# niclasborlin/dbat

Measured on AMD Instinct MI355X. Metric: LM iterations/sec, higher is better.
Workload: dtype f64

## Files before the change

### dbat_amd/csrc/dbat_core.hip

```cpp
#include <hip/hip_runtime.h>
#include <rocblas/rocblas.h>
#include <rocsolver/rocsolver.h>
#include <rccl/rccl.h>

#include <chrono>
#include <cmath>
#include <cstdio>
#include <cstdlib>
#include <memory>
#include <string>
#include <thread>
#include <type_traits>
#include <utility>
#include <atomic>
#include <vector>

#include "../../include/dbat_hip.h"
#include "chol_df.hpp"
#include "kernels.hpp"
#include "sig.hpp"
#include "heavy.hpp"
#include "plan.hpp"
#include "resect.hpp"
#include "robust.hpp"
// ... 82 lines not shown
    DevBuf<double> io_fixed, px, cam_w, z_prw, z_prv, o_uv, o_w;
    bool deterministic = false;
    DevBuf<double> det_cam_part, det_io_part, det_rr, det_u;
    DevBuf<int32_t> det_cam_chunks;
    DevBuf<double> o_rhs;
    bool uv_pre = false;
    DevBuf<uint8_t> z_est, z_mine, o_lc, o_pidx;
    DevBuf<int32_t> tile_batch, tile_cam_start, tile_cams, tile_io_start, tile_iocols;
    DevBuf<uint8_t> tile_io_simple;
    DevBuf<uint8_t> tile_cam_io;
    DevBuf<int32_t> sg_chunk, sg_tile_chunk0, sg_gcam;
    int64_t sg_nchunks = 0;
    DevBuf<uint8_t> sg_lc;
    DevBuf<double> sg_uv, sg_w;
    bool use_sig = false;
    int sig_rb = 4;
    int tile_ncx = 6;
    int64_t ntiles = 0;
    size_t lds_tile2 = 0, lds_tile3 = 0;
    int tile2_pc = TILE2_PC;
    bool use_tile2 = true;
    enum class TileRoute { none, sig, tile3, tile2 } route = TileRoute::none;
    DevBuf<int64_t> o_row, batch_start, x2z, giant_start, cm_chunk_start;
    DevBuf<int32_t> cm_pt, cm_chunk_cam, tile_order;
    DevBuf<double> cm_uv, cm_w;
    int64_t n_cm_chunks = 0, n_cm_chunks_all = 0;
    DevBuf<double> giant_W;
    int64_t ngiant = 0;
    bool use_heavy = false;
    HeavyDev hv{};
    DevBuf<int32_t> hv_obs_dst, hv_pt_io0, hv_io_dst, hv_io_pt, hv_pt_y, hv_grp_nb, hv_grp_row, hv_task, hv_ops;
    DevBuf<uint8_t> hv_obs_ld, hv_obs_ioloc, hv_io_ld;
    DevBuf<double> hv_Z;
    int giant_threads = 256;
    DevBuf<CamRec> cams, cams_f;
    bool cams_at_lin = false;

    const char *env_df_trace = nullptr;
    DevBuf<unsigned> gctr;
    DevBuf<double> gpart, rpart;
    DevBuf<double> z, zt, dz, zlin, vtmp, vtmp2, xbuf;
    DevBuf<double> red;
    DevBuf<double> jn2c, dscale, rhs, Vinv, gp, jn2p, partial, scal;
    DevBuf<int> info;
    DevBuf<double> linv, ldiag;
    DataflowChol dfchol;
    DataflowChol dfchol_ip;
    bool use_perm = true;
    bool mg_subtree = false;
    DevBuf<uint8_t> piv_have;
    bool chol_in_place = false;
    int64_t ldS = 0;
    CholEnvelope env;
    DevBuf<unsigned long long> pivmm;
    double *S = nullptr, *g_red = nullptr, *g_c = nullptr, *diagU = nullptr, *red_scal = nullptr;
    int64_t red_count = 0;
    DevBuf<double> pk;
    DevBuf<int> col_bend;
    DevBuf<int64_t> col_off;
    int64_t pk_s_count = 0;
    int env_tail0 = 0;
    int64_t nb = 0, nobs = 0;
    int grid_obs = 1, grid_z = 1, grid_zs = 1;
    size_t lds_build = 0, lds_back = 0, lds_cov = 0;
    ncclComm_t nccl = nullptr;
    dbat_hip_allreduce_fn allreduce = nullptr;
    void *allreduce_user = nullptr;
    DevBuf<double> zgather;
    bool multi() const { return nccl != nullptr || allreduce != nullptr; }
    struct { const void *kernel; size_t bytes; } lds_opt_in[8] = {};
    int n_lds_opt_in = 0;
    template <auto K, class... A>
    void launch(dim3 grid, dim3 block, size_t lds, A &&...args) {
        if (lds > 65536) {
            int i = 0;
            while (i < n_lds_opt_in && lds_opt_in[i].kernel != (const void *)K) ++i;
            if (i == n_lds_opt_in || lds_opt_in[i].bytes < lds) {
                if (i == 8) throw DeviceError{"internal: more kernels with over 64 KiB of LDS than the opt-in table holds"};
                HIPCHK(hipFuncSetAttribute((const void *)K, hipFuncAttributeMaxDynamicSharedMemorySize, (int)lds));
                lds_opt_in[i] = {(const void *)K, lds};
                n_lds_opt_in = std::max(n_lds_opt_in, i + 1);
            }
        }
        dbat::launch<K>(grid, block, lds, stream, std::forward<A>(args)...);
    }
    double f_lin = 0, trace_jtj = 0, lambda_lin = 0;
    int scale_lin = 0;
    bool have_lin = false;
    bool s_valid = false;
    bool s_dense_dirty = true;
    int n_res_evals = 0, n_lin = 0, n_solves = 0, n_trace_only = 0;

    ~Core() {
        for (auto &e : ev) if (e) (void)hipEventDestroy(e);
        for (auto &e : kev) if (e) (void)hipEventDestroy(e);
        for (auto &e : st_ev) if (e) (void)hipEventDestroy(e);
        dfchol.release(); dfchol_ip.release();
        if (hpin) (void)hipHostFree(hpin);
        if (nccl) (void)ncclCommDestroy(nccl);
        if (blas) rocblas_destroy_handle(blas);
        if (stream) (void)hipStreamDestroy(stream);
    }

    void init(const dbat_hip_problem &pb) {
        const bool init_clock = env_int("DBAT_HIP_PLAN_STATS", 0) >= 2;
        auto t_init = std::chrono::steady_clock::now();
        auto lapi = [&](const char *what) {
            if (!init_clock) return;
            const auto now = std::chrono::steady_clock::now();
            fprintf(stderr, "[create clock] %-60s %8.1f ms\n", what, std::chrono::duration<double, std::milli>(now - t_init).count());
            t_init = now;
        };
        device = pb.device;
        HIPCHK(hipSetDevice(pb.device));
        {
            hipDeviceProp_t prop;
            HIPCHK(hipGetDeviceProperties(&prop, pb.device));
            n_cu = std::max(1, prop.multiProcessorCount);
        }
        HIPCHK(hipStreamCreate(&stream));
        HIPCHK(hipHostMalloc((void **)&hpin, 64 * sizeof(double), hipHostMallocMapped | hipHostMallocCoherent));
        memset(hpin, 0, 64 * sizeof(double));
        {
            const double big = 1e300;
            memcpy(&hpin[48], &big, 8); hpin[49] = 0.0; memcpy(&hpin[50], &big, 8); hpin[51] = 0.0;
        }
        lapi("device, stream, pinned mailbox (the first call of a process initialises the HIP runtime: ~0.1 s)");
        for (auto &e : ev) HIPCHK(hipEventCreate(&e));
        for (auto &e : kev) HIPCHK(hipEventCreate(&e));
        lapi("events");
        nb = (int64_t)P.batch_start.size() - 1;
        nobs = (int64_t)P.o_cam.size();
        cam_ncol.upload(P.cam_ncol); cam_col.upload(P.cam_col); cam_iorow.upload(P.cam_iorow);
        cam_eo_est.upload(P.cam_eo_est); io_src.upload(P.io_src); io_fixed.upload(P.io_fixed);
        px.upload(P.px); cam_w.upload(P.cam_w);
        z_est.upload(P.z_est); z_mine.upload(P.z_mine); z_prw.upload(P.z_prw); z_prv.upload(P.z_prv);
        o_cam.upload(P.o_cam); o_pt.upload(P.o_pt); o_uv.upload(P.o_uv); o_w.upload(P.o_w);
        o_seg.upload(P.o_seg); o_row.upload(P.o_row); batch_start.upload(P.batch_start);
        x2z.upload(P.x2z);
        o_lc.upload(P.o_lc); o_pidx.upload(P.o_pidx); tile_batch.upload(P.tile_batch); tile_cam_start.upload(P.tile_cam_start); tile_cams.upload(P.tile_cams);
        tile_io_start.upload(P.tile_io_start); tile_iocols.upload(P.tile_iocols); tile_cam_io.upload(P.tile_cam_io);
        tile_ncx = P.shared_eo ? MAXCOL : (P.ncolmax <= 6 ? 6 : (P.ncolmax <= 14 ? 14 : (P.ncolmax <= 15 ? 15 : MAXCOL)));
        ntiles = (P.CMAX && P.nb_tiled > 0) ? (int64_t)P.tile_batch.size() - 1 : 0;
        d.nc = P.nc; d.np = P.np; d.nIOrows = P.nIOrows; d.nK = P.nK; d.nP = P.nP; d.nIOu = P.nIOu;
        d.ncolmax = P.ncolmax; d.BT = P.BT; d.NS = P.NS; d.NZ = P.NZ; d.nobs = nobs; d.nb = nb;
        d.cam_ncol = cam_ncol.p; d.cam_col = cam_col.p; d.cam_iorow = cam_iorow.p; d.cam_eo_est = cam_eo_est.p;
        d.io_src = io_src.p; d.io_fixed = io_fixed.p; d.px = px.p; d.cam_w = cam_w.p;
        d.z_est = z_est.p; d.z_mine = z_mine.p; d.z_prw = z_prw.p; d.z_prv = z_prv.p;
        d.o_cam = o_cam.p; d.o_pt = o_pt.p; d.o_uv = o_uv.p; d.o_w = P.uniform_w ? nullptr : o_w.p;
        pw = !P.uniform_w;
        d.o_seg = o_seg.p; d.o_row = o_row.p; d.batch_start = batch_start.p;
        d.CMAX = P.CMAX; d.ablate = env_int("DBAT_HIP_ABLATE", 0); d.trace_only = 0;
        d.any_prior = 0;
        for (double w : P.z_prw) if (w > 0) { d.any_prior = 1; break; }
        d.deterministic = 0; d.det_cam_part = d.det_io_part = d.det_rr = d.det_u = nullptr; d.det_cam_chunks = nullptr;
        env_df_trace = env_get("DBAT_HIP_DF_TRACE");
        d.ntiles = (int)ntiles; d.o_lc = o_lc.p; d.o_pidx = o_pidx.p;
        tile_order.upload(P.tile_order); d.tile_order = tile_order.p;
        cm_pt.upload(P.cm_pt); cm_uv.upload(P.cm_uv); cm_w.upload(P.cm_w);
        cm_chunk_cam.upload(P.cm_chunk_cam); cm_chunk_start.upload(P.cm_chunk_start);
        n_cm_chunks = P.n_cm_chunks_tiled; n_cm_chunks_all = (int64_t)P.cm_chunk_cam.size();
        ngiant = P.giant_start.empty() ? 0 : (int64_t)P.giant_start.size() - 1;
        if (ngiant > 0) {
            giant_start.upload(P.giant_start);
            giant_W.alloc((size_t)(P.giant_start.back() - P.giant_start.front()) * P.ncolmax * 3);
        }
        d.ngiant = (int)ngiant; d.giant_start = giant_start.p; d.giant_W = giant_W.p;
        use_heavy = P.hv_ok;
        if (use_heavy) {
            hv_obs_dst.upload(P.hv_obs_dst); hv_obs_ld.upload(P.hv_obs_ld); hv_obs_ioloc.upload(P.hv_obs_ioloc);
            hv_pt_io0.upload(P.hv_pt_io0); hv_io_dst.upload(P.hv_io_dst); hv_io_ld.upload(P.hv_io_ld); hv_io_pt.upload(P.hv_io_pt);
            hv_pt_y.upload(P.hv_pt_y); hv_grp_nb.upload(P.hv_grp_nb); hv_grp_row.upload(P.hv_grp_row);
            hv_task.upload(P.hv_task); hv_ops.upload(P.hv_ops);
            hv_Z.alloc((size_t)P.hv_z_doubles);
            HIPCHK(hipMemset(hv_Z.p, 0, (size_t)P.hv_z_doubles * sizeof(double)));
            hv.obs_dst = hv_obs_dst.p; hv.obs_ld = hv_obs_ld.p; hv.obs_ioloc = hv_obs_ioloc.p; hv.pt_io0 = hv_pt_io0.p;
            hv.io_dst = hv_io_dst.p; hv.io_ld = hv_io_ld.p; hv.io_pt = hv_io_pt.p; hv.pt_y = hv_pt_y.p;
            hv.grp_nb = hv_grp_nb.p; hv.grp_row = hv_grp_row.p; hv.task = hv_task.p; hv.ops = hv_ops.p;
            hv.obs0 = P.hv_obs0; hv.pt0 = P.hv_pt0; hv.ntasks = P.hv_ntasks; hv.max_batch_slots = P.hv_max_batch_slots;
        }
        if (const char *e = env_get("DBAT_HIP_GIANT_THREADS")) giant_threads = atoi(e);
        d.tile_batch = tile_batch.p; d.tile_cam_start = tile_cam_start.p; d.tile_cams = tile_cams.p;
        d.tile_io_start = tile_io_start.p; d.tile_iocols = tile_iocols.p; d.tile_cam_io = tile_cam_io.p;
        tile_io_simple.upload(P.tile_io_simple); d.tile_io_simple = P.tile_io_simple.empty() ? nullptr : tile_io_simple.p;
        use_sig = P.sg_ok && ntiles > 0 && tile_ncx <= 14;
        if (use_sig) {
            sg_chunk.upload(P.sg_chunk); sg_tile_chunk0.upload(P.sg_tile_chunk0); sg_lc.upload(P.sg_lc); sg_gcam.upload(P.sg_gcam);
            sg_nchunks = (int64_t)P.sg_chunk.size() / 8;
            sg_uv.upload(P.sg_uv);
            if (!P.uniform_w) sg_w.upload(P.sg_w);
            sig_rb = P.sg_rows_max <= 64 ? 4 : 5;
        }
        lapi("allocations and uploads of the plan");
        cams.alloc(P.nc); cams_f.alloc(P.nc);
        z.alloc(P.NZ); zt.alloc(P.NZ); dz.alloc(P.NZ); zlin.alloc(P.NZ); vtmp.alloc(P.NZ); vtmp2.alloc(P.NZ);
        xbuf.alloc(std::max<int64_t>(P.n, 1));
        ldS = ((P.NS + 1 + 7) / 8) * 8;
        d.ldS = ldS;
        const int64_t s_count = ldS * (P.NS + 1);
        red_count = s_count + 3 * P.NS + 8;
        red.alloc(red_count);
        S = red.p; g_red = S + s_count; g_c = g_red + P.NS; diagU = g_c + P.NS; red_scal = diagU + P.NS;
        ldiag.alloc(P.NS);
        {
            std::vector<int> first((size_t)P.NS, 0);
            for (int c = 0; c < P.nc; ++c)
                for (int k = 0; k < 6; ++k) first[(size_t)6 * c + k] = 6 * P.cam_first[c];
            if (P.shared_eo) env.build_dense((int)P.NS);
            else env.build((int)P.NS, 6 * P.nc, first);
            {
                const int NSi = (int)P.NS;
                std::vector<int> cb((size_t)NSi);
                std::vector<int64_t> co((size_t)NSi + 1, 0);
                env_tail0 = env.tail0;
                for (int c = 0; c < NSi; ++c) {
                    const int be = c >= env.tail0 ? c : std::min(std::max(env.band_end[c / CHOL_NB], c + 1), env.tail0);
                    cb[c] = be;
                    co[c + 1] = co[c] + (be - c) + (NSi - std::max(env.tail0, be));
                }
                pk_s_count = co[NSi];
                col_bend.upload(cb); col_off.upload(co);
            }
            use_perm = !P.shared_eo;
            if (!dfchol_ip.setup_inplace(env, ldS)) throw DeviceError{"out of device memory (Cholesky schedule)"};
            if (use_perm) {
                if (!dfchol.setup_permuted(P.nc, P.nIOu, P.cam_adj.data(), P.cam_adj_words, P.nd, P.rank))
                    throw DeviceError{"out of device memory (Cholesky schedule)"};
            }
            mg_subtree = P.mg_subtree && use_perm && dfchol.two_phase;
            if (mg_subtree) {
                std::vector<uint8_t> have((size_t)P.NS, 0);
                for (int c = 0; c < P.nc; ++c)
                    if (P.nd.cam_owner[c] < 0 || P.nd.cam_owner[c] == P.rank) for (int k = 0; k < 6; ++k) have[(size_t)6 * c + k] = 1;
                for (int64_t z = 6 * (int64_t)P.nc; z < P.NS; ++z) have[z] = 1;
                piv_have.upload(have);
            }
            linv.alloc(std::max(dfchol_ip.linv_doubles(), use_perm ? dfchol.linv_doubles() : (size_t)0));
        }
        lapi("envelope, schedules of the factorisation");
        jn2c.alloc(P.NS); dscale.alloc(P.NS); rhs.alloc(P.NS);
        Vinv.alloc((size_t)6 * P.np); gp.alloc((size_t)3 * P.np); jn2p.alloc((size_t)3 * P.np);
        HIPCHK(hipMemset(Vinv.p, 0, (size_t)6 * P.np * 8));
        HIPCHK(hipMemset(gp.p, 0, (size_t)3 * P.np * 8));
        HIPCHK(hipMemset(jn2p.p, 0, (size_t)3 * P.np * 8));
        grid_obs = (int)std::max<int64_t>(1, std::min<int64_t>(cdiv(nobs, 256), env_grid_obs()));
        grid_z = (int)std::max<int64_t>(1, std::min<int64_t>(cdiv(P.NZ, 256), 2048));
        grid_zs = (int)std::max<int64_t>(1, std::min<int64_t>(cdiv(P.NZ, 2048), 256));
        scal.alloc((size_t)16 + 4 * (size_t)P.nranks);
        HIPCHK(hipMemset(scal.p, 0, ((size_t)16 + 4 * (size_t)P.nranks) * sizeof(double)));
        info.alloc(1);
        pivmm.alloc(4);
        gctr.alloc(16); HIPCHK(hipMemset(gctr.p, 0, 16 * sizeof(unsigned)));
        rpart.alloc((size_t)grid_obs);
        gpart.alloc((size_t)8 * std::max<int64_t>(std::max<int64_t>(grid_z, cdiv(P.NS, 256)), 2048));
        lds_build = ((size_t)P.BT * P.ncolmax * 3 + (size_t)P.BT * 18) * sizeof(double);
        lds_back = (size_t)P.BT * 6 * sizeof(double);
        lds_cov = ((size_t)P.BT * P.ncolmax * 3 + (size_t)P.BT * 6) * sizeof(double);
        tile2_pc = TILE2_PC;
        static_assert(Plan::PMAX == 256 / 2, "k_build_tile2 / k_build_tile3 lay out NPROD / 2 points per batch");
        lds_tile2 = ((size_t)TILE2_NBUF * 3 * tile2_pc * TILE_LD + (size_t)2 * Plan::PMAX * 9 + (size_t)Plan::PMAX * 15 + TILE_LD) * sizeof(double);
        lds_tile3 = ((size_t)TILE3_NBUF * 3 * TILE3_PC * TILE_LD + (size_t)2 * Plan::PMAX * 9 + (size_t)2 * Plan::PMAX * 9 + TILE_LD) * sizeof(double);
        use_tile2 = P.BT == 256 && P.ncolmax <= 15;
        if (ntiles <= 0) route = TileRoute::none;
        else if (use_sig) route = TileRoute::sig;
        else if (use_tile2 && !P.with_io && tile_ncx == 6) route = TileRoute::tile3;
        else if (use_tile2 && (tile_ncx == 14 || tile_ncx == 15)) route = TileRoute::tile2;
        else throw DeviceError{"internal: tiles without a tile kernel"};
        partial.alloc((size_t)4 * std::max<int64_t>(std::max<int64_t>(std::max<int64_t>(nb + ntiles + ngiant + (int64_t)P.sg_chunk.size() / 8, n_cm_chunks_all), 2048), 1));
        HIPCHK(hipMemcpy(z.p, P.z0.data(), P.NZ * 8, hipMemcpyHostToDevice));
        HIPCHK(hipMemset(dz.p, 0, P.NZ * 8));
        HIPCHK(hipMemset(zt.p, 0, P.NZ * 8));
        precompute_image_side();
        HIPCHK(hipDeviceSynchronize());
        lapi("work arrays, image side");
    }

    void precompute_image_side() {
        uv_pre = !P.with_io;
        d.o_uv_raw = o_uv.p; d.uv_pre = uv_pre ? 1 : 0;
        if (!uv_pre || nobs == 0) return;
        prep_cams(z.p, cams_f.p);
        if (!o_rhs.p) o_rhs.alloc((size_t)2 * nobs);
        with_value<2, 3, 4, 5>(P.model, [&](auto M) {
            launch<k_uv_to_rhs<M>>(dim3((unsigned)cdiv(nobs, 256)), dim3(256), 0, d.nK, d.nP, cams_f.p, nobs, o_cam.p, o_uv.p, o_rhs.p);
            if (n_cm_chunks_all > 0) launch<k_uv_to_rhs_cm<M>>(dim3((unsigned)n_cm_chunks_all), dim3(256), 0, d.nK, d.nP, cams_f.p, cm_chunk_cam.p, cm_chunk_start.p, cm_uv.p);
            if (use_sig && sg_nchunks > 0) launch<k_uv_to_rhs_sig<M>>(dim3((unsigned)sg_nchunks), dim3(64), 0, d.nK, d.nP, cams_f.p, sg_chunk.p, sg_gcam.p, sg_uv.p);
        });
        d.o_uv = o_rhs.p;
    }

    void set_values(bool io_changed) {
        robust_reset();
        HIPCHK(hipMemcpyAsync(z.p, P.z0.data(), P.NZ * 8, hipMemcpyHostToDevice, stream));
        HIPCHK(hipMemcpyAsync(io_fixed.p, P.io_fixed.data(), P.io_fixed.size() * 8, hipMemcpyHostToDevice, stream));
        if (d.any_prior) {
            HIPCHK(hipMemcpyAsync(z_prw.p, P.z_prw.data(), P.NZ * 8, hipMemcpyHostToDevice, stream));
            HIPCHK(hipMemcpyAsync(z_prv.p, P.z_prv.data(), P.NZ * 8, hipMemcpyHostToDevice, stream));
        }
        HIPCHK(hipStreamSynchronize(stream));
        if (uv_pre && io_changed && nobs > 0) {
            HIPCHK(hipMemcpy(cm_uv.p, P.cm_uv.data(), P.cm_uv.size() * 8, hipMemcpyHostToDevice));
            if (use_sig && sg_nchunks > 0) HIPCHK(hipMemcpy(sg_uv.p, P.sg_uv.data(), P.sg_uv.size() * 8, hipMemcpyHostToDevice));
            d.o_uv = o_uv.p;
            precompute_image_side();
            HIPCHK(hipStreamSynchronize(stream));
        }
        cams_at_lin = false; have_lin = false; s_valid = false; pend_build = false; lin_pending = false;
        lambda_lin = 0; scale_lin = 0; f_lin = 0; trace_jtj = 0; near_singular = false; chol_in_place = false; replicate_next = false;
        n_res_evals = n_lin = n_solves = n_trace_only = 0;
    }

    static int env_grid_obs() { return std::min(std::max(1, env_int("DBAT_HIP_GRID_OBS", 1536)), 1 << 20); }

    int64_t tile_kernel_mfma() const {
        if (route == TileRoute::none) return 0;
        int64_t n = 0;
        if (route == TileRoute::sig) {
            for (int64_t t = 0; t < ntiles; ++t) {
                const int nio = tile_ncx > 6 ? P.tile_io_start[t + 1] - P.tile_io_start[t] : 0;
                for (int64_t q = P.sg_tile_chunk0[t]; q < P.sg_tile_chunk0[t + 1]; ++q) {
                    const int npts = P.sg_chunk[8 * q + 1], k = P.sg_chunk[8 * q + 2];
                    const int ppr = std::min(SIG_PPR, 64 / std::max(k, 1)), rbk = (6 * k + nio + 1 + 15) >> 4;
                    for (int p0 = 0; p0 < npts; p0 += ppr) n += (int64_t)((3 * std::min(ppr, npts - p0) + 3) >> 2) * (rbk * (rbk + 1) / 2);
                }
            }
            return n;
        }
        const int pc = route == TileRoute::tile3 ? TILE3_PC : tile2_pc;
        for (int64_t b = 0; b < P.nb_tiled; ++b) {
            const int64_t o1 = P.batch_start[b + 1];
            const int npts = o1 > P.batch_start[b] ? (int)P.o_pidx[o1 - 1] + 1 : 0;
            for (int p0 = 0; p0 < npts; p0 += pc) n += (int64_t)((3 * std::min(pc, npts - p0) + 3) >> 2) * 36;
        }
        return n;
    }

    bool lin_pending = false;
    bool det_timeout_pending = false;
    unsigned long long mb_seq = 0;
    bool mb_armed = false;
    void sync() {
        bool done = false;
        if (mb_armed) {
            volatile unsigned long long *slot = reinterpret_cast<volatile unsigned long long *>(hpin) + 63;
            const auto t_end = std::chrono::steady_clock::now() + std::chrono::milliseconds(20);
            for (;;) {
                for (int spin = 0; spin < 512 && !done; ++spin) { done = *slot == mb_seq; if (!done) cpu_relax(); }
                if (done || std::chrono::steady_clock::now() >= t_end) break;
            }
            __atomic_thread_fence(__ATOMIC_ACQUIRE);
            mb_armed = false;
        }
        if (!done) HIPCHK(hipStreamSynchronize(stream));
        if (det_timeout_pending) {
            det_timeout_pending = false;
            unsigned n_to = 0;
            memcpy(&n_to, hpin + 60, sizeof(unsigned));
            if (n_to) {
                HIPCHK(hipMemsetAsync(gctr.p + 7, 0, sizeof(unsigned), stream));
                throw DeviceError{"deterministic mode: " + std::to_string(n_to) + " chunk(s) of the signature kernel gave up waiting for their turn at "
                                  "the tile (spin cap): the sums of this linearisation are not order-fixed"};
            }
        }
        if (lin_pending) {
            f_lin = 0.5 * hpin[32];
            trace_jtj = hpin[34] + hpin[33];
            lin_pending = false;
        }
    }
    void mark(int i) { if (timing) HIPCHK(hipEventRecord(kev[i], stream)); }
    std::vector<hipEvent_t> st_ev;
    std::vector<int> st_id;
    bool st_on = false;
    void stage(int id) {
        if (!st_on) return;
        if (st_id.size() == st_ev.size()) { hipEvent_t e; HIPCHK(hipEventCreate(&e)); st_ev.push_back(e); }
        HIPCHK(hipEventRecord(st_ev[st_id.size()], stream));
        st_id.push_back(id);
    }
    void stages_begin() { st_id.clear(); st_on = true; stage(4); }
    void stages_end(double *out5) {
        stage(4);
        st_on = false;
        HIPCHK(hipStreamSynchronize(stream));
        for (int i = 0; i < 5; ++i) out5[i] = 0.0;
        for (size_t i = 0; i + 1 < st_id.size(); ++i) {
            float ms = 0;
            HIPCHK(hipEventElapsedTime(&ms, st_ev[i], st_ev[i + 1]));
            out5[st_id[i]] += 1e-3 * ms;
        }
    }
    void allreduce_system() {
        if (!multi()) return;
        const int64_t nvec = 3 * P.NS + 8;
        if (!pk.p) pk.alloc((size_t)(pk_s_count + nvec));
        launch<k_pack_envelope>(dim3((unsigned)P.NS), dim3(256), 0, S, ldS, (int)P.NS, env_tail0,
                           col_bend.p, col_off.p, pk.p, 1);
        HIPCHK(hipMemcpyAsync(pk.p + pk_s_count, g_red, nvec * sizeof(double), hipMemcpyDeviceToDevice, stream));
        do_allreduce(pk.p, pk_s_count + nvec);
        launch<k_pack_envelope>(dim3((unsigned)P.NS), dim3(256), 0, S, ldS, (int)P.NS, env_tail0,
                           col_bend.p, col_off.p, pk.p, 0);
        HIPCHK(hipMemcpyAsync(g_red, pk.p + pk_s_count, nvec * sizeof(double), hipMemcpyDeviceToDevice, stream));
    }
    void do_allreduce(double *buf, int64_t count) {
        if (nccl) {
            NCCLCHK(ncclAllReduce(buf, buf, (size_t)count, ncclDouble, ncclSum, nccl, stream));
        } else if (allreduce) {
            if (allreduce(allreduce_user, buf, count, (void *)stream) != 0) throw DeviceError{"all-reduce callback failed"};
        }
    }
    const double *gathered(const double *z_dev) {
        if (!multi()) return z_dev;
        if (!zgather.p) zgather.alloc((size_t)P.NZ);
        launch<k_mask_owned>(dim3((unsigned)cdiv(P.NZ, 256)), dim3(256), 0, P.NZ, z_mine.p, z_dev, zgather.p);
        do_allreduce(zgather.p, P.NZ);
        return zgather.p;
    }
    void read_scal(double *host, int n) {
        if (n <= 32) {
            HIPCHK(hipMemcpyAsync(hpin, scal.p, n * sizeof(double), hipMemcpyDeviceToHost, stream));
            sync();
            memcpy(host, hpin, n * sizeof(double));
            return;
        }
        HIPCHK(hipMemcpyAsync(host, scal.p, n * sizeof(double), hipMemcpyDeviceToHost, stream));
        sync();
    }
    void prep_cams(const double *zz, CamRec *into = nullptr) {
        if (!into) { into = cams.p; cams_at_lin = false; }
        launch<k_cam_prep>(dim3((unsigned)cdiv(P.nc, 64)), dim3(64), 0, d, zz, into);
    }
    void x_to_z(const double *x_host, double *z_dev) {
        HIPCHK(hipMemcpyAsync(z_dev, P.z0.data(), P.NZ * 8, hipMemcpyHostToDevice, stream));
        if (P.n) {
            HIPCHK(hipMemcpyAsync(xbuf.p, x_host, P.n * 8, hipMemcpyHostToDevice, stream));
            launch<k_scatter_x>(dim3((unsigned)cdiv(P.n, 256)), dim3(256), 0, P.n, x2z.p, xbuf.p, z_dev);
        }
    }
    void z_to_x(const double *z_dev, double *x_host) {
        if (!P.n) return;
        stage(4);
        z_dev = gathered(z_dev);
        launch<k_gather_x>(dim3((unsigned)cdiv(P.n, 256)), dim3(256), 0, P.n, x2z.p, z_dev, xbuf.p);
        HIPCHK(hipMemcpyAsync(x_host, xbuf.p, P.n * 8, hipMemcpyDeviceToHost, stream));
        sync();
    }

    DevBuf<double> trace_dev;
    int trace_cap = 0, trace_n = 0;
    std::vector<uint8_t> trace_have;
    void trace_begin() { trace_n = 0; trace_have.clear(); }
    void trace_put(int k, const double *z_dev) {
        if (!P.n || k < 0) return;
        if (k >= trace_cap) {
            const int cap = std::max(8, std::max(2 * trace_cap, k + 1));
            DevBuf<double> nb;
            nb.alloc((size_t)P.n * cap);
            if (trace_cap > 0) HIPCHK(hipMemcpyAsync(nb.p, trace_dev.p, (size_t)P.n * trace_cap * 8, hipMemcpyDeviceToDevice, stream));
            HIPCHK(hipStreamSynchronize(stream));
            std::swap(trace_dev.p, nb.p);
            trace_cap = cap;
        }
        stage(4);
        z_dev = gathered(z_dev);
        launch<k_gather_x>(dim3((unsigned)cdiv(P.n, 256)), dim3(256), 0, P.n, x2z.p, z_dev, trace_dev.p + (size_t)P.n * k);
        if ((int)trace_have.size() <= k) trace_have.resize((size_t)k + 1, 0);
        trace_have[k] = 1;
        trace_n = std::max(trace_n, k + 1);
    }
    void trace_truncate(int n) { trace_n = std::min(trace_n, std::max(n, 0)); }
    int trace_download(double *host, int cap_cols) {
        const int nt = std::min(trace_n, cap_cols);
        if (!P.n || nt <= 0) return std::max(nt, 0);
        HIPCHK(hipMemcpyAsync(host, trace_dev.p, (size_t)P.n * nt * 8, hipMemcpyDeviceToHost, stream));
        HIPCHK(hipStreamSynchronize(stream));
        for (int k = 0; k < nt; ++k)
            if (!trace_have[k]) std::fill(host + (size_t)P.n * k, host + (size_t)P.n * (k + 1), NAN);
        if ((size_t)P.n * trace_cap * 8 > ((size_t)256 << 20)) {
            DevBuf<double> old;
            std::swap(old.p, trace_dev.p);
            trace_cap = 0;
        }
        return nt;
    }

    double eval_f_step(const double *x, double alpha, const double *pdir, double *out) {
        stage(3);
        if ((int64_t)cdiv(P.NZ, 256) < P.nc) { axpby(1.0, x, alpha, pdir, out); return eval_f(out, nullptr, nullptr); }
        launch<k_axpby_cams>(dim3((unsigned)cdiv(P.NZ, 256)), dim3(256), 0, d, 1.0, x, alpha, pdir, out, cams_f.p);
        return eval_f(out, nullptr, nullptr, true);
    }
    double eval_f(const double *zz, double *r_w_out, double *r_unw_out, bool cams_ready = false) {
        stage(3);
        if (!cams_ready) prep_cams(zz, cams_f.p);
        mark(6);
        const bool res_tail = n_cm_chunks_all > 0 && n_cm_chunks_all <= 512 && !d.any_prior && !multi() && !r_w_out && !r_unw_out;
        with_value<2, 3, 4, 5>(P.model, [&](auto M) {
            with_value<false, true>(uv_pre, [&](auto PRE) {
                if (n_cm_chunks_all > 0)
                    launch<k_residual_cm<M, PRE>>(dim3((unsigned)n_cm_chunks_all), dim3(256), 0, d, zz, cams_f.p, cm_pt.p, cm_uv.p, pw ? cm_w.p : (const double *)nullptr,
                                                  cm_chunk_cam.p, cm_chunk_start.p, partial.p, res_tail ? gctr.p + 1 : (unsigned *)nullptr, scal.p, hpin, res_tail ? ++mb_seq : 0ull);
                mark(7);
                if (r_w_out || r_unw_out) launch<k_residual<M, PRE>>(dim3(grid_obs), dim3(256), 0, d, zz, cams_f.p, rpart.p, r_w_out, r_unw_out);
            });
        });
        if (!res_tail)
            launch<k_prior_sq>(dim3(grid_zs), dim3(1024), 0, d, zz, gpart.p, gctr.p + 1, (const double *)partial.p, n_cm_chunks_all,
                               scal.p, multi() ? (double *)nullptr : hpin, ++mb_seq);
        double s;
        if (multi()) { do_allreduce(scal.p, 1); read_scal(&s, 1); }
        else { mb_armed = true; sync(); s = hpin[0]; }
        ++n_res_evals;
        return 0.5 * s;
    }

    int det_ncx() const { return P.ncolmax <= 6 ? 6 : (P.ncolmax <= 14 ? 14 : 15); }
    bool deterministic_supported() const { return P.nranks == 1 && !P.shared_eo && P.ncolmax <= 15 && n_cm_chunks_all > 0; }
    void set_deterministic(bool on) {
        if (on && !deterministic_supported())
            throw UsageError{"deterministic mode: one rank, no shared EO blocks (camera stations), at most nine estimated IO columns per camera"};
        if (on && !det_u.p) {
            const int nc = P.nc;
            det_cam_part.alloc((size_t)std::max<int64_t>(n_cm_chunks_all, 1) * DET_CP);
            det_io_part.alloc((size_t)nc * DET_IOP);
            det_rr.alloc((size_t)nc + 1 + DET_PRIOR_PARTS);
            det_u.alloc((size_t)P.NS + 1);
            std::vector<int32_t> cr((size_t)2 * (2 * nc + 1), 0);
            for (int part = 0; part < 2; ++part) {
                const int64_t q0 = part == 0 ? 0 : n_cm_chunks, q1 = part == 0 ? n_cm_chunks : n_cm_chunks_all;
                int32_t *r = cr.data() + part * (2 * nc + 1);
                for (int c = 0; c < nc; ++c) { r[2 * c] = (int32_t)q1; r[2 * c + 1] = (int32_t)q1; }
                for (int64_t q = q0; q < q1; ++q) {
                    const int c = P.cm_chunk_cam[q];
                    if (r[2 * c] == (int32_t)q1) r[2 * c] = (int32_t)q;
                    r[2 * c + 1] = (int32_t)q + 1;
                }
                for (int c = 0; c < nc; ++c) if (r[2 * c] == (int32_t)q1) r[2 * c + 1] = (int32_t)q1;
            }
            det_cam_chunks.upload(cr);
        }
        deterministic = on;
        d.deterministic = on ? 1 : 0;
        d.det_cam_part = det_cam_part.p; d.det_io_part = det_io_part.p; d.det_rr = det_rr.p; d.det_u = det_u.p;
        d.det_cam_chunks = det_cam_chunks.p;
    }
    const double *det_z = nullptr;
    void det_camera_side() {
        const int nio = (int)P.nIOu;
        const int ncx = det_ncx();
        with_value<6, 14, 15>(ncx, [&](auto NCX) { launch<k_det_cam_reduce<NCX>>(dim3((unsigned)P.nc), dim3(256), 0, d, cams.p, S, g_c, g_red, diagU); });
        if (ncx > 6 && nio > 0) launch<k_det_io_reduce<15>>(dim3((unsigned)(nio * (nio + 1) / 2 + nio)), dim3(256), 0, d, cams.p, nio, S, g_c, g_red, diagU);
        if (d.any_prior) launch<k_det_prior_sq>(dim3(DET_PRIOR_PARTS), dim3(256), 0, d, det_z);
        launch<k_det_rows>(dim3((unsigned)cdiv(P.NS, 256)), dim3(256), 0, d, (const double *)diagU);
        if (ncx == 6) launch<k_det_round_cam<6>>(dim3((unsigned)P.nc), dim3(256), 0, d, cams.p, 0, S, g_red);
        else launch<k_det_round_cam<15>>(dim3((unsigned)P.nc + 1), dim3(256), 0, d, cams.p, nio, S, g_red);
    }

    void cam_normal(const double *zz, int64_t q0, int64_t nq, int ncx) {
        const double *w = pw ? cm_w.p : (const double *)nullptr;
        with_value<2, 3, 4, 5>(P.model, [&](auto M) { with_value<6, 14, 15>(ncx, [&](auto NCX) {
            if constexpr (NCX == 6)
                launch<k_cam_normal6<M>>(dim3((unsigned)nq), dim3(256), 0, d, zz, cams.p, cm_pt.p, cm_uv.p, w, cm_chunk_cam.p + q0, cm_chunk_start.p + q0, S, g_c, g_red, diagU);
            else
                launch<k_cam_normal<M, NCX>>(dim3((unsigned)nq), dim3(256), 0, d, zz, cams.p, cm_pt.p, cm_uv.p, w, cm_chunk_cam.p + q0, cm_chunk_start.p + q0, S, g_c, g_red, diagU);
        }); });
    }

    void build_enqueue(const double *zz, double lambda, int scale) {
        stage(0);
        const bool fused_first = !s_dense_dirty && P.NS >= P.nc;
        if (!fused_first) prep_cams(zz);
        else cams_at_lin = false;
        bool pivmm_set = false;
        if (s_dense_dirty) {
            HIPCHK(hipMemsetAsync(red.p, 0, red_count * sizeof(double), stream));
            s_dense_dirty = false;
        } else {
            launch<k_envelope_cams>(dim3((unsigned)P.NS), dim3(256), 0, d, zz, cams.p, S, ldS, (int)P.NS, env_tail0, col_bend.p, g_red, pivmm.p);
            pivmm_set = true;
        }
        if (!pivmm_set) HIPCHK(hipMemcpyAsync(pivmm.p, hpin + 48, 4 * sizeof(double), hipMemcpyHostToDevice, stream));
        int64_t npart = 0;
        const bool det_list = deterministic && route != TileRoute::sig;
        const int64_t nb_tiled = det_list ? 0 : P.nb_tiled;
        if (deterministic) {
            cam_normal(zz, 0, n_cm_chunks_all, det_ncx());
            det_z = zz;
            det_camera_side();
        }
        if (ntiles > 0 && nb_tiled > 0) {
            npart = ntiles;
            if (!deterministic && use_tile2 && tile_ncx <= 15 && n_cm_chunks > 0) cam_normal(zz, 0, n_cm_chunks, tile_ncx);
            mark(0);
            with_value<2, 3, 4, 5>(P.model, [&](auto M) {
                if (route == TileRoute::sig) {
                    with_value<6, 14>(tile_ncx, [&](auto NCX) { with_value<4, 5>(sig_rb, [&](auto RB) { with_value<false, true>(pw, [&](auto PW) {
                        launch<k_build_sig<M, RB, NCX, PW>>(dim3((unsigned)std::min<int64_t>(ntiles, n_cu)), dim3(64 * sig_waves(RB, NCX > 6)), sig_lds_bytes(RB, NCX > 6),
                                                            d, zz, cams.p, lambda, scale, S, g_red, Vinv.p, gp.p, jn2p.p, partial.p, pivmm.p, sg_chunk.p, sg_tile_chunk0.p,
                                                            sg_lc.p, sg_uv.p, PW ? sg_w.p : (const double *)nullptr, gctr.p + 5);
                    }); }); });
                } else if (route == TileRoute::tile3) {
                    launch<k_build_tile3<M, TILE3_PC, TILE3_NBUF>>(dim3((unsigned)ntiles), dim3(768), lds_tile3, d, zz, cams.p, lambda, scale, S, g_red, Vinv.p, gp.p,
                                                                   jn2p.p, partial.p, pivmm.p);
                } else {
                    with_value<14, 15>(tile_ncx, [&](auto NCX) {
                        launch<k_build_tile2<M, NCX, TILE2_PC, TILE2_NBUF>>(dim3((unsigned)ntiles), dim3(512), lds_tile2, d, zz, cams.p, lambda, scale, S, g_c, g_red,
                                                                            diagU, Vinv.p, gp.p, jn2p.p, partial.p, pivmm.p);
                    });
                }
            });
            mark(1);
        }
        const bool no_tiles = !(ntiles > 0 && nb_tiled > 0);
        if (no_tiles) mark(0);
        const int64_t nb_lists = use_heavy ? P.nb_tiled : nb;
        if (nb_lists > nb_tiled) {
            with_value<2, 3, 4, 5>(P.model, [&](auto M) { with_value<false, true>(P.with_io, [&](auto IO) {
                launch<k_build<M, IO>>(dim3((unsigned)(nb_lists - nb_tiled)), dim3(P.BT), lds_build, d, zz, cams.p, lambda, scale, S, g_c, g_red, diagU, Vinv.p, gp.p,
                                       jn2p.p, partial.p + npart, pivmm.p, (int)nb_tiled);
            }); });
            npart += nb_lists - nb_tiled;
        }
        if (use_heavy) {
            mark(10);
            if (!deterministic && n_cm_chunks_all > n_cm_chunks) cam_normal(zz, n_cm_chunks, n_cm_chunks_all - n_cm_chunks, tile_ncx);
            if (nb > P.nb_tiled) {
                with_value<2, 3, 4, 5>(P.model, [&](auto M) { with_value<6, 14, 15>(tile_ncx, [&](auto NCX) {
                    launch<k_heavy_z<M, NCX>>(dim3((unsigned)(nb - P.nb_tiled)), dim3(256), heavy_z_lds_bytes(NCX, P.hv_max_batch_slots, deterministic), d, hv, zz,
                                              cams.p, lambda, scale, hv_Z.p, Vinv.p, gp.p, jn2p.p, partial.p + npart, pivmm.p, (int)P.nb_tiled);
                }); });
                npart += nb - P.nb_tiled;
            }
            if (ngiant > 0) {
                with_value<2, 3, 4, 5>(P.model, [&](auto M) { with_value<6, 14, 15>(tile_ncx, [&](auto NCX) {
                    launch<k_heavy_z_giant<M, NCX>>(dim3((unsigned)ngiant), dim3(giant_threads), 0, d, hv, zz, cams.p, lambda, scale, hv_Z.p, Vinv.p, gp.p, jn2p.p,
                                                    partial.p + npart, pivmm.p);
                }); });
                npart += ngiant;
            }
            mark(11);
            launch<k_heavy_syrk>(dim3((unsigned)cdiv(hv.ntasks, 4)), dim3(256), 0, d, hv, (const double *)hv_Z.p, S, g_red);
            mark(12);
        }
        if (no_tiles) mark(1);
        if (ngiant > 0 && !use_heavy) {
            with_value<2, 3, 4, 5>(P.model, [&](auto M) { with_value<false, true>(P.with_io, [&](auto IO) {
                launch<k_build_giant<M, IO>>(dim3((unsigned)ngiant), dim3(giant_threads), 0, d, zz, cams.p, lambda, scale, S, g_c, g_red, diagU, Vinv.p, gp.p, jn2p.p,
                                             partial.p + npart, pivmm.p);
            }); });
            npart += ngiant;
        }
        if (deterministic && route == TileRoute::sig && !no_tiles) {
            HIPCHK(hipMemcpyAsync(hpin + 60, gctr.p + 7, sizeof(unsigned), hipMemcpyDeviceToHost, stream));
            det_timeout_pending = true;
        }
        if ((d.ablate & 32) && use_heavy && nb > P.nb_tiled) {
            unsigned long long h[16];
            HIPCHK(hipStreamSynchronize(stream));
            HIPCHK(hipMemcpyFromSymbol(h, HIP_SYMBOL(g_tile2_prof), sizeof(h)));
            static const char *nm[6] = {"evaluate", "V, g sums", "point blocks", "EO rows of Z", "IO rows of Z", "tail"};
            fprintf(stderr, "[heavy_z prof, us per batch (thread 0) avg over %d batches]", (int)(nb - P.nb_tiled));
            for (int i = 0; i < 6; ++i) fprintf(stderr, " %s=%.2f", nm[i], h[8 + i] * 0.01 / (double)std::max<int64_t>(nb - P.nb_tiled, 1));
            fprintf(stderr, "\n");
            for (int i = 8; i < 16; ++i) h[i] = 0;
            HIPCHK(hipMemcpyToSymbol(HIP_SYMBOL(g_tile2_prof), h, sizeof(h)));
        }
        if ((d.ablate & 32) && use_sig) {
            unsigned long long h[16];
            HIPCHK(hipStreamSynchronize(stream));
            HIPCHK(hipMemcpyFromSymbol(h, HIP_SYMBOL(g_tile2_prof), sizeof(h)));
            static const char *nm[8] = {"tile init", "chunk head", "pass 1", "pass 2 eval+write", "pass 2 mfma", "chunk flush", "wait for the tile", "tile flush"};
            fprintf(stderr, "[sig prof, us per tile (wave 0) avg over %d tiles]", (int)ntiles);
            for (int i = 0; i < 8; ++i) fprintf(stderr, " %s=%.2f", nm[i], h[i] * 0.01 / (double)std::max<int64_t>(ntiles, 1));
            fprintf(stderr, "\n");
            memset(h, 0, sizeof(h));
            HIPCHK(hipMemcpyToSymbol(HIP_SYMBOL(g_tile2_prof), h, sizeof(h)));
        } else if ((d.ablate & 32) && use_tile2) {
            unsigned long long h[16];
            HIPCHK(hipStreamSynchronize(stream));
            HIPCHK(hipMemcpyFromSymbol(h, HIP_SYMBOL(g_tile2_prof), sizeof(h)));
            static const char *nm[12] = {"stage(wait freed)", "P1", "pbarrier", "P2", "P3", "drain", "cons wait full", "cons zero+free", "tail/flush", "loop head", "cons product", "cons wait done"};
            fprintf(stderr, "[tile2 prof, us per tile avg over %d tiles]", (int)ntiles);
            for (int i = 0; i < 12; ++i) fprintf(stderr, " %s=%.2f", nm[i], h[i] * 0.01 / (double)std::max<int64_t>(ntiles, 1));
            fprintf(stderr, "\n");
            memset(h, 0, sizeof(h));
            HIPCHK(hipMemcpyToSymbol(HIP_SYMBOL(g_tile2_prof), h, sizeof(h)));
        }
        launch<k_build_tail>(dim3(grid_zs), dim3(1024), 0, d, zz, partial.p, npart, jn2p.p, gpart.p, gctr.p + 2, red_scal,
                zz != zlin.p ? zlin.p : (double *)nullptr);
    }
    bool pend_build = false;
    double pend_lambda = 0;
    int pend_scale = 0;
    void request_build(double lambda, int scale) {
        pend_build = true; pend_lambda = lambda; pend_scale = scale;
        lambda_lin = lambda; scale_lin = scale;
    }
    void ensure_build() {
        if (!pend_build) return;
        build(z.p, pend_lambda, pend_scale, true);
    }
    void settle_lin_point() {
        if (!pend_build) return;
        copy(zlin.p, z.p);
        cams_at_lin = false; s_valid = false; have_lin = true;
    }
    void allreduce_vectors() {
        if (!multi()) return;
        do_allreduce(g_c, 2 * P.NS + 8);
    }
    void trace_only_pass(const double *zz) {
        stage(0);
        prep_cams(zz);
        if (n_cm_chunks_all > 0) {
            with_value<2, 3, 4, 5>(P.model, [&](auto M) { with_value<6, 14, 15, MAXCOL>(tile_ncx, [&](auto NCX) {
                launch<k_trace_cm<M, NCX>>(dim3((unsigned)n_cm_chunks_all), dim3(256), 0, d, zz, cams.p, cm_pt.p, cm_uv.p, pw ? cm_w.p : (const double *)nullptr,
                                           cm_chunk_cam.p, cm_chunk_start.p, partial.p);
            }); });
        }
        launch<k_trace_tail>(dim3(grid_zs), dim3(1024), 0, d, gpart.p, gctr.p + 6, (const double *)partial.p, n_cm_chunks_all, hpin, ++mb_seq);
        mb_armed = true; lin_pending = true;
        sync();
        pend_build = false;
        lambda_lin = NAN; have_lin = false; s_valid = false;
        ++n_trace_only;
    }
    void build(const double *zz, double lambda, int scale, bool lazy = false, bool trace_only = false) {
        if (trace_only && !multi() && P.nranks == 1) { trace_only_pass(zz); return; }
        pend_build = false;
        trace_only = trace_only && use_sig && ntiles > 0;
        d.trace_only = trace_only ? 1 : 0;
        try { build_enqueue(zz, lambda, scale); } catch (...) { d.trace_only = 0; throw; }
        d.trace_only = 0;
        if (mg_subtree) allreduce_vectors();
        else allreduce_system();
        finish_enqueue(zz, lambda, scale);
        if (mg_subtree && replicate_next && multi()) allreduce_matrix();
        cams_at_lin = true;
        lin_pending = true;
        if (!lazy) sync();
        lambda_lin = trace_only ? NAN : lambda;
        scale_lin = scale;
        have_lin = !trace_only;
        s_valid = !trace_only;
        if (!trace_only) ++n_lin; else ++n_trace_only;
    }
    bool replicate_next = false;
    void allreduce_matrix() {
        if (!pk.p) pk.alloc((size_t)(pk_s_count + 3 * P.NS + 8));
        launch<k_pack_envelope>(dim3((unsigned)P.NS), dim3(256), 0, S, ldS, (int)P.NS, env_tail0, col_bend.p, col_off.p, pk.p, 1);
        do_allreduce(pk.p, pk_s_count);
        launch<k_pack_envelope>(dim3((unsigned)P.NS), dim3(256), 0, S, ldS, (int)P.NS, env_tail0, col_bend.p, col_off.p, pk.p, 0);
    }
    void finish_enqueue(const double *zz, double lambda, int scale) {
        int *df_ctl = nullptr; unsigned long long *df_q = nullptr; int df_nq = 0;
        const bool ride = use_perm && !chol_in_place && !(mg_subtree && multi()) && dfchol.reset_args(df_ctl, df_q, df_nq);
        launch<k_finish>(dim3((unsigned)cdiv(P.NS, 256)), dim3(256), 0, d, zz, lambda, scale, S, g_c, g_red, diagU, jn2c.p, dscale.p,
                gpart.p, gctr.p + 3, (const double *)red_scal, scal.p, hpin, mg_subtree && multi() ? (const uint8_t *)z_mine.p : (const uint8_t *)nullptr,
                ride ? info.p : (int *)nullptr, ride ? df_ctl : (int *)nullptr, ride ? df_q : (unsigned long long *)nullptr, ride ? df_nq : 0);
        if (ride) dfchol.reset_done = true;
        if (scale)
            launch<k_envelope_op>(dim3((unsigned)P.NS), dim3(256), 0, S, ldS, (int)P.NS, env_tail0, col_bend.p, (const double *)dscale.p, (double *)nullptr,
                                  (unsigned long long *)nullptr);
    }

    int factor_solve_enqueue() {
        if (mg_subtree && !multi())
            throw UsageError{"this handle is one of several shards: attach a communicator (dbat_hip_comm_init) or an all-reduce "
                             "callback (dbat_hip_set_allreduce) before linearising or solving"};
        stage(1);
        mark(2);
        if (use_perm && !chol_in_place && mg_subtree && multi()) {
            dfchol.solve_domain(stream, S, ldS, linv.p, info.p, ldiag.p);
            mark(8);
            do_allreduce(dfchol.top_tiles(), dfchol.top_tiles_count());
            mark(9);
            dfchol.solve_top(stream, ldS, rhs.p, linv.p, info.p, ldiag.p, dscale.p, dz.p);
        } else if (use_perm && !chol_in_place) dfchol.solve(stream, S, ldS, rhs.p, linv.p, info.p, ldiag.p, dscale.p, dz.p);
        else dfchol_ip.solve(stream, S, ldS, rhs.p, linv.p, info.p, ldiag.p, dscale.p, dz.p);
        HIPCHK(hipGetLastError());
        if (env_df_trace) (use_perm && !chol_in_place ? dfchol : dfchol_ip).dump_trace(stream, env_df_trace);
        mark(3);
        ++n_solves;
        return 0;
    }
    void backsub_enqueue() {
        stage(2);
        mark(4);
        const bool sig_bs = use_sig && P.sg_backsub_ok;
        const int64_t b_first = sig_bs ? P.nb_tiled : 0;
        const int64_t n_sig_wg = sig_bs ? cdiv(sg_nchunks, 4) : 0;
        if (n_sig_wg > 0) {
            with_value<2, 3, 4, 5>(P.model, [&](auto M) { with_value<6, 14>(tile_ncx, [&](auto NCX) {
                launch<k_backsub_sig<M, NCX>>(dim3((unsigned)n_sig_wg), dim3(256), 0, d, zlin.p, cams.p, Vinv.p, gp.p, dz.p, partial.p + 2 * (nb + ngiant), sg_chunk.p,
                                              (int)sg_nchunks, sg_gcam.p, sg_uv.p, pw ? sg_w.p : (const double *)nullptr);
            }); });
        }
        if (nb > b_first) {
            with_value<2, 3, 4, 5>(P.model, [&](auto M) { with_value<6, 14, 15, MAXCOL>(tile_ncx, [&](auto NCX) {
                launch<k_backsub<M, NCX>>(dim3((unsigned)(nb - b_first)), dim3(P.BT), lds_back, d, zlin.p, cams.p, Vinv.p, gp.p, dz.p, partial.p, (int)b_first);
            }); });
        }
        if (ngiant > 0) {
            with_value<2, 3, 4, 5>(P.model, [&](auto M) { with_value<false, true>(P.with_io, [&](auto IO) {
                launch<k_backsub_giant<M, IO>>(dim3((unsigned)ngiant), dim3(giant_threads), 0, d, zlin.p, cams.p, Vinv.p, gp.p, dz.p, partial.p + 2 * nb);
            }); });
        }
        mark(5);
        launch<k_prior_jv>(dim3(grid_zs), dim3(1024), 0, d, zlin.p, dz.p, g_c, gp.p, gpart.p, gctr.p + 4,
                (const double *)(partial.p + 2 * b_first), nb - b_first + ngiant + n_sig_wg, (const double *)ldiag.p, pivmm.p,
                (const int *)info.p, scal.p, multi() ? (double *)nullptr : hpin, ++mb_seq,
                mg_subtree && multi() ? (const uint8_t *)piv_have.p : (const uint8_t *)nullptr);
    }
    bool near_singular = false;
    const bool pivot_stats = env_on("DBAT_HIP_PIVOT_STATS");
    double rcond_est = 0.0;
    int chol_info = 0;
    double piv_last[4] = {0, 0, 0, 0};
    bool solve(double &JpJp, double &rJp, double &pp) {
        ensure_build();
        if (!s_valid) build(zlin.p, lambda_lin, scale_lin);
        s_valid = false;
        factor_solve_enqueue();
        if (!cams_at_lin) { prep_cams(zlin.p); cams_at_lin = true; }
        backsub_enqueue();
        int hinfo = 0;
        unsigned long long hmm[4];
        const int nsl = multi() ? 4 * P.nranks : 0;
        std::vector<double> h((size_t)8 + nsl);
        if (nsl) {
            HIPCHK(hipMemcpyAsync(hpin + 40, pivmm.p, sizeof(hmm), hipMemcpyDeviceToHost, stream));
            HIPCHK(hipMemcpyAsync(hpin + 44, info.p, sizeof(hinfo), hipMemcpyDeviceToHost, stream));
            HIPCHK(hipMemsetAsync(scal.p + 8, 0, (size_t)nsl * sizeof(double), stream));
            HIPCHK(hipMemcpyAsync(scal.p + 8 + 4 * P.rank, pivmm.p, 4 * sizeof(double), hipMemcpyDeviceToDevice, stream));
            do_allreduce(scal.p, 8 + nsl);
            read_scal(h.data(), 8 + nsl);
        } else {
            mb_armed = true;
            sync();
            memcpy(h.data(), hpin, 8 * sizeof(double));
        }
        memcpy(hmm, hpin + 40, sizeof(hmm));
        memcpy(&hinfo, hpin + 44, sizeof(hinfo));
        JpJp = h[0] + h[4]; rJp = h[1] + h[5]; pp = h[6];
        double mm[4];
        memcpy(mm, hmm, sizeof(mm));
        double pmin = std::min(mm[0], mm[2]), pmax = std::max(mm[1], mm[3]);
        for (int r = 0; r < nsl / 2; ++r) { pmin = std::min(pmin, h[8 + 2 * r]); pmax = std::max(pmax, h[8 + 2 * r + 1]); }
        const bool failed = hinfo != 0 || (nsl && h[7] > 0) || !std::isfinite(pp) || !std::isfinite(JpJp);
        if (failed && !(use_perm && !chol_in_place)) s_dense_dirty = true;
        const double ratio = pmax > 0 ? pmin / pmax : 0.0;
        near_singular = failed || !(ratio * ratio >= 2.220446049250313e-16);
        rcond_est = failed ? 0.0 : ratio * ratio;
        chol_info = hinfo;
        for (int q = 0; q < 4; ++q) piv_last[q] = mm[q];
        if (pivot_stats)
            fprintf(stderr, "[solve] pivots of the point blocks %.3e ... %.3e, of the reduced system %.3e ... %.3e, info %d, rcond estimate %.3e\n",
                    mm[0], mm[1], mm[2], mm[3], hinfo, rcond_est);
        return failed;
    }
    std::vector<double> cop_tmp;
    SinvView inverse_at_z(bool want_dense) {
        const bool selinv = use_perm && !multi() && !want_dense && dfchol.selinv_supported() && !env_on("DBAT_HIP_COV_DENSE");
        replicate_next = !selinv;
        try { build(z.p, 0.0, 0); } catch (...) { replicate_next = false; throw; }
        replicate_next = false;
        s_valid = false;
        SinvView SV;
        int hinfo = 0;
        if (selinv) {
            factor_solve_enqueue();
            HIPCHK(hipMemcpyAsync(&hinfo, info.p, sizeof(hinfo), hipMemcpyDeviceToHost, stream));
            sync();
            if (hinfo != 0) throw DeviceError{"posterior covariance: the reduced normal matrix is not positive definite"};
            if (!dfchol.selected_inverse(stream, linv.p)) throw DeviceError{"out of device memory (selected inverse)"};
            HIPCHK(hipGetLastError());
            SV.tiles = dfchol.d_ztiles; SV.toff = dfchol.d_toff; SV.perm = dfchol.d_perm; SV.nT = dfchol.nT;
        } else {
            chol_in_place = true;
            s_dense_dirty = true;
            factor_solve_enqueue();
            chol_in_place = false;
            HIPCHK(hipMemcpyAsync(&hinfo, info.p, sizeof(hinfo), hipMemcpyDeviceToHost, stream));
            sync();
            if (hinfo != 0) throw DeviceError{"posterior covariance: the reduced normal matrix is not positive definite"};
            if (!blas) {
                if (rocblas_create_handle(&blas) != rocblas_status_success) throw DeviceError{"rocblas_create_handle failed"};
                rocblas_set_stream(blas, stream);
            }
            if (rocsolver_dpotri(blas, rocblas_fill_lower, (rocblas_int)P.NS, S, (rocblas_int)ldS, info.p) != rocblas_status_success)
                throw DeviceError{"rocsolver_dpotri failed"};
            SV.dense = S; SV.ld = ldS;
        }
        have_lin = false;
        prep_cams(z.p);
        return SV;
    }
    void posterior_cov(double s0, double *hCEO, double *hCIO, double *hCOP, double *hSinv) {
        const SinvView SV = inverse_at_z(hSinv != nullptr);
        const double s02 = s0 * s0;
        DevBuf<double> dCEO, dCIO, dCOP;
        if (hCEO) dCEO.alloc((size_t)36 * P.nc);
        if (hCIO && P.nIOu > 0) dCIO.alloc((size_t)P.nIOu * P.nIOu);
        if (hCEO || (hCIO && P.nIOu > 0)) {
            const int64_t tot = 36 * (int64_t)P.nc + (int64_t)P.nIOu * P.nIOu;
            launch<k_cov_cam>(dim3((unsigned)cdiv(tot, 256)), dim3(256), 0, d, SV, s02, dCEO.p, dCIO.p);
        }
        if (hCOP) {
            dCOP.alloc((size_t)9 * P.np);
            HIPCHK(hipMemsetAsync(dCOP.p, 0, (size_t)9 * P.np * sizeof(double), stream));
            with_value<2, 3, 4, 5>(P.model, [&](auto M) { with_value<false, true>(P.with_io, [&](auto IO) {
                if (nb > 0) launch<k_cov_points<M, IO>>(dim3((unsigned)nb), dim3(P.BT), lds_cov, d, z.p, cams.p, Vinv.p, SV, s02, dCOP.p, HatOut{});
                if (ngiant > 0) launch<k_cov_giant<M, IO>>(dim3((unsigned)ngiant), dim3(giant_threads), 0, d, z.p, cams.p, Vinv.p, SV, s02, dCOP.p, HatOut{});
            }); });
            if (multi()) do_allreduce(dCOP.p, (int64_t)9 * P.np);
            cop_tmp.resize((size_t)9 * P.np);
            HIPCHK(hipMemcpyAsync(cop_tmp.data(), dCOP.p, (size_t)9 * P.np * sizeof(double), hipMemcpyDeviceToHost, stream));
        }
        if (hCEO) HIPCHK(hipMemcpyAsync(hCEO, dCEO.p, (size_t)36 * P.nc * sizeof(double), hipMemcpyDeviceToHost, stream));
        if (hCIO && P.nIOu > 0) HIPCHK(hipMemcpyAsync(hCIO, dCIO.p, (size_t)P.nIOu * P.nIOu * sizeof(double), hipMemcpyDeviceToHost, stream));
        if (hSinv)
            HIPCHK(hipMemcpy2DAsync(hSinv, (size_t)P.NS * sizeof(double), S, (size_t)ldS * sizeof(double),
                                    (size_t)P.NS * sizeof(double), (size_t)P.NS, hipMemcpyDeviceToHost, stream));
        sync();
        if (hCOP)
            for (int64_t p = 0; p < P.np; ++p)
                std::copy(cop_tmp.begin() + 9 * (int64_t)P.pt_rank[p], cop_tmp.begin() + 9 * (int64_t)P.pt_rank[p] + 9, hCOP + 9 * p);
    }
    void redundancy(double *hqvv, double *hrp) {
        const SinvView SV = inverse_at_z(false);
        const int64_t nprior = (int64_t)P.prior_z.size();
        DevBuf<double> qvv, dCz, Ccc, gscr, rp;
        DevBuf<int64_t> pz;
        qvv.alloc((size_t)3 * std::max<int64_t>(P.no, 1));
        dCz.alloc((size_t)P.NZ);
        Ccc.alloc((size_t)P.nc * P.ncolmax * P.ncolmax);
        HIPCHK(hipMemsetAsync(qvv.p, 0, (size_t)3 * P.no * sizeof(double), stream));
        HIPCHK(hipMemsetAsync(dCz.p, 0, (size_t)P.NZ * sizeof(double), stream));
        const int64_t nCcc = (int64_t)P.nc * P.ncolmax * P.ncolmax;
        if (nCcc > 0) launch<k_hat_cam_blocks>(dim3((unsigned)cdiv(nCcc, 256)), dim3(256), 0, d, cams.p, SV, Ccc.p);
        HatOut hat;
        hat.Ccc = Ccc.p; hat.qvv = qvv.p; hat.dCz = dCz.p;
        if (ngiant > 0) {
            gscr.alloc((size_t)(P.giant_start.back() - P.giant_start.front()) * 9);
            hat.gscr = gscr.p;
        }
        with_value<2, 3, 4, 5>(P.model, [&](auto M) { with_value<false, true>(P.with_io, [&](auto IO) {
            if (nb > 0) launch<k_cov_points<M, IO, true>>(dim3((unsigned)nb), dim3(P.BT), lds_cov, d, z.p, cams.p, Vinv.p, SV, 1.0, (double *)nullptr, hat);
            if (ngiant > 0) launch<k_cov_giant<M, IO, true>>(dim3((unsigned)ngiant), dim3(giant_threads), 0, d, z.p, cams.p, Vinv.p, SV, 1.0, (double *)nullptr, hat);
        }); });
        if (multi()) {
            do_allreduce(qvv.p, 3 * P.no);
            do_allreduce(dCz.p + P.NS, P.NZ - P.NS);
        }
        if (nprior > 0) {
            rp.alloc((size_t)nprior);
            pz.alloc((size_t)nprior);
            HIPCHK(hipMemcpyAsync(pz.p, P.prior_z.data(), (size_t)nprior * sizeof(int64_t), hipMemcpyHostToDevice, stream));
            launch<k_hat_prior>(dim3((unsigned)cdiv(nprior, 256)), dim3(256), 0, d, SV, pz.p, nprior, dCz.p, rp.p);
            HIPCHK(hipMemcpyAsync(hrp, rp.p, (size_t)nprior * sizeof(double), hipMemcpyDeviceToHost, stream));
        }
        HIPCHK(hipMemcpyAsync(hqvv, qvv.p, (size_t)3 * P.no * sizeof(double), hipMemcpyDeviceToHost, stream));
        sync();
    }
    bool pw = false;
// ... 7 lines not shown
    unsigned robust_grid() const { return (unsigned)std::max<int64_t>(1, std::min<int64_t>(cdiv(nobs, 256), 4096)); }
    void robust_scratch() {
        if (rs_bits.p || rsel_state.p) return;
        rs_bits.alloc((size_t)std::max<int64_t>(nobs, 1));
        robust_r.alloc((size_t)2 * std::max<int64_t>(P.no, 1));
        rsel_hist.alloc(2 * RSEL_BINS); rsel_hist_f.alloc(2 * RSEL_BINS);
        HIPCHK(hipMemset(rsel_hist.p, 0, 2 * RSEL_BINS * sizeof(unsigned)));
        rsel_state.alloc(4); rmax.alloc(1); rsel_red.alloc((size_t)P.nranks);
    }
    void robust_promote() {
        if (robust_on) return;
        if (nobs >= ((int64_t)1 << 31) / 2) throw UsageError{"robust weights: more than 2^30 observations on one rank"};
        robust_scratch();
        const size_t n2 = (size_t)2 * std::max<int64_t>(nobs, 1);
        o_w_base.alloc(n2);
        if (P.uniform_w) {
            o_w.alloc(n2); cm_w.alloc(n2);
            if (use_sig) { sg_w.alloc(n2); HIPCHK(hipMemsetAsync(sg_w.p, 0, n2 * sizeof(double), stream)); }
            if (nobs > 0) launch<k_robust_base>(dim3(robust_grid()), dim3(256), 0, nobs, (const int32_t *)o_cam.p, (const double *)cam_w.p, o_w_base.p);
        } else if (nobs > 0) {
            HIPCHK(hipMemcpyAsync(o_w_base.p, o_w.p, (size_t)2 * nobs * sizeof(double), hipMemcpyDeviceToDevice, stream));
        }
        {
            std::vector<int32_t> cmm((size_t)nobs);
            const int64_t ntiled = P.nb_tiled > 0 ? P.batch_start[P.nb_tiled] : 0;
            std::vector<int64_t> cnt((size_t)P.nc + 1);
            for (int part = 0; part < 2; ++part) {
                const int64_t lo = part ? ntiled : 0, hi = part ? nobs : ntiled;
                std::fill(cnt.begin(), cnt.end(), 0);
                for (int64_t o = lo; o < hi; ++o) ++cnt[P.o_cam[o] + 1];
                for (int c = 0; c < P.nc; ++c) cnt[c + 1] += cnt[c];
                for (int64_t o = lo; o < hi; ++o) cmm[o] = (int32_t)(lo + cnt[P.o_cam[o]]++);
            }
            cm_map.upload(cmm);
        }
        if (use_sig) {
            std::vector<int32_t> sgm((size_t)nobs, -1);
            for (size_t q = 0; q < P.sg_chunk.size() / 8; ++q) {
                const int32_t *ch = &P.sg_chunk[8 * q];
                const int64_t npts = ch[1], k = ch[2], m = ch[4], i0 = ch[5], g0 = ch[6];
                for (int64_t i = i0; i < i0 + npts; ++i)
                    for (int64_t j = 0; j < k; ++j) sgm[g0 + i * k + j] = (int32_t)(g0 + j * m + i);
            }
            sg_map.upload(sgm);
        }
        omega.alloc((size_t)std::max<int64_t>(nobs, 1));
        robust_on = true; pw = true; d.o_w = o_w.p;
        robust_set_ones();
    }
    void robust_apply_omega() {
        if (nobs > 0)
            launch<k_robust_apply<false>>(dim3(robust_grid()), dim3(256), 0, nobs, (const uint64_t *)nullptr, 1.0, 0, 1.0, omega.p, (const double *)o_w_base.p, o_w.p,
                                          (const int32_t *)(use_sig ? sg_map.p : nullptr), sg_w.p, (const int32_t *)cm_map.p, cm_w.p);
        s_valid = false;
    }
    void robust_set_ones() {
        if (nobs > 0) launch<k_robust_fill>(dim3(robust_grid()), dim3(256), 0, nobs, 1.0, omega.p);
        robust_apply_omega();
    }
    void robust_reset() {
        if (robust_on) {
            HIPCHK(hipStreamSynchronize(stream));
            if (P.uniform_w) {
                dev_free(o_w); dev_free(cm_w);
                if (use_sig) dev_free(sg_w);
                d.o_w = nullptr;
            } else {
                HIPCHK(hipMemcpy(o_w.p, P.o_w.data(), P.o_w.size() * sizeof(double), hipMemcpyHostToDevice));
                HIPCHK(hipMemcpy(cm_w.p, P.cm_w.data(), P.cm_w.size() * sizeof(double), hipMemcpyHostToDevice));
                if (use_sig) HIPCHK(hipMemcpy(sg_w.p, P.sg_w.data(), P.sg_w.size() * sizeof(double), hipMemcpyHostToDevice));
            }
            dev_free(o_w_base); dev_free(omega); dev_free(sg_map); dev_free(cm_map);
            robust_on = false; pw = !P.uniform_w; s_valid = false;
        }
        dev_free(rs_bits); dev_free(robust_r); dev_free(rsel_hist); dev_free(rsel_hist_f); dev_free(rsel_state); dev_free(rmax); dev_free(rsel_red);
    }
    double max_over_ranks(double v) {
        if (!multi()) return v;
        std::vector<double> h((size_t)P.nranks, 0.0);
        h[P.rank] = v;
        HIPCHK(hipMemcpyAsync(rsel_red.p, h.data(), h.size() * sizeof(double), hipMemcpyHostToDevice, stream));
        do_allreduce(rsel_red.p, P.nranks);
        HIPCHK(hipMemcpyAsync(h.data(), rsel_red.p, h.size() * sizeof(double), hipMemcpyDeviceToHost, stream));
        HIPCHK(hipStreamSynchronize(stream));
        return *std::max_element(h.begin(), h.end());
    }
    double robust_median() {
        const uint64_t total = (uint64_t)P.no;
        uint64_t st[4] = {0, 0, (total - 1) / 2, total / 2};
        HIPCHK(hipMemcpyAsync(rsel_state.p, st, sizeof st, hipMemcpyHostToDevice, stream));
        const unsigned gh = (unsigned)std::max<int64_t>(1, std::min<int64_t>(cdiv(nobs, 4096), 1024));
        for (int pass = 0; pass < RSEL_PASSES; ++pass) {
            if (nobs > 0) launch<k_rsel_hist>(dim3(gh), dim3(256), 0, nobs, (const uint64_t *)rs_bits.p, (const uint64_t *)rsel_state.p, RSEL_SHIFT[pass], RSEL_BITS[pass], rsel_hist.p);
            if (multi()) {
                launch<k_rsel_to_f64>(dim3(16), dim3(256), 0, rsel_hist.p, rsel_hist_f.p);
                do_allreduce(rsel_hist_f.p, 2 * RSEL_BINS);
                launch<k_rsel_pick<true>>(dim3(1), dim3(256), 0, rsel_hist.p, (const double *)rsel_hist_f.p, rsel_state.p, RSEL_SHIFT[pass]);
            } else {
                launch<k_rsel_pick<false>>(dim3(1), dim3(256), 0, rsel_hist.p, (const double *)nullptr, rsel_state.p, RSEL_SHIFT[pass]);
            }
        }
        HIPCHK(hipMemcpyAsync(st, rsel_state.p, sizeof st, hipMemcpyDeviceToHost, stream));
        HIPCHK(hipStreamSynchronize(stream));
        double a, b;
        memcpy(&a, &st[0], 8); memcpy(&b, &st[1], 8);
        return (a + b) / 2.0;
    }
    void robust_eval(const double *zz, const dbat_hip_robust_options &ro, double *s_ip, double *omega_ip, double &scale, double &maxchg) {
        robust_scratch();
        HIPCHK(hipMemsetAsync(robust_r.p, 0, (size_t)2 * P.no * sizeof(double), stream));
        eval_f(zz, nullptr, robust_r.p);
        if (nobs > 0)
            launch<k_robust_norm>(dim3(robust_grid()), dim3(256), 0, nobs, (const int64_t *)o_row.p, (const double *)robust_r.p,
                                  (const double *)(robust_on ? o_w_base.p : (P.uniform_w ? nullptr : o_w.p)), (const int32_t *)o_cam.p, (const double *)cam_w.p, rs_bits.p, s_ip);
        scale = 1.0;
        if (ro.scale == DBAT_HIP_SCALE_MAD && P.no > 0) {
            scale = robust_median() / ROBUST_MAD_C;
            if (scale == 0.0) scale = 1.0;
        }
        HIPCHK(hipMemsetAsync(rmax.p, 0, sizeof(unsigned long long), stream));
        if (nobs > 0)
            launch<k_robust_weight>(dim3(robust_grid()), dim3(256), 0, nobs, (const uint64_t *)rs_bits.p, scale, (int)ro.loss, ro.k,
                                    (const double *)(robust_on ? omega.p : nullptr), (const int64_t *)o_row.p, omega_ip, rmax.p);
        unsigned long long mb = 0;
        HIPCHK(hipMemcpyAsync(&mb, rmax.p, sizeof mb, hipMemcpyDeviceToHost, stream));
        HIPCHK(hipStreamSynchronize(stream));
        memcpy(&maxchg, &mb, 8);
        maxchg = max_over_ranks(maxchg);
    }
    void robust_apply_eval(const dbat_hip_robust_options &ro, double scale) {
        robust_promote();
        if (nobs > 0)
            launch<k_robust_apply<true>>(dim3(robust_grid()), dim3(256), 0, nobs, (const uint64_t *)rs_bits.p, scale, (int)ro.loss, ro.k, omega.p,
                                         (const double *)o_w_base.p, o_w.p, (const int32_t *)(use_sig ? sg_map.p : nullptr), sg_w.p,
                                         (const int32_t *)cm_map.p, cm_w.p);
        s_valid = false;
    }
    void robust_omega_ip(double *host) {
        if (!robust_on) { std::fill(host, host + P.no, 1.0); return; }
        DevBuf<double> t;
        t.alloc((size_t)std::max<int64_t>(P.no, 1));
        HIPCHK(hipMemsetAsync(t.p, 0, (size_t)P.no * sizeof(double), stream));
        if (nobs > 0) launch<k_scatter_rows1>(dim3(robust_grid()), dim3(256), 0, nobs, (const int64_t *)o_row.p, (const double *)omega.p, t.p);
        if (multi()) do_allreduce(t.p, P.no);
        HIPCHK(hipMemcpyAsync(host, t.p, (size_t)P.no * sizeof(double), hipMemcpyDeviceToHost, stream));
        HIPCHK(hipStreamSynchronize(stream));
    }
    void jtimes(const double *v, double &JvJv, double &rJv, double &vv) {
        if (!cams_at_lin) { prep_cams(zlin.p); cams_at_lin = true; }
        with_value<2, 3, 4, 5>(P.model, [&](auto M) { with_value<6, 14, 15, MAXCOL>(tile_ncx, [&](auto NCX) {
            launch<k_jtimes<M, NCX>>(dim3(grid_obs), dim3(256), 0, d, zlin.p, cams.p, v, partial.p);
        }); });
        launch<k_prior_jv>(dim3(grid_zs), dim3(1024), 0, d, zlin.p, v, g_c, gp.p, gpart.p, gctr.p + 4,
                (const double *)partial.p, (int64_t)grid_obs, (const double *)nullptr, pivmm.p, (const int *)info.p, scal.p, (double *)nullptr, 0ull, (const uint8_t *)nullptr);
        do_allreduce(scal.p, 8);
        double h[8];
        read_scal(h, 8);
        JvJv = h[0] + h[4]; rJv = h[1] + h[5]; vv = h[6];
    }
    double dot_owned(const double *a, const double *b) {
        launch<k_dot>(dim3(grid_z), dim3(256), 0, P.NZ, z_mine.p, a, b, partial.p);
        launch<k_sum_partials<1>>(dim3(1), dim3(1024), 0, partial.p, (int64_t)grid_z, scal.p, 0);
        do_allreduce(scal.p, 1);
        double s;
        read_scal(&s, 1);
        return s;
    }
    void axpby(double a, const double *x, double b, const double *y2, double *y) {
        launch<k_axpby>(dim3((unsigned)cdiv(P.NZ, 256)), dim3(256), 0, P.NZ, a, x, b, y2, y);
    }
    void gradient(double *g) {
        launch<k_gradient>(dim3((unsigned)cdiv(P.NZ, 256)), dim3(256), 0, d, g_c, gp.p, g);
    }
    void colnorm2(double *out) {
        launch<k_jn2>(dim3((unsigned)cdiv(P.NZ, 256)), dim3(256), 0, d, jn2c.p, jn2p.p, out);
    }
    void jac_blocks(const double *zz, double *a, double *b, double *cc) {
        with_value<2, 3, 4, 5>(P.model, [&](auto M) { launch<k_jac_blocks<M>>(dim3((unsigned)cdiv(nobs, 256)), dim3(256), 0, d, zz, cams.p, a, b, cc); });
    }
    void copy(double *dst, const double *src) { HIPCHK(hipMemcpyAsync(dst, src, P.NZ * 8, hipMemcpyDeviceToDevice, stream)); }
    void accept_trial() { std::swap(z.p, zt.p); }
};


struct LoopOut {
    std::vector<double> res, damp, aux;
    int code = 0, iters = 0;
    double f_final = 0;
};

static void export_residuals(Core &c, const double *zdev, double *r_unw, double *r_wgt, double *f);
static void jtimes_rows(Core &c, const double *v_dev, double *Jv);

static void keep_Jp(Core &c, const dbat_hip_options &o, const double *p_dev, std::vector<double> &Jp) {
    if (!o.term_fun) return;
    Jp.resize((size_t)c.P.m);
    jtimes_rows(c, p_dev, Jp.data());
}
static bool term_fun(Core &c, const dbat_hip_options &o, double JpJp, double f, const std::vector<double> &Jp) {
    if (o.term_fun) {
        std::vector<double> r((size_t)c.P.m);
        export_residuals(c, c.z.p, nullptr, r.data(), nullptr);
        return o.term_fun(o.term_user, Jp.data(), r.data(), c.P.m) != 0;
    }
    const double nr = std::sqrt(2 * f);
    if (o.abs_term) return nr <= o.conv_tol;
    return std::sqrt(JpJp) <= o.conv_tol * nr;
}
static bool vetoed(Core &c, const dbat_hip_options &o) {
    if (!o.veto_fun) return false;
    std::vector<double> x((size_t)c.P.n);
    c.z_to_x(c.zt.p, x.data());
    return o.veto_fun(o.veto_user, x.data(), c.P.n) != 0;
}

static inline void trace_line(const dbat_hip_options &o, int n, double res, double damp, int step = -1, double rho = NAN) {
    if (o.trace_fun) o.trace_fun(o.trace_user, o.damping, n, res, damp, step, rho);
}

static void push_trace(Core &c, const dbat_hip_options &o, LoopOut &) {
    if (!o.store_trace) return;
    c.trace_put(c.trace_n, c.z.p);
}


static void loop_gna(Core &c, const dbat_hip_options &o, LoopOut &out) {
    int n = 0;
    std::vector<double> Jp_host;
    push_trace(c, o, out);
    double f = c.eval_f(c.z.p, nullptr, nullptr);
    while (true) {
        c.build(c.z.p, 0.0, 1, true);
        out.res.push_back(std::sqrt(2 * f));
        trace_line(o, n, out.res.back(), out.damp.empty() ? NAN : out.damp.back());
        if (n == 0 && !c.P.rank_ok) { out.code = -4; break; }
        double JpJp, rJp, pp;
        const bool failed = c.solve(JpJp, rJp, pp);
        if (failed || (o.singular_test && c.near_singular)) { out.code = -2; break; }
        keep_Jp(c, o, c.dz.p, Jp_host);
        if (term_fun(c, o, JpJp, f, Jp_host)) break;
        ++n;
        const double f0 = f, fp0 = rJp;
        double alpha = 1.0;
        bool found = false;
        while (alpha >= o.alpha_min) {
            const double ft = c.eval_f_step(c.z.p, alpha, c.dz.p, c.zt.p);
            if (ft < f0 + o.mu * alpha * fp0 && !vetoed(c, o)) { found = true; f = ft; break; }
            alpha /= 2;
        }
        if (!found) alpha = 0.0;
        else c.accept_trial();
        out.damp.push_back(alpha);
        push_trace(c, o, out);
        if (alpha == 0.0) { out.code = -3; out.res.push_back(out.res.back()); break; }
        if (n > o.max_iter) { out.code = -1; out.res.push_back(std::sqrt(2 * f)); break; }
    }
    out.iters = n;
    out.f_final = f;
}

static void loop_gm(Core &c, const dbat_hip_options &o, LoopOut &out) {
    int n = 0;
    std::vector<double> Jp_host;
    push_trace(c, o, out);
    double f = 0;
    while (true) {
        f = c.eval_f(c.z.p, nullptr, nullptr);
        c.build(c.z.p, 0.0, 0, true);
        out.res.push_back(std::sqrt(2 * f));
        trace_line(o, n, out.res.back(), NAN);
        double JpJp, rJp, pp;
        const bool failed = c.solve(JpJp, rJp, pp);
        if (failed || (o.singular_test && c.near_singular)) { out.code = -2; break; }
        keep_Jp(c, o, c.dz.p, Jp_host);
        if (term_fun(c, o, JpJp, f, Jp_host)) break;
        ++n;
        c.axpby(1.0, c.z.p, 1.0, c.dz.p, c.z.p);
        push_trace(c, o, out);
        if (n > o.max_iter) { out.code = -1; break; }
    }
    out.iters = n;
    out.f_final = f;
}

static bool lambda0_needs_trace(const dbat_hip_options &o) {
    const double l0 = std::fabs(o.lambda0), lm = std::fabs(o.lambda_min);
    return o.lambda0 < 0 && o.lambda_min < 0 && l0 >= lm && l0 > 0;
}

static void loop_lm(Core &c, const dbat_hip_options &o, LoopOut &out) {
    int n = 0;
    double f = c.eval_f(c.z.p, nullptr, nullptr);
    c.build(c.z.p, 0.0, 0, false, lambda0_needs_trace(o));
    const double nx = (double)c.P.n;
    double lambda0 = o.lambda0, lambdaMin = o.lambda_min;
    if (lambda0 < 0) lambda0 = std::fabs(lambda0) * c.trace_jtj / nx;
    if (lambdaMin < 0) lambdaMin = std::fabs(lambdaMin) * c.trace_jtj / nx;
    double lambda = lambda0;
    if (lambda < lambdaMin) lambda = 0;
    out.damp.push_back(lambda);
    double prevLambda = NAN;
    double JpJp = 0, rJp = 0, pp = 0;
    std::vector<double> Jp_host;
    while (true) {
        while (n <= o.max_iter) {
            if (c.lambda_lin != lambda) c.build(c.z.p, lambda, 0, true);
            const bool failed = c.solve(JpJp, rJp, pp);
            if (!failed) keep_Jp(c, o, c.dz.p, Jp_host);
            out.res.push_back(std::sqrt(2 * f));
            if (n == 0 && !c.P.rank_ok) { out.code = -4; break; }
            if (failed) { out.code = -2; break; }
            out.damp.push_back(lambda);
            trace_line(o, n, out.res.back(), n == 0 ? NAN : lambda);
            if (o.store_trace) c.trace_put(n, c.z.p);
            ++n;
            const double fNew = c.eval_f_step(c.z.p, 1.0, c.dz.p, c.zt.p);
            if (fNew < f && !vetoed(c, o)) {
                c.accept_trial();
                lambda = lambda / 10;
                if (lambda < lambdaMin) lambda = 0;
                c.request_build(lambda, 0);
                f = fNew;
                break;
            } else {
                if (lambda == 0) lambda = lambdaMin; else lambda = lambda * 10;
            }
        }
        if (out.code != 0) break;
        if (prevLambda == 0 && term_fun(c, o, JpJp, f, Jp_host)) break;
        prevLambda = lambda;
        if (n > o.max_iter) { out.code = -1; break; }
    }
    if (o.store_trace) c.trace_put(n, c.z.p);
    out.res.push_back(std::sqrt(2 * f));
// ... 1230 lines not shown
```

### dbat_amd/csrc/env.hpp

```cpp
#pragma once
#include <cstdlib>
#include <cstring>
#include <string>

extern char **environ;

namespace dbat {

#ifdef DBAT_HIP_PROFILING
constexpr bool kProfilingBuild = true;
#else
constexpr bool kProfilingBuild = false;
#endif

struct EnvSwitch { const char *name; bool measurement; const char *what; const char *values = nullptr; };
static const EnvSwitch kEnvSwitches[] = {
    {"DBAT_HIP_SIG", false, "0: signature kernels off, 2: on wherever a chunk's rows fit (default: by group length)", "0|1|2"},
    {"DBAT_HIP_SIG_IOS_OFF", false, "self-calibration: IO rows by LDS atomics in every tile"},
    {"DBAT_HIP_CMAX", false, "cameras per tile (0: column-list kernel only)"},
    {"DBAT_HIP_BT", false, "observations per batch (128 | 256)", "128|256"},
    {"DBAT_HIP_TILE_BMIN", false, "fewest batches a tile may be capped at (default 2)"},
    {"DBAT_HIP_HEAVY", false, "0: heavy / giant points by the column-list kernels (pair terms by global atomics) instead of the matrix-core path", "0|1"},
    {"DBAT_HIP_HEAVY_KS", false, "heavy / giant points: k-steps per task of k_heavy_syrk at most (default: by the amount of work, 12 ... 96)"},
    {"DBAT_HIP_GIANT_THREADS", false, "threads of the giant-point kernels (64 | 128 | 256)", "64|128|256"},
    {"DBAT_HIP_MG_REPLICATED", false, "several ranks: envelope summed, replicated factorisation"},
    {"DBAT_HIP_ND_OFF", false, "no nested dissection"},
    {"DBAT_HIP_ND_LEAF", false, "leaf size of the dissection"},
    {"DBAT_HIP_ND_PAD_ALL", false, "every block of the dissection on a tile boundary"},
    {"DBAT_HIP_ND_JOIN_SMALL", false, "separators up to that many rows join their child's last tile"},
    {"DBAT_HIP_DF_SPLIT", false, "factorisation: helper tasks for sums longer than this many products (default 96)"},
    {"DBAT_HIP_DF_CHUNK", false, "factorisation: products per helper task (default 32)"},
    {"DBAT_HIP_DF_CHAIN", false, "factorisation: 0 = diagonal tiles as ordinary tasks (no chain role), 1 = chain role whatever the pattern", "0|1"},
    {"DBAT_HIP_DF_CHAIN_WG", false, "factorisation: workgroups of the chain role at most (default 32)"},
    {"DBAT_HIP_DF_L2", false, "factorisation: 1 = finished tiles of the compact layout are read through the L2", "0|1"},
    {"DBAT_HIP_COV_DENSE", false, "posterior covariance: the dense inverse of the reduced system (rocsolver_dpotri) instead of the selected inversion"},
    {"DBAT_HIP_SPRANK_OFF", false, "structural rank from the counting conditions only"},
    {"DBAT_HIP_PLAN_THREADS", false, "threads of the host plan (default: hardware concurrency, at most 32)"},
    {"DBAT_HIP_PLAN_GRAIN", false, "elements per thread below which a pass of the host plan is not split (tests: 1)"},
    {"DBAT_HIP_PLAN_STATS", false, "1: print layout statistics, 2: also the wall time of every section of the plan"},
    {"DBAT_HIP_PIVOT_STATS", false, "print the pivot extremes and the rcond estimate of every solve"},
    {"DBAT_HIP_ABLATE", true, "k_build_sig / tile kernels: switch phases off (results are wrong), phase clocks"},
    {"DBAT_HIP_DF_TRACE", true, "per-task clocks of the factorisation, written to this file"},
    {"DBAT_HIP_DF_TRACE_POTF2", true, "with DF_TRACE: clocks inside the chain role's factorisations as well"},
    {"DBAT_HIP_DF_ABLATE", true, "factorisation: operand tiles of the products not fetched (1: L(i,j), 2: both, 3: and no flag looks) -- timing only, wrong results", "0|1|2|3"},
    {"DBAT_HIP_DF_ORDER", true, "one of the candidate task orders instead of the simulated best"},
    {"DBAT_HIP_DF_GRID", true, "workgroups of the factorisation"},
    {"DBAT_HIP_GRID_OBS", true, "launch size of the observation-parallel kernels"},
};

inline const char *env_get(const char *name) {
    for (const EnvSwitch &e : kEnvSwitches)
        if (!strcmp(e.name, name)) return (e.measurement && !kProfilingBuild) ? nullptr : getenv(name);
    return nullptr;
}
inline int env_int(const char *name, int dflt) { const char *e = env_get(name); return e ? atoi(e) : dflt; }
inline bool env_on(const char *name) { return env_get(name) != nullptr; }

inline bool env_validate(std::string &err) {
    for (char **p = environ; p && *p; ++p) {
        if (strncmp(*p, "DBAT_HIP_", 9) != 0) continue;
        const char *eq = strchr(*p, '=');
        const std::string name(*p, eq ? (size_t)(eq - *p) : strlen(*p));
        const EnvSwitch *hit = nullptr;
        for (const EnvSwitch &e : kEnvSwitches) if (name == e.name) hit = &e;
        if (!hit) { err = "unknown environment variable " + name + " (the switches of libdbat_hip.so: csrc/env.hpp, DESIGN.md 9)"; return false; }
        if (hit->measurement && !kProfilingBuild) {
            err = name + " is a measurement switch (" + hit->what + "): this library was built without -DDBAT_HIP_PROFILING (make -C dbat_amd/csrc prof)";
            return false;
        }
        if (hit->values && eq) {
            const std::string val(eq + 1), list = std::string("|") + hit->values + "|";
            if (val.empty() || val.find('|') != std::string::npos || list.find("|" + val + "|") == std::string::npos) {
                err = name + "=" + val + ": not one of " + hit->values + " (" + hit->what + ")";
                return false;
            }
        }
    }
    return true;
}

}
```

### dbat_amd/csrc/kernels.hpp

```cpp
#pragma once
#include <hip/hip_runtime.h>

#include "model.hpp"

namespace dbat {

struct DevProblem {
    int nc, np, nIOrows, nK, nP, nIOu, ncolmax, BT;
    int64_t NS, NZ, nobs, nb;
    int64_t ldS;
    const int32_t *cam_ncol, *cam_col, *cam_iorow;
    const uint32_t *cam_eo_est;
    const int32_t *io_src;
    const double *io_fixed;
    const double *px;
    const double *cam_w;
    const uint8_t *z_est, *z_mine;
    const double *z_prw, *z_prv;
    const int32_t *o_cam, *o_pt;
    const double *o_uv;
    const double *o_uv_raw;
    int uv_pre;
    const double *o_w;
    const uint32_t *o_seg;
    const int64_t *o_row;
    const int64_t *batch_start;
    int CMAX, ntiles;
    int ablate;
    int trace_only;
    int deterministic;
    int any_prior;
    double *det_cam_part;
    double *det_io_part;
    double *det_rr;
    double *det_u;
    const int32_t *det_cam_chunks;
    const uint8_t *o_lc, *o_pidx;
    const int32_t *tile_batch, *tile_cam_start, *tile_cams;
    const int32_t *tile_order;
    const int32_t *tile_io_start, *tile_iocols;
    const uint8_t *tile_io_simple;
    const uint8_t *tile_cam_io;
    int ngiant;
    const int64_t *giant_start;
    double *giant_W;
};

#ifdef DBAT_HIP_PROFILING
#define DBAT_ABLATE(d, bits) (((d).ablate & (bits)) != 0)
#else
#define DBAT_ABLATE(d, bits) (0)
#endif

__device__ __forceinline__ void atomic_add_f64(double *p, double v) {
    unsafeAtomicAdd(p, v);
}

constexpr int DET_CP = 256;
constexpr int DET_IOP = 128;
__device__ __forceinline__ double det_round(double v, double ui, double uj) {
    const double M = 3.0 * ui * uj;
    double t = v + M;
    asm volatile("" : "+v"(t));
    return t - M;
}
__device__ __forceinline__ double det_pow2_sqrt(double a) {
    if (!(a > 0.0)) return 0.0;
    int e;
    const double m = frexp(a, &e);
    (void)m;
    return ldexp(1.0, (e + 1) >> 1);
}

template <class ZV>
__device__ __forceinline__ void cam_prep_one(const DevProblem &d, ZV zv, int c, CamRec *__restrict__ cams) {
    CamRec &r = cams[c];
    const int32_t *ec = d.cam_col + (int64_t)c * MAXCOL;
    r.c[0] = zv(ec[0]); r.c[1] = zv(ec[1]); r.c[2] = zv(ec[2]);
    const double ang[3] = {zv(ec[3]), zv(ec[4]), zv(ec[5])};
    double Mt[9], sk, ck;
    cam_rotation(ang, Mt, sk, ck);
#pragma unroll
    for (int k = 0; k < 9; ++k) r.Mt[k] = Mt[k];
    r.sk = sk; r.ck = ck;
    auto io_at = [&](int k) -> double {
        if (k >= d.nIOrows) return 0.0;
        const int32_t s = d.io_src[(int64_t)c * d.nIOrows + k];
        return s >= 0 ? zv(6 * (int64_t)d.nc + s) : d.io_fixed[(int64_t)c * d.nIOrows + k];
    };
    r.f = io_at(0); r.pp[0] = io_at(1); r.pp[1] = io_at(2); r.b[0] = io_at(3); r.b[1] = io_at(4);
#pragma unroll
    for (int k = 0; k < MAXK; ++k) r.K[k] = k < d.nK ? io_at(5 + k) : 0.0;
#pragma unroll
    for (int k = 0; k < MAXP; ++k) r.P[k] = k < d.nP ? io_at(5 + d.nK + k) : 0.0;
    r.sz = d.px[2 * c];
    r.w[0] = d.cam_w[2 * c]; r.w[1] = d.cam_w[2 * c + 1];
    const int ncol = d.cam_ncol[c];
    r.ncol = ncol;
#pragma unroll
    for (int k = 0; k < MAXCOL; ++k) r.col[k] = ec[k];
    constexpr int std8[8] = {0, 1, 2, 5, 6, 7, 8, 9};
    bool is8 = ncol == 14 && d.nK == 3 && d.nP == 2;
#pragma unroll
    for (int k = 0; k < MAXIO; ++k) {
        const int32_t row = d.cam_iorow[(int64_t)c * MAXIO + k];
        r.iorow[k] = row;
        if (k < 8) is8 = is8 && row == std8[k];
    }
    r.eo_est = d.cam_eo_est[c] | (is8 ? 0x100u : 0u);
}
__global__ void k_cam_prep(DevProblem d, const double *__restrict__ z, CamRec *__restrict__ cams) {
    const int c = blockIdx.x * blockDim.x + threadIdx.x;
    if (c < d.nc) cam_prep_one(d, [z](int64_t i) { return z[i]; }, c, cams);
}

template <int MODEL>
__global__ __launch_bounds__(256) void k_uv_to_rhs(int nK, int nP, const CamRec *__restrict__ cams, int64_t n,
                                                   const int32_t *__restrict__ cam, const double *__restrict__ uv,
                                                   double *__restrict__ rhs) {
    const int64_t o = (int64_t)blockIdx.x * blockDim.x + threadIdx.x;
    if (o >= n) return;
    ImgSide im;
    image_side<MODEL, false>(cams[cam[o]], nK, nP, uv[2 * o], uv[2 * o + 1], im);
    rhs[2 * o] = im.rhs[0]; rhs[2 * o + 1] = im.rhs[1];
}
template <int MODEL>
__global__ __launch_bounds__(256) void k_uv_to_rhs_cm(int nK, int nP, const CamRec *__restrict__ cams,
                                                      const int32_t *__restrict__ chunk_cam,
                                                      const int64_t *__restrict__ chunk_start, double *__restrict__ cm_uv) {
    const CamRec &C = cams[chunk_cam[blockIdx.x]];
    for (int64_t q = chunk_start[blockIdx.x] + threadIdx.x; q < chunk_start[blockIdx.x + 1]; q += 256) {
        ImgSide im;
        image_side<MODEL, false>(C, nK, nP, cm_uv[2 * q], cm_uv[2 * q + 1], im);
        cm_uv[2 * q] = im.rhs[0]; cm_uv[2 * q + 1] = im.rhs[1];
    }
}
template <int MODEL>
__global__ __launch_bounds__(64) void k_uv_to_rhs_sig(int nK, int nP, const CamRec *__restrict__ cams,
                                                      const int32_t *__restrict__ sg_chunk,
                                                      const int32_t *__restrict__ sg_gcam, double *__restrict__ sg_uv) {
    const int32_t *cd = sg_chunk + 8 * (int64_t)blockIdx.x;
    const int npts = cd[1], k = cd[2], gm = cd[4], gi0 = cd[5], uv0 = cd[6];
    for (int j = 0; j < k; ++j) {
        const CamRec &C = cams[sg_gcam[16 * (int64_t)blockIdx.x + j]];
        for (int i = threadIdx.x; i < npts; i += 64) {
            const int64_t q = uv0 + (int64_t)j * gm + gi0 + i;
            ImgSide im;
            image_side<MODEL, false>(C, nK, nP, sg_uv[2 * q], sg_uv[2 * q + 1], im);
            sg_uv[2 * q] = im.rhs[0]; sg_uv[2 * q + 1] = im.rhs[1];
        }
    }
}

template <int NV>
__device__ __forceinline__ void block_sum(double (&v)[NV], double *sh ) {
    const int lane = threadIdx.x & 63, wave = threadIdx.x >> 6, nw = (blockDim.x + 63) >> 6;
#pragma unroll
    for (int i = 0; i < NV; ++i) {
        double x = v[i];
        for (int off = 32; off > 0; off >>= 1) x += __shfl_down(x, off, 64);
        if (lane == 0) sh[i * nw + wave] = x;
    }
    __syncthreads();
    if (threadIdx.x == 0) {
#pragma unroll
        for (int i = 0; i < NV; ++i) {
            double s = 0;
            for (int w = 0; w < nw; ++w) s += sh[i * nw + w];
            v[i] = s;
        }
    }
    __syncthreads();
}

template <int NV, int NX = 0, int XO = 0>
__device__ __forceinline__ bool grid_sum(double (&v)[NV], double *sh , double *__restrict__ partial,
                                         unsigned *__restrict__ ctr, const double *__restrict__ extra = nullptr,
                                         int64_t n_extra = 0, int extra_stride = 1) {
    __shared__ int s_last;
    block_sum<NV>(v, sh);
    if (threadIdx.x == 0) {
#pragma unroll
        for (int i = 0; i < NV; ++i)
            __hip_atomic_store(partial + (int64_t)NV * blockIdx.x + i, v[i], __ATOMIC_RELAXED, __HIP_MEMORY_SCOPE_AGENT);
        __builtin_amdgcn_s_waitcnt(0);
        s_last = __hip_atomic_fetch_add(ctr, 1u, __ATOMIC_RELAXED, __HIP_MEMORY_SCOPE_AGENT) == gridDim.x - 1;
    }
    __syncthreads();
    if (!s_last) return false;
    double acc[NV];
#pragma unroll
    for (int i = 0; i < NV; ++i) acc[i] = 0.0;
    for (int64_t b = threadIdx.x; b < gridDim.x; b += blockDim.x)
#pragma unroll
        for (int i = 0; i < NV; ++i)
            acc[i] += __hip_atomic_load(partial + NV * b + i, __ATOMIC_RELAXED, __HIP_MEMORY_SCOPE_AGENT);
    if constexpr (NX > 0) {
        for (int64_t b = threadIdx.x; b < n_extra; b += blockDim.x)
#pragma unroll
            for (int i = 0; i < NX; ++i) acc[XO + i] += extra[extra_stride * b + i];
    }
    __syncthreads();
    block_sum<NV>(acc, sh);
    if (threadIdx.x == 0) {
#pragma unroll
        for (int i = 0; i < NV; ++i) v[i] = acc[i];
        __hip_atomic_store(ctr, 0u, __ATOMIC_RELAXED, __HIP_MEMORY_SCOPE_AGENT);
    }
    return true;
}

template <int MODEL, bool PRE>
__global__ __launch_bounds__(256) void k_residual(DevProblem d, const double *__restrict__ z,
                                                  const CamRec *__restrict__ cams,
                                                  double *__restrict__ partial,
                                                  double *__restrict__ r_w, double *__restrict__ r_unw) {
    __shared__ double sh[8];
    double acc[1] = {0.0};
    const int64_t stride = (int64_t)gridDim.x * blockDim.x;
    for (int64_t o = (int64_t)blockIdx.x * blockDim.x + threadIdx.x; o < d.nobs; o += stride) {
        const int cam = d.o_cam[o], pt = d.o_pt[o];
        const CamRec &C = cams[cam];
        const double *q = z + d.NS + 3 * (int64_t)pt;
        const double Q[3] = {q[0], q[1], q[2]};
        double r[2];
        double(*nil6)[6] = nullptr; double(*nil3)[3] = nullptr; double(*nilc)[MAXIO] = nullptr;
        obs_eval<MODEL, false, false, PRE>(C, d.nK, d.nP, Q, d.o_uv[2 * o], d.o_uv[2 * o + 1], r, nil6, nil3, nilc);
        if (r_unw) { const int64_t row = d.o_row[o]; r_unw[2 * row] = r[0]; r_unw[2 * row + 1] = r[1]; }
        const double w0 = d.o_w ? d.o_w[2 * o] : C.w[0], w1 = d.o_w ? d.o_w[2 * o + 1] : C.w[1];
        r[0] *= w0; r[1] *= w1;
        if (r_w) { r_w[2 * o] = r[0]; r_w[2 * o + 1] = r[1]; }
        acc[0] = fma2(acc[0], r[0], r[0], r[1], r[1]);
    }
    block_sum<1>(acc, sh);
    if (threadIdx.x == 0) partial[blockIdx.x] = acc[0];
}

__device__ __forceinline__ void mailbox_done(double *mailbox, unsigned long long seq);

template <int MODEL, bool PRE>
__global__ __launch_bounds__(256) void k_residual_cm(DevProblem d, const double *__restrict__ z,
                                                     const CamRec *__restrict__ cams,
                                                     const int32_t *__restrict__ cm_pt,
                                                     const double *__restrict__ cm_uv, const double *__restrict__ cm_w,
                                                     const int32_t *__restrict__ chunk_cam,
                                                     const int64_t *__restrict__ chunk_start,
                                                     double *__restrict__ partial, unsigned *__restrict__ tail_ctr = nullptr,
                                                     double *__restrict__ out = nullptr, double *__restrict__ mailbox = nullptr,
                                                     unsigned long long seq = 0) {
    __shared__ double sh[8];
    __shared__ int s_last;
    const CamRec &C = cams[chunk_cam[blockIdx.x]];
    const int64_t q0 = chunk_start[blockIdx.x], q1 = chunk_start[blockIdx.x + 1];
    double acc[1] = {0.0};
    const double2 *uvp = reinterpret_cast<const double2 *>(cm_uv), *wp = reinterpret_cast<const double2 *>(cm_w);
    for (int64_t qb = q0 + threadIdx.x; qb < q1; qb += 4 * 256) {
        int pt[4]; double2 uv[4], ww[4]; double Q[4][3];
#pragma unroll
        for (int u = 0; u < 4; ++u) {
            const int64_t q = qb + 256 * u;
            const bool on = q < q1;
            pt[u] = on ? cm_pt[q] : -1;
            uv[u] = on ? uvp[q] : double2{0, 0};
            ww[u] = (on && cm_w) ? wp[q] : double2{C.w[0], C.w[1]};
        }
#pragma unroll
        for (int u = 0; u < 4; ++u) {
            const double *p = z + d.NS + 3 * (int64_t)(pt[u] < 0 ? 0 : pt[u]);
            Q[u][0] = p[0]; Q[u][1] = p[1]; Q[u][2] = p[2];
        }
#pragma unroll
        for (int u = 0; u < 4; ++u) {
            double r[2];
            double(*nil6)[6] = nullptr; double(*nil3)[3] = nullptr; double(*nilc)[MAXIO] = nullptr;
            obs_eval<MODEL, false, false, PRE>(C, d.nK, d.nP, Q[u], uv[u].x, uv[u].y, r, nil6, nil3, nilc);
            r[0] *= ww[u].x; r[1] *= ww[u].y;
            if (pt[u] >= 0) acc[0] += r[0] * r[0] + r[1] * r[1];
        }
    }
    block_sum<1>(acc, sh);
    if (!tail_ctr) {
        if (threadIdx.x == 0) partial[blockIdx.x] = acc[0];
        return;
    }
    if (threadIdx.x == 0) {
        __hip_atomic_store(partial + blockIdx.x, acc[0], __ATOMIC_RELAXED, __HIP_MEMORY_SCOPE_AGENT);
        __builtin_amdgcn_s_waitcnt(0);
        s_last = __hip_atomic_fetch_add(tail_ctr, 1u, __ATOMIC_RELAXED, __HIP_MEMORY_SCOPE_AGENT) == gridDim.x - 1;
    }
    __syncthreads();
    if (!s_last) return;
    double tot[1] = {0.0};
    for (unsigned b = threadIdx.x; b < gridDim.x; b += blockDim.x)
        tot[0] += __hip_atomic_load(partial + b, __ATOMIC_RELAXED, __HIP_MEMORY_SCOPE_AGENT);
    __syncthreads();
    block_sum<1>(tot, sh);
    if (threadIdx.x == 0) {
        out[0] = tot[0];
        __hip_atomic_store(tail_ctr, 0u, __ATOMIC_RELAXED, __HIP_MEMORY_SCOPE_AGENT);
        if (mailbox) { mailbox[0] = tot[0]; mailbox_done(mailbox, seq); }
    }
}

__device__ __forceinline__ void mailbox_done(double *mailbox, unsigned long long seq) {
    __atomic_store_n(reinterpret_cast<unsigned long long *>(mailbox) + 63, seq, __ATOMIC_RELEASE);
}

__global__ __launch_bounds__(1024) void k_prior_sq(DevProblem d, const double *__restrict__ z,
                                                   double *__restrict__ partial, unsigned *__restrict__ ctr,
                                                   const double *__restrict__ res_partial, int64_t n_res,
                                                   double *__restrict__ out, double *__restrict__ mailbox,
                                                   unsigned long long seq) {
    __shared__ double sh[16];
    double acc[1] = {0.0};
    const int64_t stride = (int64_t)gridDim.x * blockDim.x;
    if (d.any_prior)
        for (int64_t i = (int64_t)blockIdx.x * blockDim.x + threadIdx.x; i < d.NZ; i += stride) {
            const double w = d.z_prw[i];
            if (w > 0 && d.z_mine[i]) { const double e = z[i] - d.z_prv[i]; acc[0] += w * e * e; }
        }
    if (grid_sum<1, 1>(acc, sh, partial, ctr, res_partial, n_res) && threadIdx.x == 0) {
        out[0] = acc[0];
        if (mailbox) { mailbox[0] = acc[0]; mailbox_done(mailbox, seq); }
    }
}

template <int MODEL, int NCX>
__device__ __forceinline__ void eval_obs_pre(const DevProblem &d, const CamRec &C, const double Q[3], double u,
                                             double v, double w0, double w1, unsigned est, double r[2],
                                             double E[2][NCX], double B[2][3]);

template <int MODEL, int NCX>
__global__ __launch_bounds__(256) void k_trace_cm(DevProblem d, const double *__restrict__ z,
                                                  const CamRec *__restrict__ cams,
                                                  const int32_t *__restrict__ cm_pt,
                                                  const double *__restrict__ cm_uv, const double *__restrict__ cm_w,
                                                  const int32_t *__restrict__ chunk_cam,
                                                  const int64_t *__restrict__ chunk_start,
                                                  double *__restrict__ partial) {
    __shared__ double sh[8];
    const CamRec &C = cams[chunk_cam[blockIdx.x]];
    const int64_t q0 = chunk_start[blockIdx.x], q1 = chunk_start[blockIdx.x + 1];
    const int ncol = NCX > 6 ? min(C.ncol, NCX) : 6;
    double acc[1] = {0.0};
    for (int64_t q = q0 + threadIdx.x; q < q1; q += 256) {
        const int64_t zp = d.NS + 3 * (int64_t)cm_pt[q];
        const double Q[3] = {z[zp], z[zp + 1], z[zp + 2]};
        const unsigned est = (d.z_est[zp] ? 1u : 0u) | (d.z_est[zp + 1] ? 2u : 0u) | (d.z_est[zp + 2] ? 4u : 0u);
        const double w0 = cm_w ? cm_w[2 * q] : C.w[0], w1 = cm_w ? cm_w[2 * q + 1] : C.w[1];
        double r[2], E[2][NCX], B[2][3];
        eval_obs_pre<MODEL, NCX>(d, C, Q, cm_uv[2 * q], cm_uv[2 * q + 1], w0, w1, est, r, E, B);
        double s = 0.0;
#pragma unroll
        for (int a = 0; a < NCX; ++a) if (a < ncol) s += E[0][a] * E[0][a] + E[1][a] * E[1][a];
#pragma unroll
        for (int c = 0; c < 3; ++c) s += B[0][c] * B[0][c] + B[1][c] * B[1][c];
        acc[0] += s;
    }
    block_sum<1>(acc, sh);
    if (threadIdx.x == 0) partial[blockIdx.x] = acc[0];
}
__global__ __launch_bounds__(1024) void k_trace_tail(DevProblem d, double *__restrict__ partial, unsigned *__restrict__ ctr,
// ... 471 lines not shown
        pmin = fmin(pmin, __shfl_down(pmin, off, 64));
        pmax = fmax(pmax, __shfl_down(pmax, off, 64));
    }
    if ((t & 63) == 0 && pmax > 0.0) {
        atomicMin(pivmm, (unsigned long long)__double_as_longlong(pmin));
        atomicMax(pivmm + 1, (unsigned long long)__double_as_longlong(pmax));
    }
}

template <int MODEL, bool WITH_IO>
__global__ __launch_bounds__(256) void k_build_giant(DevProblem d, const double *__restrict__ z,
                                                     const CamRec *__restrict__ cams, double lambda, int scale,
                                                     double *__restrict__ S, double *__restrict__ g_c,
                                                     double *__restrict__ g_red, double *__restrict__ diagU,
                                                     double *__restrict__ Vinv, double *__restrict__ gp,
                                                     double *__restrict__ jn2p,
                                                     double *__restrict__ partial,
                                                     unsigned long long *__restrict__ pivmm) {
    constexpr int NCX = WITH_IO ? MAXCOL : 6;
    __shared__ double sh[9 * 4];
    __shared__ double pin[9];
    const int t = threadIdx.x, BT = blockDim.x;
    const int64_t o0 = d.giant_start[blockIdx.x], o1 = d.giant_start[blockIdx.x + 1];
    const int k = (int)(o1 - o0);
    const int strideW = d.ncolmax * 3;
    double *Wg = d.giant_W + (o0 - d.giant_start[0]) * strideW;
    const int pt = d.o_pt[o0];
    double acc[9] = {0, 0, 0, 0, 0, 0, 0, 0, 0}, rr = 0.0;
    for (int i = t; i < k; i += BT) {
        const int64_t o = o0 + i;
        const CamRec &C = cams[d.o_cam[o]];
        const int ncol = WITH_IO ? C.ncol : 6;
        double r[2], E[2][NCX], B[2][3];
        eval_obs_cols<MODEL, WITH_IO>(d, C, z, o, pt, r, E, B);
        rr = fma2(rr, r[0], r[0], r[1], r[1]);
        acc[0] = fma2(acc[0], B[0][0], B[0][0], B[1][0], B[1][0]);
        acc[1] = fma2(acc[1], B[0][0], B[0][1], B[1][0], B[1][1]);
        acc[2] = fma2(acc[2], B[0][0], B[0][2], B[1][0], B[1][2]);
        acc[3] = fma2(acc[3], B[0][1], B[0][1], B[1][1], B[1][1]);
        acc[4] = fma2(acc[4], B[0][1], B[0][2], B[1][1], B[1][2]);
        acc[5] = fma2(acc[5], B[0][2], B[0][2], B[1][2], B[1][2]);
        acc[6] = fma2(acc[6], B[0][0], r[0], B[1][0], r[1]);
        acc[7] = fma2(acc[7], B[0][1], r[0], B[1][1], r[1]);
        acc[8] = fma2(acc[8], B[0][2], r[0], B[1][2], r[1]);
        double *wl = Wg + (size_t)i * strideW;
        for (int a = 0; a < NCX; ++a) {
            if (a >= ncol) break;
            double ea0 = 0, ea1 = 0;
#pragma unroll
            for (int q = 0; q < NCX; ++q) if (q == a) { ea0 = E[0][q]; ea1 = E[1][q]; }
            wl[3 * a] = ea0 * B[0][0] + ea1 * B[1][0];
            wl[3 * a + 1] = ea0 * B[0][1] + ea1 * B[1][1];
            wl[3 * a + 2] = ea0 * B[0][2] + ea1 * B[1][2];
            if (d.deterministic) continue;
            const int gcol = C.col[a];
            const double ga = ea0 * r[0] + ea1 * r[1];
            atomic_add_f64(g_c + gcol, ga);
            atomic_add_f64(g_red + gcol, ga);
            atomic_add_f64(diagU + gcol, ea0 * ea0 + ea1 * ea1);
            for (int b = 0; b < ncol; ++b) {
                const int grow = C.col[b];
                if (grow < gcol) continue;
                double eb0 = 0, eb1 = 0;
#pragma unroll
                for (int q = 0; q < NCX; ++q) if (q == b) { eb0 = E[0][q]; eb1 = E[1][q]; }
                atomic_add_f64(S + (int64_t)gcol * d.ldS + grow, ea0 * eb0 + ea1 * eb1);
            }
        }
    }
    block_sum<9>(acc, sh);
    double pmin = 1e300, pmax = 0.0;
    if (t == 0) {
        double V[6] = {acc[0], acc[1], acc[2], acc[3], acc[4], acc[5]}, g[3] = {acc[6], acc[7], acc[8]};
        const int64_t zp = d.NS + 3 * (int64_t)pt;
        const int dix[3] = {0, 3, 5};
        double jn[3];
        for (int q = 0; q < 3; ++q) {
            const double pw = d.z_prw[zp + q];
            if (pw > 0) { V[dix[q]] += pw; g[q] += pw * (z[zp + q] - d.z_prv[zp + q]); }
            jn[q] = V[dix[q]];
            jn2p[3 * (int64_t)pt + q] = jn[q];
            if (d.z_est[zp + q]) V[dix[q]] += lambda; else V[dix[q]] = 1.0;
        }
        double inv[6], Rpb[6];
        point_block_factor(V, Rpb, inv);
        const double d0 = sqrt(V[0]), l10 = V[1] / d0, l20 = V[2] / d0;
        const double d1 = sqrt(V[3] - l10 * l10), l21 = (V[4] - l20 * l10) / d1;
        const double d2 = sqrt(V[5] - l20 * l20 - l21 * l21);
        const double dd[3] = {d0, d1, d2};
        for (int q = 0; q < 3; ++q)
            if (d.z_est[zp + q]) {
                double v = scale ? dd[q] / sqrt(jn[q]) : dd[q];
                v = v == v ? v : 0.0;
                pmin = fmin(pmin, v); pmax = fmax(pmax, v);
            }
        for (int q = 0; q < 6; ++q) { pin[q] = Rpb[q]; Vinv[6 * (int64_t)pt + q] = Rpb[q]; }
        for (int q = 0; q < 3; ++q) gp[3 * (int64_t)pt + q] = g[q];
        pin[6] = Rpb[0] * g[0] + Rpb[1] * g[1] + Rpb[2] * g[2];
        pin[7] = Rpb[3] * g[1] + Rpb[4] * g[2];
        pin[8] = Rpb[5] * g[2];
        if (pmax > 0.0) {
            atomicMin(pivmm, (unsigned long long)__double_as_longlong(pmin));
            atomicMax(pivmm + 1, (unsigned long long)__double_as_longlong(pmax));
        }
    }
    __threadfence_block();
    __syncthreads();
    const double v0 = pin[0], v1 = pin[1], v2 = pin[2], v3 = pin[3], v4 = pin[4], v5 = pin[5];
    const double g0 = pin[6], g1 = pin[7], g2 = pin[8];
    for (int i = t; i < k; i += BT) {
        const int nci = WITH_IO ? cams[d.o_cam[o0 + i]].ncol : 6;
        double *wi = Wg + (size_t)i * strideW;
        for (int a = 0; a < nci; ++a) {
            const double w0 = wi[3 * a], w1 = wi[3 * a + 1], w2 = wi[3 * a + 2];
            wi[3 * a] = w0 * v0 + w1 * v1 + w2 * v2; wi[3 * a + 1] = w1 * v3 + w2 * v4; wi[3 * a + 2] = w2 * v5;
        }
    }
    __threadfence_block();
    __syncthreads();
    for (int i = t; i < k; i += BT) {
        const CamRec &Ci = cams[d.o_cam[o0 + i]];
        const int nci = WITH_IO ? Ci.ncol : 6;
        const double *wi = Wg + (size_t)i * strideW;
        for (int a = 0; a < nci; ++a) {
            const int gcol = Ci.col[a];
            const double y0 = wi[3 * a], y1 = wi[3 * a + 1], y2 = wi[3 * a + 2];
            const bool det = d.deterministic != 0;
            const double gy = -(y0 * g0 + y1 * g1 + y2 * g2);
            atomic_add_f64(g_red + gcol, det ? det_round(gy, d.det_u[gcol], d.det_u[d.NS]) : gy);
            for (int j = WITH_IO ? 0 : i; j < k; ++j) {
                const CamRec &Cj = cams[d.o_cam[o0 + j]];
                const int ncj = WITH_IO ? Cj.ncol : 6;
                const double *wj = Wg + (size_t)j * strideW;
                for (int b = 0; b < ncj; ++b) {
                    const int grow = Cj.col[b];
                    if (grow < gcol) continue;
                    if (!WITH_IO && j == i && b < a) continue;
                    const double pz = -(y0 * wj[3 * b] + y1 * wj[3 * b + 1] + y2 * wj[3 * b + 2]);
                    atomic_add_f64(S + (int64_t)gcol * d.ldS + grow, det ? det_round(pz, d.det_u[gcol], d.det_u[grow]) : pz);
                }
            }
        }
    }
    double accr[1] = {rr};
    block_sum<1>(accr, sh);
    if (t == 0) partial[blockIdx.x] = accr[0];
}

template <int MODEL, bool WITH_IO>
__global__ __launch_bounds__(256) void k_backsub_giant(DevProblem d, const double *__restrict__ z,
                                                       const CamRec *__restrict__ cams,
                                                       const double *__restrict__ Vinv, const double *__restrict__ gp,
                                                 double *__restrict__ dz,
                                                       double *__restrict__ partial ) {
    constexpr int NCX = WITH_IO ? MAXCOL : 6;
    __shared__ double sh[3 * 4];
    __shared__ double dps[3];
    const int t = threadIdx.x, BT = blockDim.x;
    const int64_t o0 = d.giant_start[blockIdx.x], o1 = d.giant_start[blockIdx.x + 1];
    const int k = (int)(o1 - o0);
    const int pt = d.o_pt[o0];
    double s[3] = {0, 0, 0};
    for (int i = t; i < k; i += BT) {
        const int64_t o = o0 + i;
        const CamRec &C = cams[d.o_cam[o]];
        const int ncol = WITH_IO ? C.ncol : 6;
        double r[2], E[2][NCX], B[2][3], tt[2] = {0, 0};
        eval_obs_cols<MODEL, WITH_IO>(d, C, z, o, pt, r, E, B);
#pragma unroll
        for (int a = 0; a < NCX; ++a)
            if (a < ncol) { const double dc = dz[C.col[a]]; tt[0] += E[0][a] * dc; tt[1] += E[1][a] * dc; }
        s[0] = fma2(s[0], B[0][0], tt[0], B[1][0], tt[1]);
        s[1] = fma2(s[1], B[0][1], tt[0], B[1][1], tt[1]);
        s[2] = fma2(s[2], B[0][2], tt[0], B[1][2], tt[1]);
    }
    block_sum<3>(s, sh);
    if (t == 0) {
        for (int q = 0; q < 3; ++q) s[q] += gp[3 * (int64_t)pt + q];
        double p0, p1, p2;
        point_block_solve_neg(Vinv + 6 * (int64_t)pt, s[0], s[1], s[2], p0, p1, p2);
        const int64_t zp = d.NS + 3 * (int64_t)pt;
        dps[0] = d.z_est[zp] ? p0 : 0.0; dps[1] = d.z_est[zp + 1] ? p1 : 0.0; dps[2] = d.z_est[zp + 2] ? p2 : 0.0;
        dz[zp] = dps[0]; dz[zp + 1] = dps[1]; dz[zp + 2] = dps[2];
    }
    __syncthreads();
    double acc[2] = {0, 0};
    for (int i = t; i < k; i += BT) {
        const int64_t o = o0 + i;
        const CamRec &C = cams[d.o_cam[o]];
        const int ncol = WITH_IO ? C.ncol : 6;
        double r[2], E[2][NCX], B[2][3], tt[2] = {0, 0};
        eval_obs_cols<MODEL, WITH_IO>(d, C, z, o, pt, r, E, B);
#pragma unroll
        for (int a = 0; a < NCX; ++a)
            if (a < ncol) { const double dc = dz[C.col[a]]; tt[0] += E[0][a] * dc; tt[1] += E[1][a] * dc; }
        const double j0 = tt[0] + B[0][0] * dps[0] + B[0][1] * dps[1] + B[0][2] * dps[2];
        const double j1 = tt[1] + B[1][0] * dps[0] + B[1][1] * dps[1] + B[1][2] * dps[2];
        acc[0] = fma2(acc[0], j0, j0, j1, j1);
    }
    block_sum<2>(acc, sh);
    if (t == 0) { partial[2 * blockIdx.x] = acc[0]; partial[2 * blockIdx.x + 1] = acc[1]; }
}

typedef double mfma_d4 __attribute__((ext_vector_type(4)));
constexpr int TILE_LD = 144;

__device__ __forceinline__ void lds_fence() {
    __builtin_amdgcn_s_waitcnt(0xc07f);
    asm volatile("" ::: "memory");
}

template <int MODEL, int NCX>
__global__ __launch_bounds__(256, 3) void k_cam_normal(DevProblem d, const double *__restrict__ z,
                                                       const CamRec *__restrict__ cams,
                                                       const int32_t *__restrict__ cm_pt, const double *__restrict__ cm_uv,
                                                       const double *__restrict__ cm_w,
                                                       const int32_t *__restrict__ chunk_cam,
                                                       const int64_t *__restrict__ chunk_start, double *__restrict__ S,
                                                       double *__restrict__ g_c, double *__restrict__ g_red,
                                                       double *__restrict__ diagU) {
    constexpr bool IO = NCX > 6;
    constexpr int GLD = 66;
    __shared__ double Gl[4 * 16 * GLD];
    const int t = threadIdx.x, lane = t & 63, w = t >> 6;
    const int cam = chunk_cam[blockIdx.x];
    const int64_t q0 = chunk_start[blockIdx.x], q1 = chunk_start[blockIdx.x + 1];
    const CamRec &C = cams[cam];
    const int ncol = IO ? min(C.ncol, NCX) : 6;
    double *Gw = Gl + w * 16 * GLD;
    for (int c = NCX + 1; c < 16; ++c) Gw[c * GLD + lane] = 0.0;
    mfma_d4 acc = {0, 0, 0, 0};
    {
        auto load_obs = [&](int64_t q, int &pt, double2 &uv, double2 &ww) {
            pt = 0; uv = double2{0, 0}; ww = double2{C.w[0], C.w[1]};
            if (q < q1) {
                pt = cm_pt[q];
                uv = reinterpret_cast<const double2 *>(cm_uv)[q];
                if (cm_w) ww = reinterpret_cast<const double2 *>(cm_w)[q];
            }
        };
        const int64_t qw = q0 + 64 * w + lane;
        int pt_a, pt_b;
        double2 uv_a, uv_b, w_a, w_b;
        load_obs(qw, pt_a, uv_a, w_a);
        load_obs(qw + 256, pt_b, uv_b, w_b);
        double Qn[3];
        { const int64_t zp = d.NS + 3 * (int64_t)pt_a; Qn[0] = z[zp]; Qn[1] = z[zp + 1]; Qn[2] = z[zp + 2]; }
        const int prow = lane & 31;
        const double *ga = Gw + (lane & 15) * GLD + (lane >> 4);
        for (int64_t base = q0 + 64 * w; base < q1; base += 256) {
            const int64_t q = base + lane;
            const double Q[3] = {Qn[0], Qn[1], Qn[2]};
            const double2 uv = uv_a, ww = w_a;
            pt_a = pt_b; uv_a = uv_b; w_a = w_b;
            { const int64_t zp = d.NS + 3 * (int64_t)pt_a; Qn[0] = z[zp]; Qn[1] = z[zp + 1]; Qn[2] = z[zp + 2]; }
            load_obs(q + 512, pt_b, uv_b, w_b);
            double r[2] = {0, 0}, E[2][NCX];
#pragma unroll
            for (int c = 0; c < NCX; ++c) { E[0][c] = 0.0; E[1][c] = 0.0; }
            if (q < q1) {
                double B[2][3];
                eval_obs_pre<MODEL, NCX>(d, C, Q, uv.x, uv.y, ww.x, ww.y, 7u, r, E, B);
            }
#pragma unroll
            for (int half = 0; half < 2; ++half) {
                if ((lane >> 5) == half) {
                    if (ncol == NCX) {
#pragma unroll
                        for (int c = 0; c < NCX; ++c) { Gw[c * GLD + prow] = E[0][c]; Gw[c * GLD + 32 + prow] = E[1][c]; }
                    } else {
#pragma unroll
                        for (int c = 0; c < NCX; ++c) {
                            const bool on = c < ncol;
                            Gw[c * GLD + prow] = on ? E[0][c] : 0.0;
                            Gw[c * GLD + 32 + prow] = on ? E[1][c] : 0.0;
                        }
                    }
                    Gw[NCX * GLD + prow] = r[0]; Gw[NCX * GLD + 32 + prow] = r[1];
                }
                lds_fence();
                if (base + 32 * half < q1) {
                    double av[16];
#pragma unroll
                    for (int kk = 0; kk < 16; ++kk) av[kk] = ga[4 * kk];
#pragma unroll
                    for (int kk = 0; kk < 16; ++kk) acc = __builtin_amdgcn_mfma_f64_16x16x4f64(av[kk], av[kk], acc, 0, 0, 0);
                }
                lds_fence();
            }
        }
    }
    double *Gs = Gl;
    __syncthreads();
#pragma unroll
    for (int e = 0; e < 4; ++e) Gs[w * 256 + ((lane >> 4) + 4 * e) * 16 + (lane & 15)] = acc[e];
    __syncthreads();
    const int i = t >> 4, j = t & 15;
    const double g = (Gs[t] + Gs[256 + t]) + (Gs[512 + t] + Gs[768 + t]);
    if (d.deterministic) { d.det_cam_part[(int64_t)blockIdx.x * DET_CP + t] = g; return; }
    if (i < ncol && g != 0.0) {
        const int64_t ri = C.col[i];
        if (j < ncol) {
            const int64_t rj = C.col[j];
            if (i > j) atomic_add_f64(S + (ri >= rj ? rj * d.ldS + ri : ri * d.ldS + rj), g);
            else if (i == j) { atomic_add_f64(S + ri * d.ldS + ri, g); atomic_add_f64(diagU + ri, g); }
        } else if (j == NCX) {
            atomic_add_f64(g_c + ri, g);
            atomic_add_f64(g_red + ri, g);
        }
    }
}

template <int MODEL>
__global__ __launch_bounds__(256) void k_cam_normal6(DevProblem d, const double *__restrict__ z,
                                                     const CamRec *__restrict__ cams,
                                                     const int32_t *__restrict__ cm_pt, const double *__restrict__ cm_uv,
                                                     const double *__restrict__ cm_w,
                                                     const int32_t *__restrict__ chunk_cam,
                                                     const int64_t *__restrict__ chunk_start, double *__restrict__ S,
                                                     double *__restrict__ g_c, double *__restrict__ g_red,
                                                     double *__restrict__ diagU) {
    __shared__ double Gs[4 * 28];
    __shared__ double Rd[4][14 * 65];
    const int t = threadIdx.x, lane = t & 63, w = t >> 6;
    const int cam = chunk_cam[blockIdx.x];
    const int64_t q0 = chunk_start[blockIdx.x], q1 = chunk_start[blockIdx.x + 1];
    const CamRec &C = cams[cam];
    double G[28];
#pragma unroll
    for (int i = 0; i < 28; ++i) G[i] = 0.0;
    const double2 *uvp = reinterpret_cast<const double2 *>(cm_uv), *wp = reinterpret_cast<const double2 *>(cm_w);
    for (int64_t qb = q0 + t; qb < q1; qb += 4 * 256) {
        int pt[4]; double2 uv[4], ww[4]; double Qv[4][3];
#pragma unroll
        for (int u = 0; u < 4; ++u) {
            const int64_t q = qb + 256 * u;
            const bool on = q < q1;
            pt[u] = on ? cm_pt[q] : -1;
            uv[u] = on ? uvp[q] : double2{0, 0};
            ww[u] = (on && cm_w) ? wp[q] : double2{C.w[0], C.w[1]};
        }
#pragma unroll
        for (int u = 0; u < 4; ++u) {
            const double *p = z + d.NS + 3 * (int64_t)(pt[u] < 0 ? 0 : pt[u]);
            Qv[u][0] = p[0]; Qv[u][1] = p[1]; Qv[u][2] = p[2];
        }
#pragma unroll
        for (int u = 0; u < 4; ++u) {
            if (pt[u] < 0) continue;
            const double d0 = Qv[u][0] - C.c[0], d1 = Qv[u][1] - C.c[1], d2 = Qv[u][2] - C.c[2];
            const double X0 = C.Mt[0] * d0 + C.Mt[1] * d1 + C.Mt[2] * d2;
            const double X1 = C.Mt[3] * d0 + C.Mt[4] * d1 + C.Mt[5] * d2;
            const double X2 = C.Mt[6] * d0 + C.Mt[7] * d1 + C.Mt[8] * d2;
            const double iz = recip(X2);
// ... 1202 lines not shown
            g[0] = h00; g[1] = h01; g[2] = h11;
#pragma unroll
            for (int q = 0; q < 3; ++q) { g[3 + q] = B[0][q]; g[6 + q] = B[1][q]; }
        }
    }
    block_sum<6>(c6, sh);
    if (t == 0) {
#pragma unroll
        for (int q = 0; q < 6; ++q) c6[q] += vi[q];
        const int64_t zp = d.NS + 3 * (int64_t)pt;
        const bool e0 = d.z_est[zp], e1 = d.z_est[zp + 1], e2 = d.z_est[zp + 2];
        if constexpr (HAT) {
#pragma unroll
            for (int q = 0; q < 6; ++q) cpp[q] = c6[q];
            hat.dCz[zp] = e0 ? c6[0] : 0.0; hat.dCz[zp + 1] = e1 ? c6[3] : 0.0; hat.dCz[zp + 2] = e2 ? c6[5] : 0.0;
        } else {
            double *out = COP + 9 * (int64_t)pt;
            out[0] = e0 ? s02 * c6[0] : 0.0;
            out[1] = out[3] = (e0 && e1) ? s02 * c6[1] : 0.0;
            out[2] = out[6] = (e0 && e2) ? s02 * c6[2] : 0.0;
            out[4] = e1 ? s02 * c6[3] : 0.0;
            out[5] = out[7] = (e1 && e2) ? s02 * c6[4] : 0.0;
            out[8] = e2 ? s02 * c6[5] : 0.0;
        }
    }
    if constexpr (HAT) {
        __syncthreads();
        for (int i = t; i < k; i += BT) {
            const double *g = hat.gscr + (o0 + i - d.giant_start[0]) * 9;
            const double B[2][3] = {{g[3], g[4], g[5]}, {g[6], g[7], g[8]}};
            hat_finish(cpp, B, g[0], g[1], g[2], hat.qvv + 3 * d.o_row[o0 + i]);
        }
    }
}

__global__ __launch_bounds__(256) void k_pack_envelope(double *__restrict__ S, int64_t ldS, int NS, int tail0,
                                                       const int *__restrict__ col_bend,
                                                       const int64_t *__restrict__ col_off,
                                                       double *__restrict__ buf, int to_packed) {
    const int c = blockIdx.x;
    const int be = col_bend[c];
    const int nband = be - c;
    const int t0 = max(tail0, be);
    const int ntot = nband + (NS - t0);
    double *col = S + (int64_t)c * ldS;
    double *pk = buf + col_off[c];
    for (int i = threadIdx.x; i < ntot; i += 256) {
        const int r = i < nband ? c + i : t0 + (i - nband);
        if (to_packed) pk[i] = col[r]; else col[r] = pk[i];
    }
}

__device__ __forceinline__ void envelope_body(double *__restrict__ S, int64_t ldS, int NS, int tail0,
                                              const int *__restrict__ col_bend, const double *__restrict__ ds,
                                              double *__restrict__ vec, unsigned long long *__restrict__ pivmm) {
    const int c = blockIdx.x;
    if (vec && threadIdx.x < 3) vec[(int64_t)threadIdx.x * NS + c] = 0.0;
    if (c == 0 && vec && threadIdx.x >= 64 && threadIdx.x < 72) vec[(int64_t)3 * NS + (threadIdx.x - 64)] = 0.0;
    if (c == 0 && pivmm && threadIdx.x >= 128 && threadIdx.x < 132)
        pivmm[threadIdx.x - 128] = (threadIdx.x & 1) ? 0ull : (unsigned long long)__double_as_longlong(1e300);
    const int be = col_bend[c];
    const int nband = be - c;
    const int t0 = max(tail0, be);
    const int ntot = nband + (NS - t0);
    double *col = S + (int64_t)c * ldS;
    const double dc = ds ? ds[c] : 0.0;
    for (int i = threadIdx.x; i < ntot; i += 256) {
        const int r = i < nband ? c + i : t0 + (i - nband);
        col[r] = ds ? col[r] * dc * ds[r] : 0.0;
    }
}
__global__ __launch_bounds__(256) void k_envelope_op(double *__restrict__ S, int64_t ldS, int NS, int tail0,
                                                     const int *__restrict__ col_bend,
                                                     const double *__restrict__ ds ,
                                                     double *__restrict__ vec = nullptr ,
                                                     unsigned long long *__restrict__ pivmm = nullptr ) {
    envelope_body(S, ldS, NS, tail0, col_bend, ds, vec, pivmm);
}
__global__ __launch_bounds__(256) void k_envelope_cams(DevProblem d, const double *__restrict__ z, CamRec *__restrict__ cams,
                                                       double *__restrict__ S, int64_t ldS, int NS, int tail0,
                                                       const int *__restrict__ col_bend, double *__restrict__ vec,
                                                       unsigned long long *__restrict__ pivmm) {
    if (threadIdx.x == 255 && (int)blockIdx.x < d.nc) cam_prep_one(d, [z](int64_t i) { return z[i]; }, (int)blockIdx.x, cams);
    envelope_body(S, ldS, NS, tail0, col_bend, nullptr, vec, pivmm);
}

__global__ void k_finish(DevProblem d, const double *__restrict__ z, double lambda, int scale,
                         double *__restrict__ S, double *__restrict__ g_c, double *__restrict__ g_red,
                         const double *__restrict__ diagU, double *__restrict__ jn2c,
                         double *__restrict__ dscale, double *__restrict__ partial, unsigned *__restrict__ ctr,
                         const double *__restrict__ red_scal, double *__restrict__ out,
                         double *__restrict__ mailbox, const uint8_t *__restrict__ mine = nullptr,
                         int *__restrict__ df_info = nullptr, int *__restrict__ df_ctl = nullptr,
                         unsigned long long *__restrict__ df_q = nullptr, int df_nq = 0) {
    if (df_ctl) {
        const int64_t g = (int64_t)blockIdx.x * blockDim.x + threadIdx.x;
        if (g == 0) { *df_info = 0; for (int q = 0; q < 8; ++q) df_ctl[q] = 0; }
        for (int64_t j = g; j < df_nq; j += (int64_t)gridDim.x * blockDim.x) df_q[j] = 0xFFFFFFFFFFFFFFFFull;
    }
    __shared__ double sh[8];
    const int64_t i = (int64_t)blockIdx.x * blockDim.x + threadIdx.x;
    double acc[1] = {0.0};
    if (i < d.NS) {
        const bool own = !mine || mine[i];
        const double pw = d.z_prw[i];
        double add = 0, g = g_red[i], jn2 = diagU[i];
        if (pw > 0) {
            const double e = pw * (z[i] - d.z_prv[i]);
            jn2 += pw;
            if (own) { g_c[i] += e; add += pw; g += e; g_red[i] = g; }
        }
        jn2c[i] = jn2;
        const bool est = d.z_est[i] != 0;
        double ds = 1.0;
        if (est) {
            if (own) add += lambda;
            if (scale && jn2 > 0) ds = 1.0 / sqrt(jn2);
            S[i * d.ldS + i] += add;
            S[i * d.ldS + d.NS] = -ds * g;
            acc[0] = jn2;
        } else {
            S[i * d.ldS + i] = own ? 1.0 : 0.0;
            S[i * d.ldS + d.NS] = 0.0;
        }
        dscale[i] = ds;
    }
    if (grid_sum<1>(acc, sh, partial, ctr) && threadIdx.x == 0) {
        out[0] = acc[0];
        if (mailbox) { mailbox[34] = acc[0]; mailbox[32] = red_scal[0]; mailbox[33] = red_scal[1]; }
    }
}

__global__ void k_mask_owned(int64_t n, const uint8_t *__restrict__ mine, const double *__restrict__ in,
                             double *__restrict__ out) {
    const int64_t i = (int64_t)blockIdx.x * blockDim.x + threadIdx.x;
    if (i < n) out[i] = mine[i] ? in[i] : 0.0;
}

__global__ void k_weight_rows(DevProblem d, const double *__restrict__ r_unw, double *__restrict__ r_wgt) {
    const int64_t k = (int64_t)blockIdx.x * blockDim.x + threadIdx.x;
    if (k >= d.nobs) return;
    const int64_t row = d.o_row[k];
    const int cam = d.o_cam[k];
    const double w0 = d.o_w ? d.o_w[2 * k] : d.cam_w[2 * cam], w1 = d.o_w ? d.o_w[2 * k + 1] : d.cam_w[2 * cam + 1];
    r_wgt[2 * row] = r_unw[2 * row] * w0;
    r_wgt[2 * row + 1] = r_unw[2 * row + 1] * w1;
}

template <int MODEL, int NCXT>
__global__ __launch_bounds__(256) void k_backsub(DevProblem d, const double *__restrict__ z,
                                                 const CamRec *__restrict__ cams,
                                                 const double *__restrict__ Vinv, const double *__restrict__ gp,
                                                 double *__restrict__ dz,
                                                 double *__restrict__ partial , int batch0) {
    constexpr int NCX = NCXT;
    constexpr bool WITH_IO = NCXT > 6;
    extern __shared__ double smem[];
    double *red = smem;
    double *dpl = red + (size_t)blockDim.x * 3;
    __shared__ double sh[16];
    const int t = threadIdx.x;
    const int batch = batch0 + blockIdx.x;
    const int64_t o0 = d.batch_start[batch];
    const int nobs = (int)(d.batch_start[batch + 1] - o0);
    const bool active = t < nobs;
    const int64_t o = o0 + t;
    double r[2] = {0, 0}, tt[2] = {0, 0};
    double E[2][NCX];
    double B[2][3] = {{0, 0, 0}, {0, 0, 0}};
    int pt = 0, seg_start = 0, seg_len = 0;
    if (active) {
        const int cam = d.o_cam[o]; pt = d.o_pt[o];
        const uint32_t sg = d.o_seg[o];
        seg_start = sg & 0xFFFF; seg_len = sg >> 16;
        const CamRec &C = cams[cam];
        const int ncol = WITH_IO ? min(C.ncol, NCX) : 6;
        eval_obs_cols_n<MODEL, NCX>(d, C, z, o, pt, r, E, B);
#pragma unroll
        for (int a = 0; a < NCX; ++a)
            if (a < ncol) { const double dc = dz[C.col[a]]; tt[0] += E[0][a] * dc; tt[1] += E[1][a] * dc; }
        red[3 * t] = B[0][0] * tt[0] + B[1][0] * tt[1];
        red[3 * t + 1] = B[0][1] * tt[0] + B[1][1] * tt[1];
        red[3 * t + 2] = B[0][2] * tt[0] + B[1][2] * tt[1];
    }
    __syncthreads();
    if (active && t == seg_start) {
        double s[3] = {gp[3 * (int64_t)pt], gp[3 * (int64_t)pt + 1], gp[3 * (int64_t)pt + 2]};
        for (int j = 0; j < seg_len; ++j) { s[0] += red[3 * (t + j)]; s[1] += red[3 * (t + j) + 1]; s[2] += red[3 * (t + j) + 2]; }
        double p0, p1, p2;
        point_block_solve_neg(Vinv + 6 * (int64_t)pt, s[0], s[1], s[2], p0, p1, p2);
        const int64_t zp = d.NS + 3 * (int64_t)pt;
        const double q0 = d.z_est[zp] ? p0 : 0.0, q1 = d.z_est[zp + 1] ? p1 : 0.0, q2 = d.z_est[zp + 2] ? p2 : 0.0;
        dz[zp] = q0; dz[zp + 1] = q1; dz[zp + 2] = q2;
        dpl[3 * t] = q0; dpl[3 * t + 1] = q1; dpl[3 * t + 2] = q2;
    }
    __syncthreads();
    double acc[2] = {0, 0};
    if (active) {
        const double *dp = dpl + 3 * seg_start;
        const double j0 = tt[0] + B[0][0] * dp[0] + B[0][1] * dp[1] + B[0][2] * dp[2];
        const double j1 = tt[1] + B[1][0] * dp[0] + B[1][1] * dp[1] + B[1][2] * dp[2];
        acc[0] = j0 * j0 + j1 * j1;
    }
    block_sum<2>(acc, sh);
    if (t == 0) { partial[2 * (int64_t)batch] = acc[0]; partial[2 * (int64_t)batch + 1] = acc[1]; }
}

__device__ __forceinline__ void fwd_ray_terms(const CamRec &C, int nK, int nP, double u, double v, double out[9]) {
    const double qx = C.sz * u, qy = -C.sz * v;
    const double xb = qx - C.pp[0], yb = qy - C.pp[1];
    const double r2 = xb * xb + yb * yb;
    double Kr = 0, pw = 1;
    for (int j = 0; j < MAXK; ++j) if (j < nK) { pw *= r2; Kr += C.K[j] * pw; }
    double dx = xb * Kr, dy = yb * Kr;
    if (nP >= 2) {
        const double P1 = C.P[0], P2 = C.P[1], P3 = nP > 2 ? 1.0 + C.P[2] : 1.0;
        dx += (P1 * (r2 + 2 * xb * xb) + 2 * P2 * xb * yb) * P3;
        dy += (P2 * (r2 + 2 * yb * yb) + 2 * P1 * xb * yb) * P3;
    }
    const double dc[3] = {qx - dx - C.pp[0], qy - dy - C.pp[1], -C.f};
    double dw[3];
#pragma unroll
    for (int i = 0; i < 3; ++i) dw[i] = C.Mt[i] * dc[0] + C.Mt[3 + i] * dc[1] + C.Mt[6 + i] * dc[2];
    const double inn = 1.0 / sqrt(dw[0] * dw[0] + dw[1] * dw[1] + dw[2] * dw[2]);
    const double d0 = dw[0] * inn, d1 = dw[1] * inn, d2 = dw[2] * inn;
    const double p00 = 1 - d0 * d0, p01 = -d0 * d1, p02 = -d0 * d2, p11 = 1 - d1 * d1, p12 = -d1 * d2, p22 = 1 - d2 * d2;
    out[0] = p00; out[1] = p01; out[2] = p02; out[3] = p11; out[4] = p12; out[5] = p22;
    out[6] = p00 * C.c[0] + p01 * C.c[1] + p02 * C.c[2];
    out[7] = p01 * C.c[0] + p11 * C.c[1] + p12 * C.c[2];
    out[8] = p02 * C.c[0] + p12 * C.c[1] + p22 * C.c[2];
}
__device__ __forceinline__ void fwd_solve(const double a[9], int rays, double *op) {
    const double nan = __longlong_as_double(0x7ff8000000000000ll);
    double inv[6];
    if (rays < 2) { op[0] = op[1] = op[2] = nan; return; }
    inv3_sym(a, inv);
    op[0] = inv[0] * a[6] + inv[1] * a[7] + inv[2] * a[8];
    op[1] = inv[1] * a[6] + inv[3] * a[7] + inv[4] * a[8];
    op[2] = inv[2] * a[6] + inv[4] * a[7] + inv[5] * a[8];
}
__global__ __launch_bounds__(256) void k_forwintersect(DevProblem d, const CamRec *__restrict__ cams,
                                                       double *__restrict__ OPout) {
    extern __shared__ double smem[];
    const int t = threadIdx.x;
    const int64_t o0 = d.batch_start[blockIdx.x];
    const int nobs = (int)(d.batch_start[blockIdx.x + 1] - o0);
    int pt = 0, seg_start = 0, seg_len = 0;
    if (t < nobs) {
        const int64_t o = o0 + t;
        pt = d.o_pt[o];
        const uint32_t sg = d.o_seg[o];
        seg_start = sg & 0xFFFF; seg_len = sg >> 16;
        fwd_ray_terms(cams[d.o_cam[o]], d.nK, d.nP, d.o_uv_raw[2 * o], d.o_uv_raw[2 * o + 1], smem + 9 * t);
    }
    __syncthreads();
    if (t < nobs && t == seg_start) {
        double a[9] = {0, 0, 0, 0, 0, 0, 0, 0, 0};
        for (int j = 0; j < seg_len; ++j)
#pragma unroll
            for (int q = 0; q < 9; ++q) a[q] += smem[9 * (t + j) + q];
        fwd_solve(a, seg_len, OPout + 3 * (int64_t)pt);
    }
}
__global__ __launch_bounds__(256) void k_forwintersect_giant(DevProblem d, const CamRec *__restrict__ cams,
                                                             double *__restrict__ OPout) {
    __shared__ double sh[9 * 4];
    const int t = threadIdx.x;
    const int64_t o0 = d.giant_start[blockIdx.x], o1 = d.giant_start[blockIdx.x + 1];
    double a[9] = {0, 0, 0, 0, 0, 0, 0, 0, 0};
    for (int64_t o = o0 + t; o < o1; o += blockDim.x) {
        double q[9];
        fwd_ray_terms(cams[d.o_cam[o]], d.nK, d.nP, d.o_uv_raw[2 * o], d.o_uv_raw[2 * o + 1], q);
#pragma unroll
        for (int i = 0; i < 9; ++i) a[i] += q[i];
    }
    block_sum<9>(a, sh);
    if (t == 0) fwd_solve(a, (int)(o1 - o0), OPout + 3 * (int64_t)d.o_pt[o0]);
}

template <int MODEL, int NCXT>
__global__ __launch_bounds__(256) void k_jtimes(DevProblem d, const double *__restrict__ z,
                                                const CamRec *__restrict__ cams, const double *__restrict__ v,
                                                double *__restrict__ partial) {
    constexpr int NCX = NCXT;
    constexpr bool WITH_IO = NCXT > 6;
    __shared__ double sh[16];
    double acc[2] = {0, 0};
    const int64_t stride = (int64_t)gridDim.x * blockDim.x;
    for (int64_t o = (int64_t)blockIdx.x * blockDim.x + threadIdx.x; o < d.nobs; o += stride) {
        const int cam = d.o_cam[o], pt = d.o_pt[o];
        const CamRec &C = cams[cam];
        const int ncol = WITH_IO ? min(C.ncol, NCX) : 6;
        double r[2], E[2][NCX], B[2][3];
        eval_obs_cols_n<MODEL, NCX>(d, C, z, o, pt, r, E, B);
        const double *vp = v + d.NS + 3 * (int64_t)pt;
        double j0 = B[0][0] * vp[0] + B[0][1] * vp[1] + B[0][2] * vp[2];
        double j1 = B[1][0] * vp[0] + B[1][1] * vp[1] + B[1][2] * vp[2];
#pragma unroll
        for (int a = 0; a < NCX; ++a)
            if (a < ncol) { const double vc = v[C.col[a]]; j0 += E[0][a] * vc; j1 += E[1][a] * vc; }
        acc[0] = fma2(acc[0], j0, j0, j1, j1);
    }
    block_sum<2>(acc, sh);
    if (threadIdx.x == 0) { partial[2 * blockIdx.x] = acc[0]; partial[2 * blockIdx.x + 1] = acc[1]; }
}

template <int MODEL, int NCXT>
__global__ __launch_bounds__(256) void k_jtimes_vec(DevProblem d, const double *__restrict__ z, const CamRec *__restrict__ cams,
                                                    const double *__restrict__ v, double *__restrict__ Jv) {
    constexpr int NCX = NCXT;
    constexpr bool WITH_IO = NCXT > 6;
    const int64_t o = (int64_t)blockIdx.x * blockDim.x + threadIdx.x;
    if (o >= d.nobs) return;
    const int cam = d.o_cam[o], pt = d.o_pt[o];
    const CamRec &C = cams[cam];
    const int ncol = WITH_IO ? min(C.ncol, NCX) : 6;
    double r[2], E[2][NCX], B[2][3];
    eval_obs_cols_n<MODEL, NCX>(d, C, z, o, pt, r, E, B);
    const double *vp = v + d.NS + 3 * (int64_t)pt;
    double j0 = B[0][0] * vp[0] + B[0][1] * vp[1] + B[0][2] * vp[2];
    double j1 = B[1][0] * vp[0] + B[1][1] * vp[1] + B[1][2] * vp[2];
#pragma unroll
    for (int a = 0; a < NCX; ++a)
        if (a < ncol) { const double vc = v[C.col[a]]; j0 += E[0][a] * vc; j1 += E[1][a] * vc; }
    const int64_t row = d.o_row[o];
    Jv[2 * row] = j0; Jv[2 * row + 1] = j1;
}

__global__ __launch_bounds__(1024) void k_prior_jv(DevProblem d, const double *__restrict__ z,
                                                  const double *__restrict__ v, const double *__restrict__ g_c,
                                                  const double *__restrict__ gp, double *__restrict__ partial,
                                                  unsigned *__restrict__ ctr, const double *__restrict__ bs_partial,
                                                  int64_t nbs, const double *__restrict__ ldiag,
                                                  unsigned long long *__restrict__ pivmm, const int *__restrict__ info,
                                                  double *__restrict__ out, double *__restrict__ mailbox,
                                                  unsigned long long seq, const uint8_t *__restrict__ piv_have = nullptr) {
    __shared__ double sh[80];
    double acc[5] = {0, 0, 0, 0, 0};
    const int64_t stride = (int64_t)gridDim.x * blockDim.x;
    double pmin = 1e300, pmax = 0.0;
    for (int64_t i = (int64_t)blockIdx.x * blockDim.x + threadIdx.x; i < d.NZ; i += stride) {
        if (ldiag && i < d.NS && d.z_est[i] && (!piv_have || piv_have[i])) {
            double p = ldiag[i];
            p = p == p ? p : 0.0;
            pmin = fmin(pmin, p); pmax = fmax(pmax, p);
        }
        if (!d.z_mine[i]) continue;
        const double w = d.any_prior ? d.z_prw[i] : 0.0, vi = d.z_est[i] ? v[i] : 0.0;
        if (w > 0) acc[0] += w * vi * vi;
        acc[1] += (i < d.NS ? g_c[i] : gp[i - d.NS]) * vi;
        acc[2] += vi * vi;
    }
    if (ldiag && (int64_t)blockIdx.x * blockDim.x < d.NS) {
        for (int off = 32; off > 0; off >>= 1) {
            pmin = fmin(pmin, __shfl_down(pmin, off, 64));
            pmax = fmax(pmax, __shfl_down(pmax, off, 64));
        }
        if ((threadIdx.x & 63) == 0 && pmax > 0.0) {
            atomicMin(pivmm + 2, (unsigned long long)__double_as_longlong(fmax(pmin, 0.0)));
            atomicMax(pivmm + 3, (unsigned long long)__double_as_longlong(pmax));
        }
        __builtin_amdgcn_s_waitcnt(0);
    }
    if (grid_sum<5, 2, 3>(acc, sh, partial, ctr, bs_partial, nbs, 2) && threadIdx.x == 0) {
        out[0] = acc[3]; out[1] = acc[4]; out[4] = acc[0]; out[5] = acc[1]; out[6] = acc[2];
        out[7] = info && __hip_atomic_load(info, __ATOMIC_RELAXED, __HIP_MEMORY_SCOPE_AGENT) != 0 ? 1.0 : 0.0;
        out[2] = 0.0; out[3] = 0.0;
        if (mailbox) {
            mailbox[0] = acc[3]; mailbox[1] = acc[4]; mailbox[4] = acc[0]; mailbox[5] = acc[1]; mailbox[6] = acc[2];
            for (int q = 0; q < 4; ++q)
                mailbox[40 + q] = __longlong_as_double((long long)__hip_atomic_load(pivmm + q, __ATOMIC_RELAXED, __HIP_MEMORY_SCOPE_AGENT));
            const int hi = __hip_atomic_load(info, __ATOMIC_RELAXED, __HIP_MEMORY_SCOPE_AGENT);
            long long w = hi;
            mailbox[44] = __longlong_as_double(w);
            mailbox_done(mailbox, seq);
        }
    }
}

__global__ __launch_bounds__(256) void k_dot(int64_t n, const uint8_t *__restrict__ mine,
                                             const double *__restrict__ a, const double *__restrict__ b ,
                                             double *__restrict__ partial) {
    __shared__ double sh[8];
    double acc[1] = {0};
    const int64_t stride = (int64_t)gridDim.x * blockDim.x;
    for (int64_t i = (int64_t)blockIdx.x * blockDim.x + threadIdx.x; i < n; i += stride)
        if (!mine || mine[i]) acc[0] += a[i] * (b ? b[i] : 1.0);
    block_sum<1>(acc, sh);
    if (threadIdx.x == 0) partial[blockIdx.x] = acc[0];
}

__global__ void k_axpby(int64_t n, double a, const double *__restrict__ x, double b,
                        const double *__restrict__ y2, double *__restrict__ y) {
    const int64_t i = (int64_t)blockIdx.x * blockDim.x + threadIdx.x;
    if (i < n) y[i] = a * x[i] + b * y2[i];
}
__global__ void k_axpby_cams(DevProblem d, double a, const double *__restrict__ x, double b,
                             const double *__restrict__ y2, double *__restrict__ y, CamRec *__restrict__ cams) {
    const int64_t i = (int64_t)blockIdx.x * blockDim.x + threadIdx.x;
    if (i < d.NZ) y[i] = a * x[i] + b * y2[i];
    if (threadIdx.x == blockDim.x - 1 && (int)blockIdx.x < d.nc)
        cam_prep_one(d, [=](int64_t q) { return a * x[q] + b * y2[q]; }, (int)blockIdx.x, cams);
}

__global__ void k_gradient(DevProblem d, const double *__restrict__ g_c, const double *__restrict__ gp,
                           double *__restrict__ g) {
    const int64_t i = (int64_t)blockIdx.x * blockDim.x + threadIdx.x;
    if (i >= d.NZ) return;
    double v = 0;
    if (d.z_est[i]) v = i < d.NS ? g_c[i] : (d.z_mine[i] ? gp[i - d.NS] : 0.0);
    g[i] = v;
}

__global__ void k_jn2(DevProblem d, const double *__restrict__ jn2c, const double *__restrict__ jn2p,
                      double *__restrict__ out) {
    const int64_t i = (int64_t)blockIdx.x * blockDim.x + threadIdx.x;
    if (i >= d.NZ) return;
    double v = 0;
    if (d.z_est[i]) v = i < d.NS ? jn2c[i] : (d.z_mine[i] ? jn2p[i - d.NS] : 0.0);
    out[i] = v;
}

__global__ void k_scatter_x(int64_t n, const int64_t *__restrict__ x2z, const double *__restrict__ x,
                            double *__restrict__ z) {
    const int64_t i = (int64_t)blockIdx.x * blockDim.x + threadIdx.x;
    if (i < n) z[x2z[i]] = x[i];
}
__global__ void k_gather_x(int64_t n, const int64_t *__restrict__ x2z, const double *__restrict__ z,
                           double *__restrict__ x) {
    const int64_t i = (int64_t)blockIdx.x * blockDim.x + threadIdx.x;
    if (i < n) x[i] = z[x2z[i]];
}

template <int MODEL>
__global__ __launch_bounds__(256) void k_jac_blocks(DevProblem d, const double *__restrict__ z,
                                                    const CamRec *__restrict__ cams,
                                                    double *__restrict__ JEO, double *__restrict__ JOP,
                                                    double *__restrict__ JIO) {
    const int64_t o = (int64_t)blockIdx.x * blockDim.x + threadIdx.x;
    if (o >= d.nobs) return;
    const int cam = d.o_cam[o], pt = d.o_pt[o];
    const CamRec &C = cams[cam];
    const double *q = z + d.NS + 3 * (int64_t)pt;
    const double Q[3] = {q[0], q[1], q[2]};
    double r[2], A[2][6], B[2][3], Cf[2][MAXIO];
    obs_eval<MODEL, true, true>(C, d.nK, d.nP, Q, d.o_uv_raw[2 * o], d.o_uv_raw[2 * o + 1], r, A, B, Cf);
    const int64_t k = d.o_row[o];
    if (JEO) for (int c = 0; c < 6; ++c) { JEO[12 * k + 2 * c] = A[0][c]; JEO[12 * k + 2 * c + 1] = A[1][c]; }
    if (JOP) for (int c = 0; c < 3; ++c) { JOP[6 * k + 2 * c] = B[0][c]; JOP[6 * k + 2 * c + 1] = B[1][c]; }
    if (JIO) for (int c = 0; c < d.nIOrows; ++c) {
        JIO[2 * (int64_t)d.nIOrows * k + 2 * c] = Cf[0][c];
        JIO[2 * (int64_t)d.nIOrows * k + 2 * c + 1] = Cf[1][c];
    }
}


template <int MODEL>
__global__ __launch_bounds__(256) void k_jac_sample(DevProblem d, const double *__restrict__ z,
                                                    const CamRec *__restrict__ cams, int64_t n,
                                                    const int64_t *__restrict__ pos, double *__restrict__ res,
                                                    double *__restrict__ JEO, double *__restrict__ JOP,
                                                    double *__restrict__ JIO) {
    const int64_t i = (int64_t)blockIdx.x * blockDim.x + threadIdx.x;
    if (i >= n) return;
    const int64_t o = pos[i];
    const CamRec &C = cams[d.o_cam[o]];
    const double *q = z + d.NS + 3 * (int64_t)d.o_pt[o];
    const double Q[3] = {q[0], q[1], q[2]};
    double r[2], A[2][6], B[2][3], Cf[2][MAXIO];
    obs_eval<MODEL, true, true>(C, d.nK, d.nP, Q, d.o_uv_raw[2 * o], d.o_uv_raw[2 * o + 1], r, A, B, Cf);
    res[2 * i] = r[0]; res[2 * i + 1] = r[1];
    for (int c = 0; c < 6; ++c) { JEO[12 * i + 2 * c] = A[0][c]; JEO[12 * i + 2 * c + 1] = A[1][c]; }
    for (int c = 0; c < 3; ++c) { JOP[6 * i + 2 * c] = B[0][c]; JOP[6 * i + 2 * c + 1] = B[1][c]; }
    for (int c = 0; c < d.nIOrows; ++c) {
        JIO[2 * (int64_t)d.nIOrows * i + 2 * c] = Cf[0][c];
        JIO[2 * (int64_t)d.nIOrows * i + 2 * c + 1] = Cf[1][c];
    }
}

}
```

### dbat_amd/csrc/sig.hpp

```cpp
#pragma once
#include <cstddef>
#include <type_traits>

#include "kernels.hpp"

namespace dbat {

constexpr int SIG_LDK = 18;
constexpr int SIG_PPR = 6;
constexpr int SIG_KMAXR = 13;
constexpr int SIG_NW = 8;
constexpr int SIG_CAMW = (int)(offsetof(CamRec, ncol) / 8) + 1;
constexpr int SIG_CAMW_IO = (int)((sizeof(CamRec) + 7) / 8);
constexpr int SIG_STILE = 8064;
#ifndef DBAT_SIG_IO_WAVES
#define DBAT_SIG_IO_WAVES 4
#endif
constexpr int SIG_IO_CAMS = DBAT_SIG_IO_WAVES == 8 ? 16 : 21;
__host__ __device__ constexpr int sig_stile(bool io) { return io && DBAT_SIG_IO_WAVES == 8 ? 6336 : SIG_STILE; }
__host__ __device__ constexpr int sig_cams(bool io) { return io ? SIG_IO_CAMS : 21; }

struct SigLds {
    int next_chunk, abort_;
    int flush_turn;
// ... 522 lines not shown
#pragma unroll
            for (int ks = 0; ks < 5; ++ks) {
                double (&cur)[RB] = (ks & 1) ? opb : opa;
                double (&nxt)[RB] = (ks & 1) ? opa : opb;
                if (ks + 1 < 5) load_ops(ks + 1, nxt);
                if (ks < ksteps) {
#pragma unroll
                    for (int r1 = 0; r1 < RB; ++r1)
                        if (r1 < rbk) {
#pragma unroll
                            for (int r2 = 0; r2 <= r1; ++r2)
                                acc[r1 * (r1 + 1) / 2 + r2] = __builtin_amdgcn_mfma_f64_16x16x4f64(
                                    cur[r1], cur[r2], acc[r1 * (r1 + 1) / 2 + r2], 0, 0, 0);
                        }
                }
            }
            lds_fence();
            __builtin_amdgcn_wave_barrier();
            lap(4);
        }
        if (d.deterministic) {
            volatile int *turn = &sy.flush_turn;
            int spins = 0;
            for (; *turn != ch_cur - ch0 && spins < (1 << 24); ++spins) __builtin_amdgcn_s_sleep(1);
            if (spins >= (1 << 24) && lane == 0) atomicAdd(det_timeouts, 1u);
        }
        {
            const int r6k = ry;
            int tcm[RB];
#pragma unroll
            for (int r2 = 0; r2 < RB; ++r2) tcm[r2] = sy.tmap[wave][min(16 * r2 + (lane & 15), 79)];
#pragma unroll
            for (int r1 = 0; r1 < RB; ++r1) {
                if (r1 >= rbk) break;
#pragma unroll
                for (int e = 0; e < 4; ++e) {
                    const int lr = 16 * r1 + (lane >> 4) + 4 * e;
                    const bool yrow = lr == r6k;
                    double *row = stile + (yrow ? STILE : sy.toff[wave][min(lr, 79)]);
                    if (!DBAT_ABLATE(d, 8)) {
#pragma unroll
                        for (int r2 = 0; r2 < r1; ++r2) {
                            const double v = acc[r1 * (r1 + 1) / 2 + r2][e];
                            atomic_add_f64(row + tcm[r2], yrow ? -v : v);
                        }
                        const double v = acc[r1 * (r1 + 1) / 2 + r1][e];
                        const int lcol = 16 * r1 + (lane & 15);
                        if (lcol <= lr && lcol < r6k && v != 0.0) atomic_add_f64(row + tcm[r1], yrow ? -v : v);
                    }
                }
            }
        }
        if (d.deterministic) {
            lds_fence();
            if (lane == 0) { volatile int *turn = &sy.flush_turn; *turn = ch_cur - ch0 + 1; }
        }
        __builtin_amdgcn_wave_barrier();
        lap(5);
    }
    lap(6);
    __syncthreads();
    lap(6);
    {
        constexpr int NCOLW = (128 + NW - 1) / NW;
        double v0[NCOLW], v1[NCOLW];
#pragma unroll
        for (int q = 0; q < NCOLW; ++q) {
            const int tc = wave + q * NW, tr = tc + lane;
            v0[q] = (tc < nrows && tr < nrows) ? stile[tr * (tr + 1) / 2 + tc] : 0.0;
            v1[q] = (tc < nrows && tr + 64 < nrows) ? stile[(tr + 64) * (tr + 65) / 2 + tc] : 0.0;
            if (d.deterministic && tc < nrows) {
                const double uc = sy.urow[tc];
                if (tr < nrows) v0[q] = det_round(v0[q], sy.urow[tr], uc);
                if (tr + 64 < nrows) v1[q] = det_round(v1[q], sy.urow[tr + 64], uc);
            }
        }
        if (!DBAT_ABLATE(d, 16)) {
#pragma unroll
            for (int q = 0; q < NCOLW; ++q) {
                const int tc = wave + q * NW, tr = tc + lane;
                if (tc < nrows) {
                    const int64_t gcol = sy.grow[tc] * d.ldS;
                    if (v0[q] != 0.0) atomic_add_f64(S + gcol + sy.grow[tr], -v0[q]);
                    if (v1[q] != 0.0) atomic_add_f64(S + gcol + sy.grow[tr + 64], -v1[q]);
                }
            }
        }
    }
    for (int i = t; i < nrows; i += NT) {
        const double v = d.deterministic ? det_round(vt[i], sy.urow[i], sy.uf) : vt[i];
        if (v != 0.0) atomic_add_f64(g_red + sy.grow[i], v);
    }
    double accr[1] = {rr};
    block_sum<1>(accr, sh);
    if (t == 0) partial[part_slot] = accr[0];
    pmin = pmin < 1e300 ? sqrt(pmin) : pmin; pmax = sqrt(pmax);
    for (int off = 32; off > 0; off >>= 1) {
        pmin = fmin(pmin, __shfl_down(pmin, off, 64));
        pmax = fmax(pmax, __shfl_down(pmax, off, 64));
    }
    if ((t & 63) == 0 && pmax > 0.0) {
        atomicMin(pivmm, (unsigned long long)__double_as_longlong(pmin));
        atomicMax(pivmm + 1, (unsigned long long)__double_as_longlong(pmax));
    }
    lap(7);
    if (prof)
        for (int i = 0; i < 8; ++i) if (tp[i]) atomicAdd(&g_tile2_prof[i], (unsigned long long)tp[i]);
}

template <int MODEL, int RB, int NCX, bool PW>
__global__ __launch_bounds__(64 * sig_waves(RB, (NCX > 6))) void k_build_sig(DevProblem d, const double *__restrict__ z,
                                                   const CamRec *__restrict__ cams, double lambda, int scale,
                                                   double *__restrict__ S, double *__restrict__ g_red,
                                                   double *__restrict__ Vinv, double *__restrict__ gp,
                                                   double *__restrict__ jn2p,
                                                   double *__restrict__ partial, unsigned long long *__restrict__ pivmm,
                                                   const int32_t *__restrict__ sg_chunk,
                                                   const int32_t *__restrict__ sg_tile_chunk0,
                                                   const uint8_t *__restrict__ sg_lc, const double *__restrict__ sg_uv,
                                                   const double *__restrict__ sg_w, unsigned *__restrict__ tile_ctr) {
    __shared__ unsigned s_ticket;
    __shared__ SigLds sy;
    __shared__ double sh[16];
    for (;;) {
        if (threadIdx.x == 0) s_ticket = __hip_atomic_fetch_add(tile_ctr, 1u, __ATOMIC_RELAXED, __HIP_MEMORY_SCOPE_AGENT);
        __syncthreads();
        const unsigned ti = s_ticket;
        if (ti >= (unsigned)d.ntiles) {
            if (threadIdx.x == 0 && ti == (unsigned)d.ntiles + gridDim.x - 1)
                __hip_atomic_store(tile_ctr, 0u, __ATOMIC_RELAXED, __HIP_MEMORY_SCOPE_AGENT);
            return;
        }
        const int tile = d.tile_order[ti];
        int ios = 0;
        if constexpr (NCX > 6) ios = d.tile_io_simple ? d.tile_io_simple[tile] : 0;
#ifdef DBAT_SIG_ONLY_IOS
        ios = DBAT_SIG_ONLY_IOS;
#endif
        if (NCX > 6 && ios == 1)
            build_sig_tile<MODEL, RB, NCX, (NCX > 6 ? 1 : 0), PW>(d, tile, (int)ti, z, cams, lambda, scale, S, g_red, Vinv, gp, jn2p, partial, pivmm, sg_chunk, sg_tile_chunk0, sg_lc, sg_uv, sg_w, tile_ctr + 2, sy, sh);
        else if (NCX > 6 && ios == 2)
            build_sig_tile<MODEL, RB, NCX, (NCX > 6 ? 2 : 0), PW>(d, tile, (int)ti, z, cams, lambda, scale, S, g_red, Vinv, gp, jn2p, partial, pivmm, sg_chunk, sg_tile_chunk0, sg_lc, sg_uv, sg_w, tile_ctr + 2, sy, sh);
        else
            build_sig_tile<MODEL, RB, NCX, 0, PW>(d, tile, (int)ti, z, cams, lambda, scale, S, g_red, Vinv, gp, jn2p, partial, pivmm, sg_chunk, sg_tile_chunk0, sg_lc, sg_uv, sg_w, tile_ctr + 2, sy, sh);
        __syncthreads();
    }
}

template <int MODEL, int NCX>
__global__ __launch_bounds__(256) void k_backsub_sig(DevProblem d, const double *__restrict__ z,
                                                     const CamRec *__restrict__ cams,
                                                     const double *__restrict__ Vinv, const double *__restrict__ gp,
                                                     double *__restrict__ dz, double *__restrict__ partial ,
                                                     const int32_t *__restrict__ sg_chunk, int nchunks,
                                                     const int32_t *__restrict__ sg_gcam,
                                                     const double *__restrict__ sg_uv, const double *__restrict__ sg_w) {
    constexpr int CW = (int)((sizeof(CamRec) + 7) / 8);
    __shared__ double sh[8];
    __shared__ double crec[4][SIG_KMAXR][CW];
    __shared__ double dcs[4][SIG_KMAXR][NCX];
    const int t = threadIdx.x, lane = t & 63;
    const int wv = t >> 6;
    const int ch = __builtin_amdgcn_readfirstlane(blockIdx.x * 4 + (t >> 6));
    double acc[2] = {0, 0};
    if (ch < nchunks) {
        const int32_t *cd = sg_chunk + 8 * (int64_t)ch;
        const int pt0 = cd[0], npts = cd[1], k = cd[2], gm = cd[4], gi0 = cd[5], uv0 = cd[6];
        const int mycam = lane < k ? sg_gcam[16 * (int64_t)ch + lane] : 0;
        for (int base = 0; base < k * CW; base += 64) {
            const int idx = base + lane, c = min(idx / CW, k - 1), f = idx - c * CW;
            const int cam = __builtin_amdgcn_ds_bpermute(4 * c, mycam);
            if (idx < k * CW) crec[wv][c][f] = reinterpret_cast<const double *>(cams + cam)[f];
        }
        __builtin_amdgcn_wave_barrier();
        for (int idx = lane; idx < k * NCX; idx += 64) {
            const int c = idx / NCX, a = idx - c * NCX;
            const CamRec &C = *reinterpret_cast<const CamRec *>(crec[wv][c]);
            const bool on = a < (NCX > 6 ? min(C.ncol, NCX) : 6) && (NCX > 6 || ((C.eo_est >> a) & 1u));
            dcs[wv][c][a] = on ? dz[C.col[a]] : 0.0;
        }
        __builtin_amdgcn_wave_barrier();
        const int G = npts > 32 ? 64 : (npts > 16 ? 32 : (npts > 8 ? 16 : 8));
        const int pi = lane & (G - 1), jh = lane / G, jstep = 64 / G;
        const bool act = pi < npts;
        const int pt = pt0 + (act ? pi : 0);
        const int64_t zp = d.NS + 3 * (int64_t)pt;
        const double Q[3] = {z[zp], z[zp + 1], z[zp + 2]};
        const unsigned est = (d.z_est[zp] ? 1u : 0u) | (d.z_est[zp + 1] ? 2u : 0u) | (d.z_est[zp + 2] ? 4u : 0u);
        const double2 *uvp = reinterpret_cast<const double2 *>(sg_uv), *wp = reinterpret_cast<const double2 *>(sg_w);
        const int64_t q0 = uv0 + gi0 + (act ? pi : 0);
        double sB[3] = {0, 0, 0}, V0[6] = {0, 0, 0, 0, 0, 0}, tt2 = 0;
        auto sweep = [&](auto per_obs_w) {
        for (int j = jh; j < k; j += jstep) {
            const CamRec &C = *reinterpret_cast<const CamRec *>(crec[wv][j]);
            double2 uv = {0, 0};
            if constexpr (NCX > 6) uv = uvp[q0 + (int64_t)j * gm];
            double w0, w1;
            if constexpr (decltype(per_obs_w)::value) { const double2 ww = wp[q0 + (int64_t)j * gm]; w0 = ww.x; w1 = ww.y; }
            else { w0 = C.w[0]; w1 = C.w[1]; }
            double B[2][3], t0 = 0, t1 = 0;
            if constexpr (NCX > 6) {
                obs_step_dot<MODEL, true>(C, Q, uv.x, uv.y, w0, w1, est, dcs[wv][j], t0, t1, B);
            } else {
                sig_step_dot6(C, Q, w0, w1, dcs[wv][j], t0, t1, B);
            }
#define DBAT_ACC2(acc, a, b, c, e) acc = __builtin_fma(a, b, __builtin_fma(c, e, acc))
            DBAT_ACC2(tt2, t0, t0, t1, t1);
            DBAT_ACC2(sB[0], B[0][0], t0, B[1][0], t1);
            DBAT_ACC2(sB[1], B[0][1], t0, B[1][1], t1);
            DBAT_ACC2(sB[2], B[0][2], t0, B[1][2], t1);
            DBAT_ACC2(V0[0], B[0][0], B[0][0], B[1][0], B[1][0]);
            DBAT_ACC2(V0[1], B[0][0], B[0][1], B[1][0], B[1][1]);
            DBAT_ACC2(V0[2], B[0][0], B[0][2], B[1][0], B[1][2]);
            DBAT_ACC2(V0[3], B[0][1], B[0][1], B[1][1], B[1][1]);
            DBAT_ACC2(V0[4], B[0][1], B[0][2], B[1][1], B[1][2]);
            DBAT_ACC2(V0[5], B[0][2], B[0][2], B[1][2], B[1][2]);
#undef DBAT_ACC2
        }
        };
        if (sg_w) sweep(std::true_type{}); else sweep(std::false_type{});
        for (int m = G; m < 64; m <<= 1) {
#pragma unroll
            for (int c = 0; c < 3; ++c) sB[c] += lane_get(sB[c], lane ^ m);
#pragma unroll
            for (int c = 0; c < 6; ++c) V0[c] += lane_get(V0[c], lane ^ m);
            tt2 += lane_get(tt2, lane ^ m);
        }
        {
            const double s0 = gp[3 * (int64_t)pt] + sB[0], s1 = gp[3 * (int64_t)pt + 1] + sB[1], s2 = gp[3 * (int64_t)pt + 2] + sB[2];
            double p0, p1, p2;
            point_block_solve_neg(Vinv + 6 * (int64_t)pt, s0, s1, s2, p0, p1, p2);
            const double d0 = (est & 1u) ? p0 : 0.0, d1 = (est & 2u) ? p1 : 0.0, d2 = (est & 4u) ? p2 : 0.0;
            if (act && lane == pi) {
                dz[zp] = d0; dz[zp + 1] = d1; dz[zp + 2] = d2;
                acc[0] = tt2 + 2.0 * (d0 * sB[0] + d1 * sB[1] + d2 * sB[2])
                       + d0 * (V0[0] * d0 + V0[1] * d1 + V0[2] * d2) + d1 * (V0[1] * d0 + V0[3] * d1 + V0[4] * d2)
                       + d2 * (V0[2] * d0 + V0[4] * d1 + V0[5] * d2);
            }
        }
    }
    block_sum<2>(acc, sh);
    if (t == 0) { partial[2 * blockIdx.x] = acc[0]; partial[2 * blockIdx.x + 1] = acc[1]; }
}

}
```

Measured before the change: 634.4.

## Fuse trial-point update and point-side sums into back-substitution kernels

The back-substitution kernels now write the trial point zt = z + dz for each solved point and accumulate the point-side g'p, p'p and prior sums into widened per-block partials. Extra leading blocks update the camera entries and unvisited points and prepare the trial camera records. k_prior_jv then only covers the camera rows and folds in those partials, and eval_f_step skips its axpby/camera-prep launch when the fused results are still valid. This removes a full pass over the parameter vector and one launch per LM step, at the cost of validity-tracking state that could go stale and wider partial rows.

```diff
diff --git a/dbat_amd/csrc/dbat_core.hip b/dbat_amd/csrc/dbat_core.hip
--- a/dbat_amd/csrc/dbat_core.hip
+++ b/dbat_amd/csrc/dbat_core.hip
@@ -258,6 +258,8 @@
         d.o_seg = o_seg.p; d.o_row = o_row.p; d.batch_start = batch_start.p;
         d.CMAX = P.CMAX; d.ablate = env_int("DBAT_HIP_ABLATE", 0); d.trace_only = 0;
         d.any_prior = 0;
+        d.all_mine = 1;
+        for (uint8_t m : P.z_mine) if (!m) { d.all_mine = 0; break; }
         for (double w : P.z_prw) if (w > 0) { d.any_prior = 1; break; }
         d.deterministic = 0; d.det_cam_part = d.det_io_part = d.det_rr = d.det_u = nullptr; d.det_cam_chunks = nullptr;
         env_df_trace = env_get("DBAT_HIP_DF_TRACE");
@@ -372,11 +374,12 @@
         else if (use_tile2 && !P.with_io && tile_ncx == 6) route = TileRoute::tile3;
         else if (use_tile2 && (tile_ncx == 14 || tile_ncx == 15)) route = TileRoute::tile2;
         else throw DeviceError{"internal: tiles without a tile kernel"};
-        partial.alloc((size_t)4 * std::max<int64_t>(std::max<int64_t>(std::max<int64_t>(nb + ntiles + ngiant + (int64_t)P.sg_chunk.size() / 8, n_cm_chunks_all), 2048), 1));
+        partial.alloc((size_t)BS_NP * std::max<int64_t>(std::max<int64_t>(std::max<int64_t>(nb + ntiles + ngiant + (int64_t)P.sg_chunk.size() / 8, n_cm_chunks_all), 2048), 1));
         HIPCHK(hipMemcpy(z.p, P.z0.data(), P.NZ * 8, hipMemcpyHostToDevice));
         HIPCHK(hipMemset(dz.p, 0, P.NZ * 8));
         HIPCHK(hipMemset(zt.p, 0, P.NZ * 8));
         precompute_image_side();
+        list_unvisited_points();
         HIPCHK(hipDeviceSynchronize());
         lapi("work arrays, image side");
     }
@@ -412,6 +415,7 @@
             HIPCHK(hipStreamSynchronize(stream));
         }
         cams_at_lin = false; have_lin = false; s_valid = false; pend_build = false; lin_pending = false;
+        step_points_ready = false; z_at_lin = false;
         lambda_lin = 0; scale_lin = 0; f_lin = 0; trace_jtj = 0; near_singular = false; chol_in_place = false; replicate_next = false;
         n_res_evals = n_lin = n_solves = n_trace_only = 0;
     }
@@ -534,9 +538,11 @@
     }
     void prep_cams(const double *zz, CamRec *into = nullptr) {
         if (!into) { into = cams.p; cams_at_lin = false; }
+        else if (into == cams_f.p) step_points_ready = false;
         launch<k_cam_prep>(dim3((unsigned)cdiv(P.nc, 64)), dim3(64), 0, d, zz, into);
     }
     void x_to_z(const double *x_host, double *z_dev) {
+        touched(z_dev);
         HIPCHK(hipMemcpyAsync(z_dev, P.z0.data(), P.NZ * 8, hipMemcpyHostToDevice, stream));
         if (P.n) {
             HIPCHK(hipMemcpyAsync(xbuf.p, x_host, P.n * 8, hipMemcpyHostToDevice, stream));
@@ -592,6 +598,9 @@
 
     double eval_f_step(const double *x, double alpha, const double *pdir, double *out) {
         stage(3);
+        const bool ready = step_points_ready && z_at_lin && alpha == 1.0 && x == z.p && pdir == dz.p && out == zt.p;
+        step_points_ready = false;
+        if (ready) return eval_f(out, nullptr, nullptr, true);
         if ((int64_t)cdiv(P.NZ, 256) < P.nc) { axpby(1.0, x, alpha, pdir, out); return eval_f(out, nullptr, nullptr); }
         launch<k_axpby_cams>(dim3((unsigned)cdiv(P.NZ, 256)), dim3(256), 0, d, 1.0, x, alpha, pdir, out, cams_f.p);
         return eval_f(out, nullptr, nullptr, true);
@@ -794,6 +803,7 @@
         }
         launch<k_build_tail>(dim3(grid_zs), dim3(1024), 0, d, zz, partial.p, npart, jn2p.p, gpart.p, gctr.p + 2, red_scal,
                 zz != zlin.p ? zlin.p : (double *)nullptr);
+        if (zz != zlin.p) z_at_lin = zz == z.p;
     }
     bool pend_build = false;
     double pend_lambda = 0;
@@ -896,27 +906,56 @@
         const bool sig_bs = use_sig && P.sg_backsub_ok;
         const int64_t b_first = sig_bs ? P.nb_tiled : 0;
         const int64_t n_sig_wg = sig_bs ? cdiv(sg_nchunks, 4) : 0;
+        double *const zt_out = fuse_tails ? zt.p : (double *)nullptr;
+        bool cams_pending = fuse_tails;
+        auto step_cams = [&](int threads) {
+            StepCams sc{cams_f.p, (const int32_t *)pt_rest.p, n_pt_rest, 0};
+            if (cams_pending) sc.nxb = (int)cdiv(P.nc, (threads + 63) / 64);
+            cams_pending = false;
+            return sc;
+        };
         if (n_sig_wg > 0) {
+            const StepCams sc = step_cams(256);
             with_value<2, 3, 4, 5>(P.model, [&](auto M) { with_value<6, 14>(tile_ncx, [&](auto NCX) {
-                launch<k_backsub_sig<M, NCX>>(dim3((unsigned)n_sig_wg), dim3(256), 0, d, zlin.p, cams.p, Vinv.p, gp.p, dz.p, partial.p + 2 * (nb + ngiant), sg_chunk.p,
-                                              (int)sg_nchunks, sg_gcam.p, sg_uv.p, pw ? sg_w.p : (const double *)nullptr);
+                launch<k_backsub_sig<M, NCX>>(dim3((unsigned)(n_sig_wg + sc.nxb)), dim3(256), 0, d, zlin.p, cams.p, Vinv.p, gp.p, dz.p, partial.p + BS_NP * (nb + ngiant), zt_out,
+                                              sc, sg_chunk.p, (int)sg_nchunks, sg_gcam.p, sg_uv.p, pw ? sg_w.p : (const double *)nullptr);
             }); });
         }
         if (nb > b_first) {
+            const StepCams sc = step_cams(P.BT);
             with_value<2, 3, 4, 5>(P.model, [&](auto M) { with_value<6, 14, 15, MAXCOL>(tile_ncx, [&](auto NCX) {
-                launch<k_backsub<M, NCX>>(dim3((unsigned)(nb - b_first)), dim3(P.BT), lds_back, d, zlin.p, cams.p, Vinv.p, gp.p, dz.p, partial.p, (int)b_first);
+                launch<k_backsub<M, NCX>>(dim3((unsigned)(nb - b_first + sc.nxb)), dim3(P.BT), lds_back, d, zlin.p, cams.p, Vinv.p, gp.p, dz.p, partial.p, (int)b_first, zt_out, sc);
             }); });
         }
         if (ngiant > 0) {
+            const StepCams sc = step_cams(giant_threads);
             with_value<2, 3, 4, 5>(P.model, [&](auto M) { with_value<false, true>(P.with_io, [&](auto IO) {
-                launch<k_backsub_giant<M, IO>>(dim3((unsigned)ngiant), dim3(giant_threads), 0, d, zlin.p, cams.p, Vinv.p, gp.p, dz.p, partial.p + 2 * nb);
+                launch<k_backsub_giant<M, IO>>(dim3((unsigned)(ngiant + sc.nxb)), dim3(giant_threads), 0, d, zlin.p, cams.p, Vinv.p, gp.p, dz.p, partial.p + BS_NP * nb, zt_out, sc);
             }); });
         }
         mark(5);
-        launch<k_prior_jv>(dim3(grid_zs), dim3(1024), 0, d, zlin.p, dz.p, g_c, gp.p, gpart.p, gctr.p + 4,
-                (const double *)(partial.p + 2 * b_first), nb - b_first + ngiant + n_sig_wg, (const double *)ldiag.p, pivmm.p,
+        const int grid_jv = fuse_tails ? (int)std::max<int64_t>(1, std::min<int64_t>(cdiv(P.NS, 1024), grid_zs)) : grid_zs;
+        launch<k_prior_jv>(dim3(grid_jv), dim3(1024), 0, d, zlin.p, dz.p, g_c, gp.p, gpart.p, gctr.p + 4,
+                (const double *)(partial.p + BS_NP * b_first), nb - b_first + ngiant + n_sig_wg, (const double *)ldiag.p, pivmm.p,
                 (const int *)info.p, scal.p, multi() ? (double *)nullptr : hpin, ++mb_seq,
-                mg_subtree && multi() ? (const uint8_t *)piv_have.p : (const uint8_t *)nullptr);
+                mg_subtree && multi() ? (const uint8_t *)piv_have.p : (const uint8_t *)nullptr, fuse_tails ? 2 : 1);
+        step_points_ready = fuse_tails && !cams_pending;
+    }
+    const bool fuse_tails = env_int("DBAT_HIP_FUSE_TAILS", 1) != 0;
+    bool step_points_ready = false, z_at_lin = false;
+    void touched(const double *dst) {
+        if (dst == z.p) z_at_lin = false;
+        if (dst == z.p || dst == dz.p || dst == zt.p) step_points_ready = false;
+    }
+    DevBuf<int32_t> pt_rest;
+    int64_t n_pt_rest = 0;
+    void list_unvisited_points() {
+        std::vector<uint8_t> seen((size_t)P.np, 0);
+        for (int32_t p : P.o_pt) seen[(size_t)p] = 1;
+        std::vector<int32_t> rest;
+        for (int64_t p = 0; p < P.np; ++p) if (!seen[(size_t)p]) rest.push_back((int32_t)p);
+        n_pt_rest = (int64_t)rest.size();
+        if (n_pt_rest) pt_rest.upload(rest);
     }
     bool near_singular = false;
     const bool pivot_stats = env_on("DBAT_HIP_PIVOT_STATS");
@@ -1230,7 +1269,7 @@
             launch<k_jtimes<M, NCX>>(dim3(grid_obs), dim3(256), 0, d, zlin.p, cams.p, v, partial.p);
         }); });
         launch<k_prior_jv>(dim3(grid_zs), dim3(1024), 0, d, zlin.p, v, g_c, gp.p, gpart.p, gctr.p + 4,
-                (const double *)partial.p, (int64_t)grid_obs, (const double *)nullptr, pivmm.p, (const int *)info.p, scal.p, (double *)nullptr, 0ull, (const uint8_t *)nullptr);
+                (const double *)partial.p, (int64_t)grid_obs, (const double *)nullptr, pivmm.p, (const int *)info.p, scal.p, (double *)nullptr, 0ull, (const uint8_t *)nullptr, 0);
         do_allreduce(scal.p, 8);
         double h[8];
         read_scal(h, 8);
@@ -1245,6 +1284,7 @@
         return s;
     }
     void axpby(double a, const double *x, double b, const double *y2, double *y) {
+        touched(y);
         launch<k_axpby>(dim3((unsigned)cdiv(P.NZ, 256)), dim3(256), 0, P.NZ, a, x, b, y2, y);
     }
     void gradient(double *g) {
@@ -1256,8 +1296,8 @@
     void jac_blocks(const double *zz, double *a, double *b, double *cc) {
         with_value<2, 3, 4, 5>(P.model, [&](auto M) { launch<k_jac_blocks<M>>(dim3((unsigned)cdiv(nobs, 256)), dim3(256), 0, d, zz, cams.p, a, b, cc); });
     }
-    void copy(double *dst, const double *src) { HIPCHK(hipMemcpyAsync(dst, src, P.NZ * 8, hipMemcpyDeviceToDevice, stream)); }
-    void accept_trial() { std::swap(z.p, zt.p); }
+    void copy(double *dst, const double *src) { touched(dst); HIPCHK(hipMemcpyAsync(dst, src, P.NZ * 8, hipMemcpyDeviceToDevice, stream)); }
+    void accept_trial() { std::swap(z.p, zt.p); step_points_ready = false; z_at_lin = false; }
 };
 
 
diff --git a/dbat_amd/csrc/env.hpp b/dbat_amd/csrc/env.hpp
--- a/dbat_amd/csrc/env.hpp
+++ b/dbat_amd/csrc/env.hpp
@@ -33,6 +33,7 @@
     {"DBAT_HIP_DF_CHAIN", false, "factorisation: 0 = diagonal tiles as ordinary tasks (no chain role), 1 = chain role whatever the pattern", "0|1"},
     {"DBAT_HIP_DF_CHAIN_WG", false, "factorisation: workgroups of the chain role at most (default 32)"},
     {"DBAT_HIP_DF_L2", false, "factorisation: 1 = finished tiles of the compact layout are read through the L2", "0|1"},
+    {"DBAT_HIP_FUSE_TAILS", false, "0: the back-substitution leaves neither the trial point nor the point-side sums g'p, p'p (k_prior_jv and k_axpby_cams pass over the parameter vectors instead)", "0|1"},
     {"DBAT_HIP_COV_DENSE", false, "posterior covariance: the dense inverse of the reduced system (rocsolver_dpotri) instead of the selected inversion"},
     {"DBAT_HIP_SPRANK_OFF", false, "structural rank from the counting conditions only"},
     {"DBAT_HIP_PLAN_THREADS", false, "threads of the host plan (default: hardware concurrency, at most 32)"},
diff --git a/dbat_amd/csrc/kernels.hpp b/dbat_amd/csrc/kernels.hpp
--- a/dbat_amd/csrc/kernels.hpp
+++ b/dbat_amd/csrc/kernels.hpp
@@ -29,6 +29,7 @@
     int ablate;
     int trace_only;
     int deterministic;
+    int all_mine;
     int any_prior;
     double *det_cam_part;
     double *det_io_part;
@@ -208,6 +209,36 @@
         __hip_atomic_store(ctr, 0u, __ATOMIC_RELAXED, __HIP_MEMORY_SCOPE_AGENT);
     }
     return true;
+}
+
+constexpr int BS_NP = 5;
+struct StepCams { CamRec *cams_t; const int32_t *rest; int64_t n_rest; int nxb; };
+__device__ __forceinline__ void step_cams_block(const DevProblem &d, const double *__restrict__ z, const double *dz,
+                                                double *__restrict__ zt, const StepCams &sc) {
+    const int64_t g0 = (int64_t)blockIdx.x * blockDim.x + threadIdx.x, stride = (int64_t)sc.nxb * blockDim.x;
+    for (int64_t i = g0; i < d.NS; i += stride) zt[i] = z[i] + dz[i];
+    for (int64_t i = g0; i < 3 * sc.n_rest; i += stride) {
+        const int64_t e = d.NS + 3 * (int64_t)sc.rest[i / 3] + i % 3;
+        zt[e] = z[e] + dz[e];
+    }
+    const int nw = (blockDim.x + 63) >> 6;
+    if ((threadIdx.x & 63) == 0)
+        for (int c = blockIdx.x * nw + (threadIdx.x >> 6); c < d.nc; c += sc.nxb * nw)
+            cam_prep_one(d, [=](int64_t q) { return z[q] + dz[q]; }, c, sc.cams_t);
+}
+__device__ __forceinline__ void backsub_point_tail(const DevProblem &d, int64_t zp, const double zv[3] ,
+                                                   const double g[3], const double dp[3], double *__restrict__ zt,
+                                                   double (&acc)[BS_NP]) {
+    if (!zt) return;
+#pragma unroll
+    for (int c = 0; c < 3; ++c) {
+        zt[zp + c] = zv[c] + dp[c];
+        if (!d.all_mine && !d.z_mine[zp + c]) continue;
+        const double w = d.any_prior ? d.z_prw[zp + c] : 0.0;
+        if (w > 0) acc[0] += w * dp[c] * dp[c];
+        acc[1] += g[c] * dp[c];
+        acc[2] += dp[c] * dp[c];
+    }
 }
 
 template <int MODEL, bool PRE>
@@ -985,12 +1016,16 @@
                                                        const CamRec *__restrict__ cams,
                                                        const double *__restrict__ Vinv, const double *__restrict__ gp,
                                                  double *__restrict__ dz,
-                                                       double *__restrict__ partial ) {
+                                                       double *__restrict__ partial ,
+                                                       double *__restrict__ zt ,
+                                                       StepCams sc) {
+    if ((int)blockIdx.x < sc.nxb) { step_cams_block(d, z, dz, zt, sc); return; }
+    const int bid = blockIdx.x - sc.nxb;
     constexpr int NCX = WITH_IO ? MAXCOL : 6;
-    __shared__ double sh[3 * 4];
+    __shared__ double sh[BS_NP * 4];
     __shared__ double dps[3];
     const int t = threadIdx.x, BT = blockDim.x;
-    const int64_t o0 = d.giant_start[blockIdx.x], o1 = d.giant_start[blockIdx.x + 1];
+    const int64_t o0 = d.giant_start[bid], o1 = d.giant_start[bid + 1];
     const int k = (int)(o1 - o0);
     const int pt = d.o_pt[o0];
     double s[3] = {0, 0, 0};
@@ -1008,6 +1043,7 @@
         s[2] = fma2(s[2], B[0][2], tt[0], B[1][2], tt[1]);
     }
     block_sum<3>(s, sh);
+    double tail[BS_NP] = {0, 0, 0, 0, 0};
     if (t == 0) {
         for (int q = 0; q < 3; ++q) s[q] += gp[3 * (int64_t)pt + q];
         double p0, p1, p2;
@@ -1015,9 +1051,13 @@
         const int64_t zp = d.NS + 3 * (int64_t)pt;
         dps[0] = d.z_est[zp] ? p0 : 0.0; dps[1] = d.z_est[zp + 1] ? p1 : 0.0; dps[2] = d.z_est[zp + 2] ? p2 : 0.0;
         dz[zp] = dps[0]; dz[zp + 1] = dps[1]; dz[zp + 2] = dps[2];
+        const double g3[3] = {gp[3 * (int64_t)pt], gp[3 * (int64_t)pt + 1], gp[3 * (int64_t)pt + 2]};
+        const double dp3[3] = {dps[0], dps[1], dps[2]};
+        const double zv3[3] = {z[zp], z[zp + 1], z[zp + 2]};
+        backsub_point_tail(d, zp, zv3, g3, dp3, zt, tail);
     }
     __syncthreads();
-    double acc[2] = {0, 0};
+    double acc[BS_NP] = {tail[0], tail[1], tail[2], 0, 0};
     for (int i = t; i < k; i += BT) {
         const int64_t o = o0 + i;
         const CamRec &C = cams[d.o_cam[o]];
@@ -1029,10 +1069,12 @@
             if (a < ncol) { const double dc = dz[C.col[a]]; tt[0] += E[0][a] * dc; tt[1] += E[1][a] * dc; }
         const double j0 = tt[0] + B[0][0] * dps[0] + B[0][1] * dps[1] + B[0][2] * dps[2];
         const double j1 = tt[1] + B[1][0] * dps[0] + B[1][1] * dps[1] + B[1][2] * dps[2];
-        acc[0] = fma2(acc[0], j0, j0, j1, j1);
-    }
-    block_sum<2>(acc, sh);
-    if (t == 0) { partial[2 * blockIdx.x] = acc[0]; partial[2 * blockIdx.x + 1] = acc[1]; }
+        acc[3] = fma2(acc[3], j0, j0, j1, j1);
+    }
+    block_sum<BS_NP>(acc, sh);
+    if (t == 0)
+#pragma unroll
+        for (int q = 0; q < BS_NP; ++q) partial[BS_NP * (int64_t)bid + q] = acc[q];
 }
 
 typedef double mfma_d4 __attribute__((ext_vector_type(4)));
@@ -2541,15 +2583,18 @@
                                                  const CamRec *__restrict__ cams,
                                                  const double *__restrict__ Vinv, const double *__restrict__ gp,
                                                  double *__restrict__ dz,
-                                                 double *__restrict__ partial , int batch0) {
+                                                 double *__restrict__ partial , int batch0,
+                                                 double *__restrict__ zt ,
+                                                 StepCams sc) {
+    if ((int)blockIdx.x < sc.nxb) { step_cams_block(d, z, dz, zt, sc); return; }
     constexpr int NCX = NCXT;
     constexpr bool WITH_IO = NCXT > 6;
     extern __shared__ double smem[];
     double *red = smem;
     double *dpl = red + (size_t)blockDim.x * 3;
-    __shared__ double sh[16];
+    __shared__ double sh[BS_NP * 4];
     const int t = threadIdx.x;
-    const int batch = batch0 + blockIdx.x;
+    const int batch = batch0 + (int)blockIdx.x - sc.nxb;
     const int64_t o0 = d.batch_start[batch];
     const int nobs = (int)(d.batch_start[batch + 1] - o0);
     const bool active = t < nobs;
@@ -2558,6 +2603,7 @@
     double E[2][NCX];
     double B[2][3] = {{0, 0, 0}, {0, 0, 0}};
     int pt = 0, seg_start = 0, seg_len = 0;
+    double acc[BS_NP] = {0, 0, 0, 0, 0};
     if (active) {
         const int cam = d.o_cam[o]; pt = d.o_pt[o];
         const uint32_t sg = d.o_seg[o];
@@ -2582,17 +2628,22 @@
         const double q0 = d.z_est[zp] ? p0 : 0.0, q1 = d.z_est[zp + 1] ? p1 : 0.0, q2 = d.z_est[zp + 2] ? p2 : 0.0;
         dz[zp] = q0; dz[zp + 1] = q1; dz[zp + 2] = q2;
         dpl[3 * t] = q0; dpl[3 * t + 1] = q1; dpl[3 * t + 2] = q2;
+        const double g3[3] = {gp[3 * (int64_t)pt], gp[3 * (int64_t)pt + 1], gp[3 * (int64_t)pt + 2]};
+        const double dp3[3] = {q0, q1, q2};
+        const double zv3[3] = {z[zp], z[zp + 1], z[zp + 2]};
+        backsub_point_tail(d, zp, zv3, g3, dp3, zt, acc);
     }
     __syncthreads();
-    double acc[2] = {0, 0};
     if (active) {
         const double *dp = dpl + 3 * seg_start;
         const double j0 = tt[0] + B[0][0] * dp[0] + B[0][1] * dp[1] + B[0][2] * dp[2];
         const double j1 = tt[1] + B[1][0] * dp[0] + B[1][1] * dp[1] + B[1][2] * dp[2];
-        acc[0] = j0 * j0 + j1 * j1;
-    }
-    block_sum<2>(acc, sh);
-    if (t == 0) { partial[2 * (int64_t)batch] = acc[0]; partial[2 * (int64_t)batch + 1] = acc[1]; }
+        acc[3] = j0 * j0 + j1 * j1;
+    }
+    block_sum<BS_NP>(acc, sh);
+    if (t == 0)
+#pragma unroll
+        for (int q = 0; q < BS_NP; ++q) partial[BS_NP * (int64_t)batch + q] = acc[q];
 }
 
 __device__ __forceinline__ void fwd_ray_terms(const CamRec &C, int nK, int nP, double u, double v, double out[9]) {
@@ -2723,12 +2774,20 @@
                                                   int64_t nbs, const double *__restrict__ ldiag,
                                                   unsigned long long *__restrict__ pivmm, const int *__restrict__ info,
                                                   double *__restrict__ out, double *__restrict__ mailbox,
-                                                  unsigned long long seq, const uint8_t *__restrict__ piv_have = nullptr) {
+                                                  unsigned long long seq, const uint8_t *__restrict__ piv_have = nullptr,
+                                                  int bs_rows = 0) {
     __shared__ double sh[80];
     double acc[5] = {0, 0, 0, 0, 0};
     const int64_t stride = (int64_t)gridDim.x * blockDim.x;
+    const int64_t n_mine = bs_rows == 2 ? d.NS : d.NZ;
     double pmin = 1e300, pmax = 0.0;
-    for (int64_t i = (int64_t)blockIdx.x * blockDim.x + threadIdx.x; i < d.NZ; i += stride) {
+    if (bs_rows == 2) {
+        const int64_t g0 = (int64_t)blockIdx.x * blockDim.x + threadIdx.x;
+        for (int64_t b = g0; b < nbs; b += stride)
+#pragma unroll
+            for (int q = 0; q < BS_NP; ++q) acc[q] += bs_partial[BS_NP * b + q];
+    }
+    for (int64_t i = (int64_t)blockIdx.x * blockDim.x + threadIdx.x; i < n_mine; i += stride) {
         if (ldiag && i < d.NS && d.z_est[i] && (!piv_have || piv_have[i])) {
             double p = ldiag[i];
             p = p == p ? p : 0.0;
@@ -2751,7 +2810,10 @@
         }
         __builtin_amdgcn_s_waitcnt(0);
     }
-    if (grid_sum<5, 2, 3>(acc, sh, partial, ctr, bs_partial, nbs, 2) && threadIdx.x == 0) {
+    static_assert(BS_NP == 5, "k_prior_jv: a row of the back-substitution's partial sums is its own acc[]");
+    const bool last = bs_rows ? grid_sum<5, BS_NP, 0>(acc, sh, partial, ctr, bs_partial, bs_rows == 2 ? 0 : nbs, BS_NP)
+                              : grid_sum<5, 2, 3>(acc, sh, partial, ctr, bs_partial, nbs, 2);
+    if (last && threadIdx.x == 0) {
         out[0] = acc[3]; out[1] = acc[4]; out[4] = acc[0]; out[5] = acc[1]; out[6] = acc[2];
         out[7] = info && __hip_atomic_load(info, __ATOMIC_RELAXED, __HIP_MEMORY_SCOPE_AGENT) != 0 ? 1.0 : 0.0;
         out[2] = 0.0; out[3] = 0.0;
diff --git a/dbat_amd/csrc/sig.hpp b/dbat_amd/csrc/sig.hpp
--- a/dbat_amd/csrc/sig.hpp
+++ b/dbat_amd/csrc/sig.hpp
@@ -698,17 +698,20 @@
                                                      const CamRec *__restrict__ cams,
                                                      const double *__restrict__ Vinv, const double *__restrict__ gp,
                                                      double *__restrict__ dz, double *__restrict__ partial ,
+                                                     double *__restrict__ zt , StepCams sc,
                                                      const int32_t *__restrict__ sg_chunk, int nchunks,
                                                      const int32_t *__restrict__ sg_gcam,
                                                      const double *__restrict__ sg_uv, const double *__restrict__ sg_w) {
     constexpr int CW = (int)((sizeof(CamRec) + 7) / 8);
-    __shared__ double sh[8];
+    __shared__ double sh[BS_NP * 4];
     __shared__ double crec[4][SIG_KMAXR][CW];
     __shared__ double dcs[4][SIG_KMAXR][NCX];
     const int t = threadIdx.x, lane = t & 63;
     const int wv = t >> 6;
-    const int ch = __builtin_amdgcn_readfirstlane(blockIdx.x * 4 + (t >> 6));
-    double acc[2] = {0, 0};
+    if ((int)blockIdx.x < sc.nxb) { step_cams_block(d, z, dz, zt, sc); return; }
+    const int bid = blockIdx.x - sc.nxb;
+    const int ch = __builtin_amdgcn_readfirstlane(bid * 4 + (t >> 6));
+    double acc[BS_NP] = {0, 0, 0, 0, 0};
     if (ch < nchunks) {
         const int32_t *cd = sg_chunk + 8 * (int64_t)ch;
         const int pt0 = cd[0], npts = cd[1], k = cd[2], gm = cd[4], gi0 = cd[5], uv0 = cd[6];
@@ -773,20 +776,25 @@
             tt2 += lane_get(tt2, lane ^ m);
         }
         {
-            const double s0 = gp[3 * (int64_t)pt] + sB[0], s1 = gp[3 * (int64_t)pt + 1] + sB[1], s2 = gp[3 * (int64_t)pt + 2] + sB[2];
+            const double g3[3] = {gp[3 * (int64_t)pt], gp[3 * (int64_t)pt + 1], gp[3 * (int64_t)pt + 2]};
+            const double s0 = g3[0] + sB[0], s1 = g3[1] + sB[1], s2 = g3[2] + sB[2];
             double p0, p1, p2;
             point_block_solve_neg(Vinv + 6 * (int64_t)pt, s0, s1, s2, p0, p1, p2);
             const double d0 = (est & 1u) ? p0 : 0.0, d1 = (est & 2u) ? p1 : 0.0, d2 = (est & 4u) ? p2 : 0.0;
             if (act && lane == pi) {
                 dz[zp] = d0; dz[zp + 1] = d1; dz[zp + 2] = d2;
-                acc[0] = tt2 + 2.0 * (d0 * sB[0] + d1 * sB[1] + d2 * sB[2])
+                const double dp3[3] = {d0, d1, d2};
+                backsub_point_tail(d, zp, Q, g3, dp3, zt, acc);
+                acc[3] = tt2 + 2.0 * (d0 * sB[0] + d1 * sB[1] + d2 * sB[2])
                        + d0 * (V0[0] * d0 + V0[1] * d1 + V0[2] * d2) + d1 * (V0[1] * d0 + V0[3] * d1 + V0[4] * d2)
                        + d2 * (V0[2] * d0 + V0[4] * d1 + V0[5] * d2);
             }
         }
     }
-    block_sum<2>(acc, sh);
-    if (t == 0) { partial[2 * blockIdx.x] = acc[0]; partial[2 * blockIdx.x + 1] = acc[1]; }
+    block_sum<BS_NP>(acc, sh);
+    if (t == 0)
+#pragma unroll
+        for (int q = 0; q < BS_NP; ++q) partial[BS_NP * (int64_t)bid + q] = acc[q];
 }
 
 }
```

New measurement: 637.3, median of 6. Within noise of the previous version (+0.5%).
